# SaurabhIndi/unet-segmentation

Measured on AMD Instinct MI355X. Metric: training images/sec (512×512×1, batch=8) at 1/2/4/8 MI355X; IoU vs ref, higher is better.
Workload: dtype fp32; 1 GPU; U-Net train step 512x512x1, batch 8/GPU, fp32 GEMMs (fwd+WCE+bwd+SGD); global_batch=8, image=512, parallelism=dp1

## Files before the change

### include/unet_hip.h

```cpp
#ifndef UNET_HIP_H
#define UNET_HIP_H

#include <stddef.h>
#include <stdint.h>

#ifdef __cplusplus
extern "C" {
#endif

typedef void* unet_stream_t;

const char* unet_version(void);
const char* unet_last_error(void);

typedef struct unet_plan unet_plan;

unet_plan* unet_plan_create(int n, int c_in, int h, int w, int n_classes);

enum { UNET_PREC_FP32 = 0, UNET_PREC_BF16 = 1, UNET_PREC_BF16X3 = 2 };
unet_plan* unet_plan_create_ex(int n, int c_in, int h, int w, int n_classes, int precision);
int unet_plan_precision(const unet_plan* p);
void unet_plan_destroy(unet_plan* p);
int unet_plan_out_hw(const unet_plan* p, int* out_h, int* out_w);
size_t unet_plan_workspace_bytes(const unet_plan* p);
size_t unet_plan_forward_workspace_bytes(const unet_plan* p);
int unet_plan_num_params(const unet_plan* p);
int unet_plan_num_grads(const unet_plan* p);

int unet_plan_forward(unet_plan* p, void* const* host_params, const float* x_nchw,
                      float* logits_nchw, void* workspace, int train, unet_stream_t stream);

int unet_plan_num_segments(const unet_plan* p);
int unet_plan_segment_grads(const unet_plan* p, int seg, int* first_grad, int* n_grads);
int unet_plan_backward(unet_plan* p, void* const* host_params, void* const* host_grads,
                       const float* x_nchw, const float* dlogits_nchw, void* workspace,
                       int seg_begin, int seg_end, unet_stream_t stream);
size_t unet_plan_input_grad_scratch_bytes(const unet_plan* p);
int unet_plan_input_grad(unet_plan* p, void* const* params, float* dx, void* workspace, void* scratch,
                         unet_stream_t stream);
enum { UNET_BWD_DEFER_JOIN = 1 };
int unet_plan_backward_ex(unet_plan* p, void* const* host_params, void* const* host_grads,
                          const float* x_nchw, const float* dlogits_nchw, void* workspace,
                          int seg_begin, int seg_end, int flags, unet_stream_t stream);
int unet_plan_wait_segment(unet_plan* p, int seg, unet_stream_t stream);
int unet_plan_join(unet_plan* p, unet_stream_t stream);

enum {
  UNET_KC_CONV_FWD = 0, UNET_KC_CONV_DGRAD = 1, UNET_KC_CONV_WGRAD = 2,
  UNET_KC_STAGE1 = 3,
  UNET_KC_ELEMWISE = 4,
  UNET_KC_BOTTLENECK = 5,
  UNET_KC_COUNT = 6
};
int unet_plan_set_timing(unet_plan* p, int enable);
int unet_plan_timing(const unet_plan* p, double* ms, double* flops, double* bytes, int* launches);
int unet_plan_timing_mfma_flops(const unet_plan* p, double* mfma_flops);
size_t unet_plan_timing_sites(const unet_plan* p, char* buf, size_t cap);

int unet_wce_fwd_bwd(const float* logits, const int64_t* targets, const float* weights,
                     int n, int k, int h, int w,
                     const int64_t* t_strides , const int64_t* w_strides ,
                     float* loss_out, float* dlogits, float grad_scale, void* ws,
                     unet_stream_t stream);
int unet_scale_by_device_scalar(float* x, size_t n, const float* g, unet_stream_t stream);
int unet_scale_by_device_scalar_out(const float* x, float* y, size_t n, const float* g, unet_stream_t stream);

int unet_sgd_momentum(float* p, const float* g, float* buf, size_t n, float lr, float momentum,
                      float grad_scale, int first_step, unet_stream_t stream);

int unet_iou_counts(const uint8_t* pred, const uint8_t* gt, size_t n, unsigned long long* out,
                    unet_stream_t stream);
int unet_mask_from_logits(const float* logits, uint8_t* mask, int n, int h, int w,
                          unet_stream_t stream);

size_t unet_elastic_ws_bytes(int n, int h, int w);
int unet_elastic_deform(const uint8_t* image, const uint16_t* labels, int n, int h, int w,
                        const double* noise, double alpha, double sigma, float* x_out,
                        uint8_t* target_out, uint8_t* image_out, void* ws, unet_stream_t stream);
int unet_elastic_deform_ex(const uint8_t* image, const uint16_t* labels, int n, int h, int w,
                           const double* noise, double alpha, double sigma, float* x_out,
                           uint8_t* target_out, uint8_t* image_out, uint16_t* ids_out, void* ws,
                           unet_stream_t stream);

int unet_tile_gather(const float* image, int c, int h, int w, int tile_in, int tile_out, int top, int left,
                     int nx, int first, int stride, int ntiles, float* tiles, unet_stream_t stream);
int unet_tile_scatter(const float* tile_logits, int k, int tile_out, int nx, int first, int stride, int ntiles,
                      int h, int w, float* logits, uint8_t* mask, unet_stream_t stream);

size_t unet_weight_map_ws_bytes(int n);
int unet_weight_map(const uint16_t* labels, int n, int h, int w, double w0, double sigma, float* weights,
                    double* weights64, void* ws, unet_stream_t stream);

size_t unet_weight_map_border_ws_bytes(int n, int h, int w);
int unet_weight_map_border(const uint16_t* labels, int n, int h, int w, double w0, double sigma, float* weights,
                           double* weights64, int32_t* d1sq, int32_t* d2sq, void* ws, unet_stream_t stream);

size_t unet_instance_masks_ws_bytes(int n, int h, int w);
int unet_instance_masks(const uint8_t* mask, int n, int h, int w, int min_size, uint16_t* labels, void* ws,
                        unet_stream_t stream);
size_t unet_rand_index_ws_bytes(int h, int w);
int unet_rand_index(const uint16_t* gt, const uint16_t* pred, int h, int w, double* out, void* ws,
                    unet_stream_t stream);

typedef struct unet_tracker unet_tracker;
unet_tracker* unet_tracker_create(int h, int w, double iou_track, double iou_division, int max_children);
void unet_tracker_destroy(unet_tracker* t);
size_t unet_tracker_ws_bytes(int h, int w);
int unet_tracker_add_frame(unet_tracker* t, const uint16_t* labels, int frame, void* ws, unet_stream_t stream);
int unet_tracker_step_host(unet_tracker* t, int frame, int n_curr, const int32_t* host_labels,
                           const int64_t* host_areas, const int64_t* host_inter);
int unet_tracker_num_tracks(const unet_tracker* t);
int unet_tracker_tracks(const unet_tracker* t, int32_t* host_out, int cap);
int unet_linear_sum_assignment(long long nr, long long nc, const double* host_cost, int64_t* host_row_ind,
                               int64_t* host_col_ind);

enum { UNET_CTC_SEG = 0, UNET_CTC_TRA = 1 };
enum { UNET_CTC_GT = 0, UNET_CTC_RES = 1 };
typedef struct unet_ctc unet_ctc;
unet_ctc* unet_ctc_create(void);
void unet_ctc_destroy(unet_ctc* c);
size_t unet_ctc_ws_bytes(int t, int h, int w);
int unet_ctc_add_frames(unet_ctc* c, int kind, const uint16_t* gt, const uint16_t* res, const int32_t* host_frames,
                        int t, int h, int w, void* ws, unet_stream_t stream);
int unet_ctc_add_frame_host(unet_ctc* c, int kind, int frame, int n_gt, const int32_t* host_gt_labels,
                            const int64_t* host_gt_areas, int n_res, const int32_t* host_res_labels,
                            const int64_t* host_res_areas, int n_pairs, const int64_t* host_pairs);
int unet_ctc_set_tracks(unet_ctc* c, int side, const int32_t* host_rows, int n);
int unet_ctc_measures(unet_ctc* c, double* host_out, int64_t* host_counts);
long long unet_ctc_log(unet_ctc* c, char* buf, size_t cap);
int unet_ctc_num_frames(const unet_ctc* c, int kind);
int unet_ctc_frame_sizes(const unet_ctc* c, int kind, int index, int32_t* host_out);
int unet_ctc_frame_tables(const unet_ctc* c, int kind, int index, int32_t* host_gt_labels, int64_t* host_gt_areas,
                          int32_t* host_res_labels, int64_t* host_res_areas, int64_t* host_pairs);
int unet_ctc_stats(const unet_ctc* c, int64_t* host_out);

enum { UNET_WARP_FORCE_WS = 1 };
size_t unet_warping_error_ws_bytes(int n, int h, int w);
int unet_warping_error(const uint16_t* gt, const uint8_t* pred, int n, int h, int w, int radius, int separate,
                       int max_sweeps, int flags, uint8_t* warped, int64_t* counts, void* ws, unet_stream_t stream);
void unet_simple_point_table(uint8_t out[256]);

int unet_set_tuning(const char* key, int value);
size_t unet_tuning_report(char* buf, size_t len);
int unet_tuning_reset(void);
long long unet_slab_fallbacks(int reset);
long long unet_nondeterministic_sites(int reset);
long long unet_fused_bnb_sites(int reset);
long long unet_wgrad_oihw_sites(int reset);
long long unet_igemm_plane_launches(int reset);
int unet_tuning_save(const char* path);
int unet_tuning_load(const char* path);

int unet_conv3x3_fwd(const float* x, int n, int h, int w, int ci, const float* wt_oihw,
                     const float* bias, int co, const float* x_scale, const float* x_shift,
                     float* y, void* ws, unet_stream_t stream);
int unet_conv3x3_dgrad(const float* dy, int n, int h, int w, int ci, const float* wt_oihw,
                       int co, float* dx, void* ws, unet_stream_t stream);
int unet_conv3x3_wgrad(const float* x, const float* dy, int n, int h, int w, int ci, int co,
                       float* dw_oihw, float* db, void* ws, unet_stream_t stream);
size_t unet_conv_ws_bytes(int n, int h, int w, int ci, int co);
int unet_convT2_fwd(const float* x, int n, int h, int w, int ci, const float* wt, const float* bias,
                    int co, float* y, void* ws, unet_stream_t stream);
int unet_convT2_bwd(const float* x, const float* dy, int n, int h, int w, int ci, const float* wt,
                    int co, float* dx, float* dw, float* db, void* ws, unet_stream_t stream);
int unet_maxpool2_fwd(const float* x, int n, int h, int w, int c, float* y, uint8_t* arg,
                      unet_stream_t stream);
int unet_maxpool2_bwd(const float* dy, const uint8_t* arg, int n, int h, int w, int c, float* dx,
                      unet_stream_t stream);
int unet_bn_train_fwd(const float* x, int n, int h, int w, int c, const float* gamma,
                      const float* beta, float* running_mean, float* running_var, float* y,
                      float* save_mean, float* save_invstd, void* ws, unet_stream_t stream);
int unet_bn_train_bwd(const float* x, const float* dy, int n, int h, int w, int c,
                      const float* gamma, const float* save_mean, const float* save_invstd,
                      float* dx, float* dgamma, float* dbeta, void* ws, unet_stream_t stream);
size_t unet_bn_ws_bytes(int c);

size_t unet_bn_relu_ws_bytes(int n, int h, int w, int c);
int unet_bn_relu_fwd(const float* x, int n, int h, int w, int c, const float* gamma, const float* beta,
                     float* running_mean, float* running_var, int64_t* nbt, float momentum, float eps,
                     int training, int relu, float* y, float* save_mean, float* save_invstd, void* ws,
                     unet_stream_t stream);
int unet_bn_relu_bwd(const float* x, const float* y, const float* dy, int n, int h, int w, int c,
                     const float* gamma, const float* save_mean, const float* save_invstd, int training,
                     int relu, float* dx, float* dgamma, float* dbeta, void* ws, unet_stream_t stream);
size_t unet_conv_first_ws_bytes(int n, int ci, int h, int w);
int unet_conv_first_fwd(const float* x_nchw, int n, int ci, int h, int w, const float* wt, const float* bias,
                        float* y, unet_stream_t stream);
int unet_conv_first_bwd(const float* x_nchw, const float* dy, int n, int ci, int h, int w, const float* wt,
                        float* dx_nchw, float* dw, float* db, void* ws, unet_stream_t stream);
size_t unet_conv1x1_ws_bytes(int k);
int unet_conv1x1_fwd(const float* x, int n, int h, int w, int c, const float* wt, const float* bias, int k,
                     float* logits_nchw, unet_stream_t stream);
int unet_conv1x1_bwd(const float* x, const float* dlogits_nchw, int n, int h, int w, int c, const float* wt, int k,
                     float* dx, float* dw, float* db, void* ws, unet_stream_t stream);

int unet_peak_probe(int kind, int reps, double* result, unet_stream_t stream);

#ifdef __cplusplus
}
#endif
#endif
```

### unet-segmentation_amd/csrc/igemm.hip

```cpp
#include <algorithm>
#include <cstdio>
#include <cstdlib>

#include "gemm_common.h"
#include "ring_common.h"

namespace unet {
constexpr int igemm_minw(int BM, int BN, int WM, int WN, int BK) {
  const int lds = 2 * (BM + BN) * (BK + 4) * 4 + WM * 3 * BN * 4;
  int blocks = 163840 / lds;
  if (blocks > 8) blocks = 8;
  int w = blocks * WM * WN * 64 / 256;
  if (WM * WN >= 8 && w > 2) w = 2;
  return w < 1 ? 1 : (w > 8 ? 8 : w);
}

template <int BM, int BN, int WM, int WN, int BK, int ABL = 0, int PF = 1>
__global__ __launch_bounds__(WM * WN * 64, igemm_minw(BM, BN, WM, WN, BK)) void k_igemm(const IgemmArgs args) {
  constexpr int NT = WM * WN * 64;
  constexpr int LDK = BK + 4;
  constexpr int TM = BM / (WM * 32), TN = BN / (WN * 32);
  constexpr int C4 = BK / 4;
  constexpr int RPP = NT / C4;
  constexpr int AV = BM / RPP, BV = BN / RPP;
// ... 963 lines not shown
int g_tune_igemm = env_int("UNET_IGEMM_VARIANT", -1);
int g_tune_wgrad = env_int("UNET_WGRAD_VARIANT", -1);
std::atomic<long long> g_slab_fallbacks{0};
int g_wino_max = env_int("UNET_WINO_MAX", 4);
int g_wino_dgrad_max = env_int("UNET_WINO_DGRAD_MAX", 4);
int g_wino_wgrad_max = env_int("UNET_WINO_WGRAD_MAX", 6);
int g_wino4_fwd_min_cg = env_int("UNET_WINO4_FWD_MIN_CG", 128);
int g_wino4_fwd_small_cg = env_int("UNET_WINO4_FWD_SMALL_CG", 0);
template <int BM, int BN, int WM, int WN, int BK>
static hipError_t go_igemm(const IgemmArgs& a, hipStream_t s) {
  if (a.N % BN != 0 || a.K % BK != 0 || a.a.Cg % BK != 0 || a.a.c_split % BK != 0) return hipErrorInvalidValue;
  if (a.batch > 1) {
    if (a.ksplit > 1 || a.batch_rows < 1) return hipErrorInvalidValue;
    dim3 grid((a.batch_rows + BM - 1) / BM, a.N / BN, a.batch);
    if (WM == 2 && WN == 2 && igemm_plane_applies(a, BM, BN, BK)) return launch_igemm_plane(a, s, grid, BM, BN, BK);
    hipLaunchKernelGGL((k_igemm<BM, BN, WM, WN, BK>), grid, dim3(WM * WN * 64), 0, s, a);
    return hipGetLastError();
  }
  dim3 grid((a.M + BM - 1) / BM, a.N / BN, a.ksplit > 1 ? a.ksplit : 1);
  hipLaunchKernelGGL((k_igemm<BM, BN, WM, WN, BK>), grid, dim3(WM * WN * 64), 0, s, a);
  return hipGetLastError();
}

template <int BM, int BN, int WM, int WN>
static hipError_t go_igemm_g(const IgemmArgs& a, hipStream_t s) {
  if (a.N % BN != 0 || a.K % 16 != 0 || a.a.Cg % 16 != 0 || a.a.c_split % 16 != 0) return hipErrorInvalidValue;
  static bool attr = false;
  const size_t full = igemm_g_smem<BM, BN>(1024);
  if (!attr) {
    hipError_t e = hipFuncSetAttribute(reinterpret_cast<const void*>(&k_igemm_g<BM, BN, WM, WN>),
                                       hipFuncAttributeMaxDynamicSharedMemorySize, (int)full);
    if (e != hipSuccess) return e;
    attr = true;
  }
  const bool tf = a.a.s[0].scale != nullptr || (a.a.c_split < a.a.Cg && a.a.s[1].scale != nullptr);
  if (tf && a.a.Cg > 1024) return hipErrorInvalidValue;
  const size_t smem = igemm_g_smem<BM, BN>(tf ? a.a.Cg : 0);
  dim3 grid((a.M + BM - 1) / BM, a.N / BN, a.ksplit > 1 ? a.ksplit : 1);
  hipLaunchKernelGGL((k_igemm_g<BM, BN, WM, WN>), grid, dim3(WM * WN * 64), smem, s, a);
  return hipGetLastError();
}

template <int TH, int TW, int BN, int WM, int WN, int MINW>
static hipError_t go_halo32(const IgemmArgs& a, hipStream_t s) {
  if (a.b == nullptr || a.N % BN != 0 || a.a.Cg % 16 != 0 || a.a.c_split % 16 != 0 || a.a.taps_h != 3 ||
      a.a.taps_w != 3 || a.a.stride != 1 || a.K != 9 * a.a.Cg)
    return hipErrorInvalidValue;
  constexpr size_t smem = conv3_f32_smem<TH, TW, BN>();
  static bool attr = false;
  if (!attr) {
    hipError_t e = hipFuncSetAttribute(reinterpret_cast<const void*>(&k_conv3_f32<TH, TW, BN, WM, WN, MINW>),
                                       hipFuncAttributeMaxDynamicSharedMemorySize, (int)smem);
    if (e != hipSuccess) return e;
    attr = true;
  }
  const long long tiles = (long long)a.a.nimg * ((a.a.Hg + TH - 1) / TH) * ((a.a.Wg + TW - 1) / TW);
  dim3 grid((unsigned)tiles, a.N / BN, a.ksplit > 1 ? a.ksplit : 1);
  hipLaunchKernelGGL((k_conv3_f32<TH, TW, BN, WM, WN, MINW>), grid, dim3(WM * WN * 64), smem, s, a);
  return hipGetLastError();
}


template <int BM, int BN>
static hipError_t go_wgrad_f32(const WgradArgs& a, hipStream_t s, dim3 grid) {
  hipLaunchKernelGGL((k_wgrad<BM, BN, 2, 2>), grid, dim3(256), 0, s, a);
  return hipGetLastError();
}

bool reg_tile_fits(const IgemmArgs& a, const IgemmTile& t) {
  return igemm_prec_ok(a, t) && a.N % t.bn == 0 && a.K % t.bk == 0 && a.a.Cg % t.bk == 0 && a.a.c_split % t.bk == 0;
}
bool halo_tile_fits(const IgemmArgs& a, const IgemmTile& t) {
  return igemm_prec_ok(a, t) && a.N % t.bn == 0 && a.a.taps_h == 3 && a.a.taps_w == 3 && a.a.stride == 1 &&
         a.K == 9 * a.a.Cg && a.a.Cg % t.ch == 0 && a.a.c_split % t.ch == 0 && (!t.bf16 || a.a.Cg <= 1024);
}
template <int BM, int BN, int WM, int WN, int BK>
static constexpr IgemmTile reg_tile(int id, int slots) {
  return {id, IgemmFamily::Reg, BM, BN, BK, slots, 0, 0, 0, 0, false, false, true, true, reg_tile_fits,
          &go_igemm<BM, BN, WM, WN, BK>, nullptr, nullptr};
}
template <int BM, int BN, int WM, int WN>
static constexpr IgemmTile dma_tile(int id, int slots) {
  return {id, IgemmFamily::Reg, BM, BN, 16, slots, 0, 0, 0, 0, false, false, true, true, reg_tile_fits,
          &go_igemm_g<BM, BN, WM, WN>, nullptr, nullptr};
}
template <int TH, int TW, int BN, int WM, int WN, int MINW>
static constexpr IgemmTile halo32_tile(int id, int slots) {
  return conv3_tile(id, IgemmFamily::Halo, TH, TW, BN, 16, slots, false, false, true, halo_tile_fits,
                    &go_halo32<TH, TW, BN, WM, WN, MINW>);
}
static const IgemmTile kF32Tiles[] = {
    reg_tile<256, 128, 4, 2, 16>(4, 2),    reg_tile<128, 128, 2, 2, 16>(1, 3),   reg_tile<64, 128, 2, 2, 16>(2, 4),
    reg_tile<128, 64, 2, 2, 16>(8, 4),     reg_tile<256, 64, 4, 1, 16>(6, 2),    reg_tile<128, 128, 2, 2, 32>(3, 2),
    reg_tile<64, 128, 2, 2, 32>(9, 2),     reg_tile<256, 64, 4, 1, 32>(7, 1),    dma_tile<256, 128, 4, 2>(11, 2),
    dma_tile<128, 128, 2, 2>(12, 3),       dma_tile<64, 128, 2, 2>(13, 4),       dma_tile<128, 64, 2, 2>(14, 4),
    halo32_tile<8, 32, 64, 8, 1, 4>(51, 2), halo32_tile<16, 16, 64, 8, 1, 4>(52, 2), halo32_tile<8, 32, 64, 4, 1, 2>(53, 2),
    halo32_tile<8, 16, 64, 4, 1, 2>(54, 2),
};

const std::vector<IgemmTile>& igemm_tiles() {
  static const std::vector<IgemmTile> table = [] {
    std::vector<IgemmTile> v;
    for (IgemmTileRows r : {tile_rows(kF32Tiles), igemm_bf16_tile_rows(), conv3_dma_tile_rows(), conv3_ring_tile_rows(),
                            conv3_ring_pt_tile_rows(), conv3_flat_tile_rows(), wino_tile_rows(),
                            conv3_ring_persistent_tile_rows(), gemm_ring_tile_rows(), gemm_ring_p1_tile_rows(),
                            gemm_ring_p2_tile_rows(), conv3_c64_tile_rows()})
      v.insert(v.end(), r.p, r.p + r.n);
    std::stable_partition(v.begin(), v.end(), [](const IgemmTile& t) { return t.tuned; });
    return v;
  }();
  return table;
}

const IgemmTile* igemm_tile(int id) {
  static const std::vector<const IgemmTile*> by_id = [] {
    std::vector<const IgemmTile*> v;
    for (const IgemmTile& t : igemm_tiles()) {
      if ((size_t)t.id >= v.size()) v.resize(t.id + 1, nullptr);
      v[t.id] = &t;
    }
    return v;
  }();
  return id >= 0 && (size_t)id < by_id.size() ? by_id[id] : nullptr;
}

bool igemm_tile_fits(const IgemmArgs& a, int tile) {
  const IgemmTile* t = igemm_tile(tile);
  if (!t) return false;
  const bool fwd = a.fwd != 0;
  if (t->wino_m > (fwd ? g_wino_max : g_wino_dgrad_max)) return false;
  if (fwd && t->wino_m >= 4 && a.a.Cg < g_wino4_fwd_min_cg && a.a.Cg > g_wino4_fwd_small_cg) return false;
  return t->fits(a, *t);
}
long long igemm_tile_count(const IgemmArgs& a, int tile) {
  const IgemmTile* t = igemm_tile(tile);
  if (!t) return 0;
  if (t->count) return t->count(a);
  if (t->th) return (long long)a.a.nimg * ((a.a.Hg + t->th - 1) / t->th) * ((a.a.Wg + t->tw - 1) / t->tw) * (a.N / t->bn);
  return (long long)((a.M + t->bm - 1) / t->bm) * (a.N / t->bn);
}
int igemm_tile_slots(int tile) {
  const IgemmTile* t = igemm_tile(tile);
  return t ? t->slots : 0;
}
size_t igemm_slab_bytes(const IgemmArgs& a, int ksplit) {
  return ksplit > 1 ? (size_t)ksplit * a.M * a.N * sizeof(float) : 0;
}

static hipError_t go_tile(const IgemmArgs& a, hipStream_t s, int tile) {
  const IgemmTile* t = igemm_tile(tile);
  return t ? t->go(a, s) : hipErrorInvalidValue;
}

static bool igemm_args_ok(const IgemmArgs& a) {
  return a.M > 0 && a.N > 0 && a.K > 0 && (a.K % 16) == 0 && (a.a.Cg % 16) == 0 && (a.a.c_split % 16) == 0;
}

GemmChoice resolve_forced_igemm(const IgemmArgs& a, int knob) {
  return knob > 0 && igemm_tile_fits(a, knob) ? GemmChoice{knob, 1} : GemmChoice{};
}

int igemm_heuristic_tile(const IgemmArgs& a) {
  const GemmChoice forced = resolve_forced_igemm(a, g_tune_igemm);
  if (forced.tile >= 0) return forced.tile;
  const long long cus = num_cus();
  if (a.bh != nullptr) {
    if (a.K % 32 || a.a.Cg % 32 || a.a.c_split % 32) return -1;
    if (a.N % 128 == 0) {
      const long long t256 = ((a.M + 255) / 256) * (long long)(a.N / 128);
      const long long t128 = ((a.M + 127) / 128) * (long long)(a.N / 128);
      if (a.N >= 256 && t256 >= 3 * cus / 2) return 21;
      if (t128 >= 2 * cus) return 22;
      return 24;
    }
    return a.N % 64 == 0 ? 23 : -1;
  }
  if (a.N % 128 == 0) {
    const long long t256 = ((a.M + 255) / 256) * (long long)(a.N / 128);
    const long long t128 = ((a.M + 127) / 128) * (long long)(a.N / 128);
    if (a.N >= 256 && t256 >= 3 * cus / 2) return 4;
    if (t128 >= 4 * cus) return 1;
    return 2;
  }
  if (a.N % 64 == 0) return 8;
  return -1;
}

hipError_t launch_igemm(const IgemmArgs& a0, hipStream_t s) {
  if (!igemm_args_ok(a0)) return hipErrorInvalidValue;
  IgemmArgs a = a0;
  a.ksplit = 1;
  return go_tile(a, s, igemm_heuristic_tile(a));
}

hipError_t launch_igemm_v(const IgemmArgs& a0, hipStream_t s, GemmChoice c) {
  if (c.tile < 0) return launch_igemm(a0, s);
  if (!igemm_args_ok(a0) || !igemm_tile_fits(a0, c.tile)) return hipErrorInvalidValue;
  const IgemmTile& t = *igemm_tile(c.tile);
  IgemmArgs a = a0;
  const int nk = a.K / t.bk;
  if (t.family == IgemmFamily::Wino && c.split >= 100) a.wino_choice.tile = c.split - 100;
  int ks = c.split < 1 || t.wino_m ? 1 : (c.split > nk ? nk : c.split);
  if (ks > 1) {
    const int per = (nk + ks - 1) / ks;
    ks = (nk + per - 1) / per;
  }
  a.ksplit = ks;
  if (ks > 1 && (!t.ksplit || a.slab == nullptr || a.N % 64 != 0)) return hipErrorInvalidValue;
  hipError_t e = t.go(a, s);
  if (e != hipSuccess || ks == 1) return e;
  dim3 grid((a.M + 127) / 128, a.N / 64);
  hipLaunchKernelGGL(k_splitk_epi, grid, dim3(256), 0, s, a);
  return hipGetLastError();
}

static bool wgrad_column_fits(const WgradArgs& a, const WgradTile& t) {
  return t.bf16 == (a.bf16 != 0) && a.Mo % t.bm == 0 && a.No % t.bn == 0;
}
template <int BM, int BN>
static constexpr WgradTile wgrad_f32_tile(int id) {
  return {id, WgradFamily::Column, BM, BN, 0, 0, 0, false, 8, wgrad_column_fits, nullptr, &go_wgrad_f32<BM, BN>};
}
template <int TH, int TW>
static constexpr WgradTile wgrad3_f32_tile(int id) {
  return {id, WgradFamily::Halo, 64, 64, TH, TW, 0, false, 4, wgrad3_f32_fits,
          [](const WgradArgs& a, hipStream_t s, WgradMode m) { return go_wgrad3_f32<TH, TW>(a, s, m.per_cu); }, nullptr};
}
static const WgradTile kWgradF32Tiles[] = {wgrad_f32_tile<128, 128>(0), wgrad_f32_tile<128, 192>(1),
                                           wgrad_f32_tile<64, 192>(2), wgrad_f32_tile<64, 128>(3),
                                           wgrad_f32_tile<64, 64>(4)};
static const WgradTile kWgrad3F32Tiles[] = {wgrad3_f32_tile<8, 16>(22), wgrad3_f32_tile<4, 32>(23)};

const std::vector<WgradTile>& wgrad_tiles() {
  static const std::vector<WgradTile> table = [] {
    std::vector<WgradTile> v;
    for (WgradTileRows r : {tile_rows(kWgradF32Tiles), wgrad_bf16_tile_rows(), wgrad3_bf16_tile_rows(),
                            tile_rows(kWgrad3F32Tiles), wgrad3w_tile_rows(), wgrad3_ring_tile_rows(),
                            wgradT_ring_tile_rows(), wino_wgrad_tile_rows()})
      v.insert(v.end(), r.p, r.p + r.n);
    return v;
  }();
  return table;
}

const WgradTile* wgrad_tile(int id) {
  for (const WgradTile& t : wgrad_tiles())
    if (t.id == id) return &t;
  return nullptr;
}

WgradMode decode(const WgradTile& t, int code) {
  WgradMode m{t.default_per_cu, -1, false};
  switch (t.family) {
    case WgradFamily::Column:
      m.slab = code >= 100;
      if (m.slab) code -= 100;
      if (code > 0) m.per_cu = code;
      break;
    case WgradFamily::Halo:
      if (code > 0) m.per_cu = code;
      break;
    case WgradFamily::Ring:
    case WgradFamily::RingT:
      if (code <= 0) code = t.default_per_cu;
      m.slab = code >= 10;
      m.per_cu = m.slab ? code - 10 : code;
      break;
    case WgradFamily::Wino:
      m.slab = code >= 1000;
      code %= 1000;
      if (code >= 100) m.inner = code / 100 - 1;
      if (code % 100 > 0) m.per_cu = code % 100;
      break;
  }
  return m;
}
int encode(const WgradTile& t, WgradMode m) {
  switch (t.family) {
    case WgradFamily::Column: return m.per_cu + (m.slab ? 100 : 0);
    case WgradFamily::Halo: return m.per_cu;
    case WgradFamily::Ring:
    case WgradFamily::RingT: return m.per_cu + (m.slab ? 10 : 0);
    default: return m.per_cu + 100 * (m.inner + 1) + (m.slab ? 1000 : 0);
  }
}

bool wgrad_tile_fits(const WgradArgs& a, int tile) {
  const WgradTile* t = wgrad_tile(tile);
  if (!t || t->wino_m > g_wino_wgrad_max) return false;
  if (a.batch > 1 && (t->family != WgradFamily::Column || t->bf16)) return false;
  return t->fits(a, *t);
}

GemmChoice resolve_forced_wgrad(const WgradArgs& a, int knob) {
  const bool bf16 = a.bf16 != 0;
  const WgradTile* t = wgrad_tile(knob);
  if (t && (bf16 ? knob >= 10 : t->family != WgradFamily::Column) && wgrad_tile_fits(a, knob))
    return {knob, t->family == WgradFamily::Column ? knob : 1};
  t = wgrad_tile(knob - 1000);
  if (t && t->family == WgradFamily::Wino && !bf16 && wgrad_tile_fits(a, t->id)) return {t->id, encode(*t, {0, -1, true})};
  t = wgrad_tile(knob - 100);
  if (t && t->bf16 == bf16 && wgrad_tile_fits(a, t->id)) {
    if (t->family == WgradFamily::Column) return {t->id, encode(*t, {2, -1, true})};
    if (t->family == WgradFamily::Ring || t->family == WgradFamily::RingT) return {t->id, encode(*t, {1, -1, true})};
  }
  if (knob == 1 && !bf16) return {4, 8};
  return {};
}

static int wgrad_heuristic_tile(const WgradArgs& a) {
  if (a.bf16) {
    if (wgrad3_fits(a)) return 20;
    if (a.Mo % 128 == 0 && a.No % 128 == 0) return 10;
    return a.No % 128 == 0 ? 12 : 13;
  }
  if (a.Mo % 128 == 0 && a.No % 128 == 0) return 0;
  if (a.Mo % 128 == 0 && a.No % 192 == 0) return 1;
  if (a.No % 192 == 0) return 2;
  return a.No % 128 == 0 ? 3 : 4;
}

hipError_t launch_wgrad_v(const WgradArgs& a0, hipStream_t s, GemmChoice c) {
  WgradArgs a = a0;
  if (a.Mo % 64 != 0 || a.P <= 0 || a.gb.Cg % 4 != 0 || a.gb.c_split % 4 != 0 || a.ga.Cg % 4 != 0)
    return hipErrorInvalidValue;
  const bool heuristic = c.tile < 0 && resolve_forced_wgrad(a, g_tune_wgrad).tile < 0;
  if (heuristic) c.tile = wgrad_heuristic_tile(a);
  else if (c.tile < 0) c = resolve_forced_wgrad(a, g_tune_wgrad);
  if (!wgrad_tile_fits(a, c.tile)) return hipErrorInvalidValue;
  const WgradTile& t = *wgrad_tile(c.tile);
  WgradMode m = decode(t, c.split);
  if (heuristic && t.family == WgradFamily::Column) m = {g_tune_wgrad >= 2 ? g_tune_wgrad : 8, -1, false};
  if (t.go) return t.go(a, s, m);
  int pps = 0;
  const int splits = wgrad_splits(a, t, m.per_cu, pps);
  a.pix_per_split = pps;
  const size_t plane = (size_t)a.Mo * a.No;
  if (!(m.slab && wgrad_slab_fits(a, splits))) {
    if (m.slab) ++g_slab_fallbacks;
    a.slab = nullptr;
  }
  else if (splits == 1) a.slab = a.out;
// ... 57 lines not shown
```

### unet-segmentation_amd/csrc/ops.hip

```cpp
#include <algorithm>
#include <cerrno>
#include <string>

#include "../../include/unet_hip.h"
#include "unet_internal.h"

using namespace unet;

namespace unet {
extern int g_tune_igemm, g_tune_wgrad, g_autotune, g_force_split, g_force_tile, g_concurrent, g_wino_max,
    g_wino_dgrad_max, g_wino_wgrad_max, g_bf16_norm, g_bn_fold, g_wino4_fwd_min_cg, g_wino4_fwd_small_cg,
    g_maxpool_vec8, g_wgrad_fwd_u, g_ctc_chunk_frames, g_ctc_dense_cells;
hipError_t launch_fill(float* p, size_t n, float v, hipStream_t s);
hipError_t launch_pair_sum(const double* st, int g, int c, float* out, hipStream_t s);
}

namespace {
thread_local std::string g_op_err;
inline size_t al256(size_t b) { return (b + 255) / 256 * 256; }
int g_op_prec = UNET_PREC_FP32;
int g_op_a16 = 0;

hipError_t op_b_to_bf16(IgemmArgs& a, size_t n, void* scratch, hipStream_t s) {
  if (g_op_prec == UNET_PREC_FP32) return hipSuccess;
  uint16_t* bh = reinterpret_cast<uint16_t*>(scratch);
  uint16_t* bl = g_op_prec == UNET_PREC_BF16X3 ? bh + n : nullptr;
  hipError_t e = launch_f2bf(a.b, bh, n, s, bl);
  a.bh = bh;
  a.bl = bl;
  a.b = nullptr;
  return e;
}
}

namespace {
__global__ void k_relu_mask(const float* __restrict__ dy, const float* __restrict__ y, long long n4,
                            float* __restrict__ dz) {
  for (long long i = blockIdx.x * (long long)blockDim.x + threadIdx.x; i < n4; i += (long long)gridDim.x * blockDim.x) {
    const float4 g = reinterpret_cast<const float4*>(dy)[i], v = reinterpret_cast<const float4*>(y)[i];
    reinterpret_cast<float4*>(dz)[i] =
        make_float4(v.x > 0.f ? g.x : 0.f, v.y > 0.f ? g.y : 0.f, v.z > 0.f ? g.z : 0.f, v.w > 0.f ? g.w : 0.f);
  }
}

__global__ void k_bn_eval_stats(int C, const float* rm, const float* rv, float eps, float* mean, float* invstd) {
  const int c = blockIdx.x * blockDim.x + threadIdx.x;
  if (c >= C) return;
  mean[c] = rm[c];
  invstd[c] = (float)(1.0 / sqrt((double)rv[c] + (double)eps));
}
}

#define OPCK(x)                                                           \
  do {                                                                    \
    hipError_t e_ = (x);                                                  \
    if (e_ != hipSuccess) return e_ == hipErrorInvalidValue ? -EINVAL : -EIO; \
  } while (0)

extern "C" {

static size_t op_wino_bytes(int ci, int co) { return al256(sizeof(float) * 36 * (size_t)ci * co); }
static size_t op_wgrad_wino_bytes(int n, int h, int w, int ci, int co);
static size_t op_wgrad_extra_bytes(int n, int h, int w, int ci, int co);
static void op_set_wino(IgemmArgs& a, void* ws, int n, int h, int w, int ci, int co) {
  const size_t ws_bytes = unet_conv_ws_bytes(n, h, w, ci, co);
  const IgemmTile* forced = igemm_tile(g_tune_igemm);
  if (forced && forced->family == IgemmFamily::Wino && op_wgrad_extra_bytes(n, h, w, ci, co)) {
    a.wino_ws = reinterpret_cast<float*>(reinterpret_cast<char*>(ws) + ws_bytes - op_wino_bytes(ci, co) -
                                         op_wgrad_extra_bytes(n, h, w, ci, co));
    a.wino_ws_bytes = op_wgrad_wino_bytes(n, h, w, ci, co);
    return;
  }
  a.wino_ws = reinterpret_cast<float*>(reinterpret_cast<char*>(ws) + ws_bytes - op_wino_bytes(ci, co));
  a.wino_ws_bytes = op_wino_bytes(ci, co);
}

static size_t op_wgrad_wino_bytes(int n, int h, int w, int ci, int co) {
  return al256(wino_ws_bytes_grid(n, h, w, ci, co));
}
static size_t op_wgrad_slab_bytes(int n, int h, int w, int ci, int co) {
  const long long t4 = (long long)n * ((h + 3) / 4) * ((w + 3) / 4);
  return al256(sizeof(float) * 64 * (size_t)std::min<long long>(64, (t4 + 255) / 256) * ci * co);
}
static size_t op_wgrad_extra_bytes(int n, int h, int w, int ci, int co) {
  const size_t b = op_wgrad_wino_bytes(n, h, w, ci, co) + op_wgrad_slab_bytes(n, h, w, ci, co);
  return b <= ((size_t)256 << 20) ? b : 0;
}

size_t unet_conv_ws_bytes(int n, int h, int w, int ci, int co) {
  const size_t wb = al256(sizeof(float) * 9 * (size_t)ci * co);
  const size_t pad = al256(sizeof(float) * (size_t)n * (h + 2) * (w + 2) * co);
  const size_t misc = al256(sizeof(float) * 4 * co) + al256(sizeof(double) * kStatGroups * 2 * co);
  const size_t x16 = al256(sizeof(uint16_t) * (size_t)n * h * w * ci);
  return 2 * wb + pad + misc + x16 + op_wgrad_extra_bytes(n, h, w, ci, co) + op_wino_bytes(ci, co);
}

int unet_conv3x3_fwd(const float* x, int n, int h, int w, int ci, const float* wt, const float* bias, int co,
                     const float* xs, const float* xb, float* y, void* ws, unet_stream_t st) {
  if (ci % 16 || co % 64 || h < 3 || w < 3) return -EINVAL;
  hipStream_t s = reinterpret_cast<hipStream_t>(st);
  float* wf = reinterpret_cast<float*>(ws);
  OPCK(launch_pack_conv(wt, co, ci, 3, 3, wf, nullptr, s));
  IgemmArgs a;
  Src x0;
  x0.ptr = x;
  x0.H = h;
  x0.W = w;
  x0.C = ci;
  x0.scale = xs;
  x0.shift = xb;
  if (g_op_prec == UNET_PREC_BF16 && g_op_a16) {
    const size_t wb = al256(sizeof(float) * 9 * (size_t)ci * co);
    const size_t off = 2 * wb + al256(sizeof(float) * (size_t)n * (h + 2) * (w + 2) * co) +
                       al256(sizeof(float) * 4 * co) + al256(sizeof(double) * kStatGroups * 2 * co);
    uint16_t* x16 = reinterpret_cast<uint16_t*>(reinterpret_cast<char*>(ws) + off);
    OPCK(launch_f2bf(x, x16, (size_t)n * h * w * ci, s));
    x0.ptr = reinterpret_cast<const float*>(x16);
    x0.h16 = 1;
  }
  a.a.s[0] = a.a.s[1] = x0;
  a.a.Cg = a.a.c_split = ci;
  a.a.taps_h = a.a.taps_w = 3;
  a.a.Hg = h - 2;
  a.a.Wg = w - 2;
  a.a.nimg = n;
  a.b = wf;
  a.M = n * (h - 2) * (w - 2);
  a.N = co;
  a.K = 9 * ci;
  a.e.bias = bias;
  a.e.d[0] = Dst{y, h - 2, w - 2, co, 0, 0};
  op_set_wino(a, ws, n, h, w, ci, co);
  OPCK(op_b_to_bf16(a, 9 * (size_t)ci * co, reinterpret_cast<char*>(ws) + al256(sizeof(float) * 9 * (size_t)ci * co),
                    s));
  OPCK(launch_igemm(a, s));
  return 0;
}

int unet_conv3x3_dgrad(const float* dy, int n, int h, int w, int ci, const float* wt, int co, float* dx, void* ws,
                       unet_stream_t st) {
  if (ci % 64 || co % 16 || h < 3 || w < 3) return -EINVAL;
  hipStream_t s = reinterpret_cast<hipStream_t>(st);
  char* p = reinterpret_cast<char*>(ws);
  const size_t wb = al256(sizeof(float) * 9 * (size_t)ci * co);
  float* wf = reinterpret_cast<float*>(p);
  float* wd = reinterpret_cast<float*>(p + wb);
  float* dyp = reinterpret_cast<float*>(p + 2 * wb);
  float* coef = reinterpret_cast<float*>(p + 2 * wb + al256(sizeof(float) * (size_t)n * (h + 2) * (w + 2) * co));
  OPCK(launch_pack_conv(wt, co, ci, 3, 3, wf, wd, s));
  OPCK(launch_fill(coef, co, 1.f, s));
  OPCK(launch_fill(coef + co, 3 * (size_t)co, 0.f, s));
  const int dy16 = g_op_prec == UNET_PREC_BF16 && g_op_a16;
  OPCK(launch_bnb_apply(dy, dy, coef, n, h - 2, w - 2, co, dyp, 2, s, dy16, 0));
  IgemmArgs a;
  Src d;
  d.ptr = dyp;
  d.h16 = dy16;
  d.H = h + 2;
  d.W = w + 2;
  d.C = co;
  a.a.s[0] = a.a.s[1] = d;
  a.a.Cg = a.a.c_split = co;
  a.a.taps_h = a.a.taps_w = 3;
  a.a.Hg = h;
  a.a.Wg = w;
  a.a.nimg = n;
  a.b = wd;
  a.M = n * h * w;
  a.N = ci;
  a.K = 9 * co;
  a.e.d[0] = Dst{dx, h, w, ci, 0, 0};
  op_set_wino(a, ws, n, h, w, ci, co);
  OPCK(op_b_to_bf16(a, 9 * (size_t)ci * co, wf, s));
  OPCK(launch_igemm(a, s));
  return 0;
}

int unet_conv3x3_wgrad(const float* x, const float* dy, int n, int h, int w, int ci, int co, float* dw, float* db,
                       void* ws, unet_stream_t st) {
  if (ci % 64 || co % 64 || h < 3 || w < 3) return -EINVAL;
  hipStream_t s = reinterpret_cast<hipStream_t>(st);
  char* p = reinterpret_cast<char*>(ws);
  const size_t wb = al256(sizeof(float) * 9 * (size_t)ci * co);
  float* dwp = reinterpret_cast<float*>(p);
  double* st2 = reinterpret_cast<double*>(p + 2 * wb + al256(sizeof(float) * (size_t)n * (h + 2) * (w + 2) * co) +
                                          al256(sizeof(float) * 4 * co));
  OPCK(hipMemsetAsync(dwp, 0, sizeof(float) * 9 * (size_t)ci * co, s));
  WgradArgs a;
  Src d;
  d.ptr = dy;
  d.H = h - 2;
  d.W = w - 2;
  d.C = co;
  a.ga.s[0] = a.ga.s[1] = d;
  a.ga.Cg = a.ga.c_split = co;
  a.ga.Hg = h - 2;
  a.ga.Wg = w - 2;
  a.ga.nimg = n;
  Src xs;
  xs.ptr = x;
  xs.H = h;
  xs.W = w;
  xs.C = ci;
  a.gb.s[0] = a.gb.s[1] = xs;
  a.gb.Cg = a.gb.c_split = ci;
  a.gb.taps_h = a.gb.taps_w = 3;
  a.gb.Hg = h - 2;
  a.gb.Wg = w - 2;
  a.gb.nimg = n;
  a.Mo = co;
  a.No = 9 * ci;
  a.P = n * (h - 2) * (w - 2);
  a.out = dwp;
  a.bf16 = g_op_prec != UNET_PREC_FP32;
  a.split = g_op_prec == UNET_PREC_BF16X3;
  if (g_op_prec == UNET_PREC_BF16 && g_op_a16) {
    uint16_t* dy16 = reinterpret_cast<uint16_t*>(p + 2 * wb);
    float* coef = reinterpret_cast<float*>(p + 2 * wb + al256(sizeof(float) * (size_t)n * (h + 2) * (w + 2) * co));
    uint16_t* x16 = reinterpret_cast<uint16_t*>(p + 2 * wb + al256(sizeof(float) * (size_t)n * (h + 2) * (w + 2) * co) +
                                                al256(sizeof(float) * 4 * co) +
                                                al256(sizeof(double) * kStatGroups * 2 * co));
    OPCK(launch_fill(coef, co, 1.f, s));
    OPCK(launch_fill(coef + co, 3 * (size_t)co, 0.f, s));
    OPCK(launch_bnb_apply(dy, dy, coef, n, h - 2, w - 2, co, reinterpret_cast<float*>(dy16), 2, s, 1, 0));
    OPCK(launch_f2bf(x, x16, (size_t)n * h * w * ci, s));
    a.ga.s[0].ptr = a.ga.s[1].ptr = reinterpret_cast<const float*>(dy16);
    a.ga.s[0].H = a.ga.s[1].H = h + 2;
    a.ga.s[0].W = a.ga.s[1].W = w + 2;
    a.ga.s[0].oy = a.ga.s[1].oy = a.ga.s[0].ox = a.ga.s[1].ox = 2;
    a.ga.s[0].h16 = a.ga.s[1].h16 = 1;
    a.gb.s[0].ptr = a.gb.s[1].ptr = reinterpret_cast<const float*>(x16);
    a.gb.s[0].h16 = a.gb.s[1].h16 = 1;
  }
  const WgradTile* forced = wgrad_tile(g_tune_wgrad >= 1000 ? g_tune_wgrad - 1000 : g_tune_wgrad);
  if (forced && forced->family == WgradFamily::Wino && !a.bf16 && op_wgrad_extra_bytes(n, h, w, ci, co)) {
    char* e = p + unet_conv_ws_bytes(n, h, w, ci, co) - op_wino_bytes(ci, co) - op_wgrad_extra_bytes(n, h, w, ci, co);
    a.wino_ws = reinterpret_cast<float*>(e);
    a.wino_ws_bytes = op_wgrad_wino_bytes(n, h, w, ci, co);
    a.slab = reinterpret_cast<float*>(e + a.wino_ws_bytes);
    a.slab_bytes = op_wgrad_slab_bytes(n, h, w, ci, co);
  }
  OPCK(launch_wgrad(a, s));
  OPCK(launch_permute_last2(dwp, co, 9, ci, dw, s));
  if (db) {
    OPCK(hipMemsetAsync(st2, 0, sizeof(double) * kStatGroups * 2 * co, s));
    OPCK(launch_channel_stats(dy, (size_t)n * (h - 2) * (w - 2), co, st2, s));
    OPCK(launch_pair_sum(st2, kStatGroups, co, db, s));
  }
  return 0;
}

int unet_convT2_fwd(const float* x, int n, int h, int w, int ci, const float* wt, const float* bias, int co, float* y,
                    void* ws, unet_stream_t st) {
  if (ci % 16 || co % 16) return -EINVAL;
  hipStream_t s = reinterpret_cast<hipStream_t>(st);
  char* p = reinterpret_cast<char*>(ws);
  float* wf = reinterpret_cast<float*>(p);
  float* wd = reinterpret_cast<float*>(p + al256(sizeof(float) * 4 * (size_t)ci * co));
  OPCK(launch_pack_convT(wt, ci, co, wf, wd, s));
  IgemmArgs a;
  Src x0;
  x0.ptr = x;
  x0.H = h;
  x0.W = w;
  x0.C = ci;
  a.a.s[0] = a.a.s[1] = x0;
  a.a.Cg = a.a.c_split = ci;
  a.a.Hg = h;
  a.a.Wg = w;
  a.a.nimg = n;
  a.b = wf;
  a.M = n * h * w;
  a.N = 4 * co;
  a.K = ci;
  a.e.bias = bias;
  a.e.shuffle_co = co;
  a.e.d[0] = Dst{y, 2 * h, 2 * w, co, 0, 0};
  OPCK(op_b_to_bf16(a, 4 * (size_t)ci * co, p + 2 * al256(sizeof(float) * 4 * (size_t)ci * co), s));
  OPCK(launch_igemm(a, s));
  return 0;
}

int unet_convT2_bwd(const float* x, const float* dy, int n, int h, int w, int ci, const float* wt, int co, float* dx,
                    float* dw, float* db, void* ws, unet_stream_t st) {
  if (ci % 64 || co % 64) return -EINVAL;
  hipStream_t s = reinterpret_cast<hipStream_t>(st);
  char* p = reinterpret_cast<char*>(ws);
  const size_t wb = al256(sizeof(float) * 4 * (size_t)ci * co);
  float* wf = reinterpret_cast<float*>(p);
  float* wd = reinterpret_cast<float*>(p + wb);
  float* dwp = reinterpret_cast<float*>(p + 2 * wb);
  double* st2 = reinterpret_cast<double*>(p + 3 * wb);
  OPCK(launch_pack_convT(wt, ci, co, wf, wd, s));
  Src d;
  d.ptr = dy;
  d.H = 2 * h;
  d.W = 2 * w;
  d.C = co;
  IgemmArgs a;
  a.a.s[0] = a.a.s[1] = d;
  a.a.Cg = a.a.c_split = co;
  a.a.taps_h = a.a.taps_w = 2;
  a.a.stride = 2;
  a.a.Hg = h;
  a.a.Wg = w;
  a.a.nimg = n;
  a.b = wd;
  a.M = n * h * w;
  a.N = ci;
  a.K = 4 * co;
  a.e.d[0] = Dst{dx, h, w, ci, 0, 0};
  OPCK(op_b_to_bf16(a, 4 * (size_t)ci * co, wf, s));
  OPCK(launch_igemm(a, s));
  OPCK(hipMemsetAsync(dwp, 0, sizeof(float) * 4 * (size_t)ci * co, s));
  WgradArgs g;
  Src x0;
  x0.ptr = x;
  x0.H = h;
  x0.W = w;
  x0.C = ci;
  g.ga.s[0] = g.ga.s[1] = x0;
  g.ga.Cg = g.ga.c_split = ci;
  g.ga.Hg = h;
  g.ga.Wg = w;
  g.ga.nimg = n;
// ... 81 lines not shown
  double* stats = reinterpret_cast<double*>(p);
  float* scale = reinterpret_cast<float*>(p + al256(sizeof(double) * kStatGroups * 2 * c));
  float* shift = scale + al256(sizeof(float) * c) / 4;
  const size_t pix = (size_t)n * h * w;
  if (training) {
    OPCK(hipMemsetAsync(stats, 0, sizeof(double) * kStatGroups * 2 * c, s));
    OPCK(launch_channel_stats(x, pix, c, stats, s));
    OPCK(launch_bn_finalize(stats, c, (double)pix, gamma, beta, rm, rv, nbt, save_mean, save_invstd, scale, shift,
                            momentum, eps, s));
  } else {
    OPCK(launch_bn_eval_prepare(c, gamma, beta, rm, rv, scale, shift, eps, s));
    hipLaunchKernelGGL(k_bn_eval_stats, dim3((c + 255) / 256), dim3(256), 0, s, c, rm, rv, eps, save_mean,
                       save_invstd);
    OPCK(hipGetLastError());
  }
  OPCK(launch_affine_relu(x, pix, c, scale, shift, relu, y, s));
  return 0;
}

int unet_bn_relu_bwd(const float* x, const float* y, const float* dy, int n, int h, int w, int c, const float* gamma,
                     const float* save_mean, const float* save_invstd, int training, int relu, float* dx,
                     float* dgamma, float* dbeta, void* ws, unet_stream_t st) {
  if (!x || !dy || !dx || !gamma || c < 4 || c % 4 || 256 % (c / 4) || n < 1 || (relu && !y)) return -EINVAL;
  hipStream_t s = reinterpret_cast<hipStream_t>(st);
  char* p = reinterpret_cast<char*>(ws);
  double* stats = reinterpret_cast<double*>(p);
  float* coef = reinterpret_cast<float*>(p + al256(sizeof(double) * kStatGroups * 2 * c));
  float* dz = reinterpret_cast<float*>(p + unet_bn_ws_bytes(c));
  const size_t pix = (size_t)n * h * w;
  const float* g = dy;
  if (relu) {
    const long long n4 = (long long)(pix * c / 4);
    hipLaunchKernelGGL(k_relu_mask, dim3((unsigned)std::min<long long>((n4 + 255) / 256, 8192)), dim3(256), 0, s, dy,
                       y, n4, dz);
    OPCK(hipGetLastError());
    g = dz;
  }
  OPCK(hipMemsetAsync(stats, 0, sizeof(double) * kStatGroups * 2 * c, s));
  OPCK(launch_bn_bwd_stats(g, x, save_mean, save_invstd, pix, c, stats, s));
  OPCK(launch_bnb_finalize(stats, c, (double)pix, gamma, save_mean, save_invstd, dgamma, dbeta, nullptr, coef, s,
                           training ? 0 : 1));
  OPCK(launch_bnb_apply(g, x, coef, n, h, w, c, dx, 0, s));
  return 0;
}

size_t unet_conv_first_ws_bytes(int n, int ci, int h, int w) {
  (void)n; (void)h; (void)w;
  return conv_first_wgrad_ws_bytes(ci) + al256(sizeof(double) * kStatGroups * 2 * 64);
}

int unet_conv_first_fwd(const float* x, int n, int ci, int h, int w, const float* wt, const float* bias, float* y,
                        unet_stream_t st) {
  if (!x || !wt || !bias || !y || n < 1 || ci < 1 || h < 3 || w < 3) return -EINVAL;
  OPCK(launch_conv_first_fwd(x, n, ci, h, w, wt, bias, 64, y, nullptr, reinterpret_cast<hipStream_t>(st)));
  return 0;
}

int unet_conv_first_bwd(const float* x, const float* dy, int n, int ci, int h, int w, const float* wt, float* dx,
                        float* dw, float* db, void* ws, unet_stream_t st) {
  if (!x || !dy || !wt || !dw || !db || !ws || n < 1 || ci < 1 || h < 3 || w < 3) return -EINVAL;
  hipStream_t s = reinterpret_cast<hipStream_t>(st);
  char* p = reinterpret_cast<char*>(ws);
  float* slabs = reinterpret_cast<float*>(p);
  double* st2 = reinterpret_cast<double*>(p + conv_first_wgrad_ws_bytes(ci));
  Src d;
  d.ptr = dy;
  d.H = h - 2;
  d.W = w - 2;
  d.C = 64;
  OPCK(launch_conv_first_wgrad(x, n, ci, h, w, d, 64, dw, slabs, s));
  OPCK(hipMemsetAsync(st2, 0, sizeof(double) * kStatGroups * 2 * 64, s));
  OPCK(launch_channel_stats(dy, (size_t)n * (h - 2) * (w - 2), 64, st2, s));
  OPCK(launch_pair_sum(st2, kStatGroups, 64, db, s));
  if (dx) OPCK(launch_conv_first_dgrad(dy, n, ci, h, w, wt, dx, s));
  return 0;
}

size_t unet_conv1x1_ws_bytes(int k) { return al256(sizeof(double) * ((size_t)k * 64 + k)); }

int unet_conv1x1_fwd(const float* x, int n, int h, int w, int c, const float* wt, const float* bias, int k,
                     float* logits, unet_stream_t st) {
  if (!x || !wt || !bias || !logits || c != 64 || k < 1 || n < 1) return -EINVAL;
  Src s0;
  s0.ptr = x;
  s0.H = h;
  s0.W = w;
  s0.C = 64;
  OPCK(launch_head_fwd(s0, n, h, w, 64, wt, bias, k, logits, reinterpret_cast<hipStream_t>(st)));
  return 0;
}

int unet_conv1x1_bwd(const float* x, const float* dl, int n, int h, int w, int c, const float* wt, int k, float* dx,
                     float* dw, float* db, void* ws, unet_stream_t st) {
  if (!x || !dl || !wt || !dw || !db || !ws || c != 64 || k < 1 || n < 1) return -EINVAL;
  OPCK(launch_head_bwd_plain(x, dl, n, h, w, wt, k, dx, dw, db, reinterpret_cast<double*>(ws),
                             reinterpret_cast<hipStream_t>(st)));
  return 0;
}

int unet_wce_fwd_bwd(const float* logits, const int64_t* t, const float* wm, int n, int k, int h, int w,
                     const int64_t* ts, const int64_t* wsd, float* loss, float* dl, float gscale, void* ws,
                     unet_stream_t st) {
  if (!ts || !wsd || k < 1) return -EINVAL;
  OPCK(launch_wce(logits, t, wm, n, k, h, w, ts, wsd, loss, dl, gscale, reinterpret_cast<double*>(ws),
                  reinterpret_cast<hipStream_t>(st)));
  return 0;
}

int unet_scale_by_device_scalar(float* x, size_t n, const float* g, unet_stream_t st) {
  OPCK(launch_scale_by_dev(x, x, n, g, reinterpret_cast<hipStream_t>(st)));
  return 0;
}

int unet_scale_by_device_scalar_out(const float* x, float* y, size_t n, const float* g, unet_stream_t st) {
  OPCK(launch_scale_by_dev(x, y, n, g, reinterpret_cast<hipStream_t>(st)));
  return 0;
}

int unet_sgd_momentum(float* p, const float* g, float* buf, size_t n, float lr, float mom, float gscale, int first,
                      unet_stream_t st) {
  OPCK(launch_sgd(p, g, buf, n, lr, mom, gscale, first, reinterpret_cast<hipStream_t>(st)));
  return 0;
}

int unet_iou_counts(const uint8_t* a, const uint8_t* b, size_t n, unsigned long long* out, unet_stream_t st) {
  OPCK(launch_iou(a, b, n, out, reinterpret_cast<hipStream_t>(st)));
  return 0;
}

int unet_set_tuning(const char* key, int value) {
  if (!key) return -EINVAL;
  const std::string k(key);
  if (k == "igemm_variant") g_tune_igemm = value;
  else if (k == "wgrad_variant") g_tune_wgrad = value;
  else if (k == "autotune") g_autotune = value;
  else if (k == "force_split") g_force_split = value;
  else if (k == "force_tile") g_force_tile = value;
  else if (k == "concurrent") g_concurrent = value;
  else if (k == "wino_max") g_wino_max = value;
  else if (k == "bf16_norm") g_bf16_norm = value;
  else if (k == "bn_fold") g_bn_fold = value != 0;
  else if (k == "wino_dgrad_max") g_wino_dgrad_max = value;
  else if (k == "wino_wgrad_max") g_wino_wgrad_max = value;
  else if (k == "wino4_fwd_min_cg") g_wino4_fwd_min_cg = value;
  else if (k == "wino4_fwd_small_cg") g_wino4_fwd_small_cg = value;
  else if (k == "op_a16") g_op_a16 = value != 0;
  else if (k == "maxpool_vec8") g_maxpool_vec8 = value;
  else if (k == "bnb_fuse") g_bnb_fuse = value;
  else if (k == "wgrad_early_u") g_wgrad_early_u = value;
  else if (k == "wgrad_fwd_u") g_wgrad_fwd_u = value;
  else if (k == "wgrad_plane") g_wgrad_plane = value;
  else if (k == "wgrad_oihw") g_wgrad_oihw = value;
  else if (k == "igemm_plane") g_igemm_plane = value;
  else if (k == "wino_point_tile") g_wino_point_tile = value;
  else if (k == "ctc_chunk_frames" || k == "ctc_dense_cells") {
    if (value < -1 || (value == 0 && k == "ctc_chunk_frames")) return -EINVAL;
    (k == "ctc_chunk_frames" ? g_ctc_chunk_frames : g_ctc_dense_cells) = value;
  }
  else if (k == "deterministic") g_deterministic = value != 0;
  else if (k == "op_precision") {
    if (value != UNET_PREC_FP32 && value != UNET_PREC_BF16 && value != UNET_PREC_BF16X3) return -EINVAL;
    g_op_prec = value;
  } else return -EINVAL;
  return 0;
}

int unet_tile_gather(const float* image, int c, int h, int w, int tile_in, int tile_out, int top, int left, int nx,
                     int first, int stride, int ntiles, float* tiles, unet_stream_t st) {
  if (!image || !tiles) return -EINVAL;
  OPCK(launch_tile_gather(image, c, h, w, tile_in, tile_out, top, left, nx, first, stride, ntiles, tiles,
                          reinterpret_cast<hipStream_t>(st)));
  return 0;
}

int unet_tile_scatter(const float* tile_logits, int k, int tile_out, int nx, int first, int stride, int ntiles, int h,
                      int w, float* logits, uint8_t* mask, unet_stream_t st) {
  if (!tile_logits) return -EINVAL;
  OPCK(launch_tile_scatter(tile_logits, k, tile_out, nx, first, stride, ntiles, h, w, logits, mask,
                           reinterpret_cast<hipStream_t>(st)));
  return 0;
}

size_t unet_instance_masks_ws_bytes(int n, int h, int w) {
  return n > 0 && h > 0 && w > 0 ? instance_masks_ws_bytes(n, h, w) : 0;
}

int unet_instance_masks(const uint8_t* mask, int n, int h, int w, int min_size, uint16_t* labels, void* ws,
                        unet_stream_t st) {
  if (!mask || !labels || !ws) return -EINVAL;
  OPCK(launch_instance_masks(mask, n, h, w, min_size, labels, ws, reinterpret_cast<hipStream_t>(st)));
  return 0;
}

size_t unet_rand_index_ws_bytes(int h, int w) { return h > 0 && w > 0 ? rand_index_ws_bytes(h, w) : 0; }

int unet_rand_index(const uint16_t* gt, const uint16_t* pred, int h, int w, double* out, void* ws,
                    unet_stream_t st) {
  if (!gt || !pred || !out || !ws) return -EINVAL;
  OPCK(launch_rand_index(gt, pred, h, w, out, ws, reinterpret_cast<hipStream_t>(st)));
  return 0;
}

size_t unet_weight_map_ws_bytes(int n) { return n > 0 ? weight_map_ws_bytes(n) : 0; }

int unet_weight_map(const uint16_t* labels, int n, int h, int w, double w0, double sigma, float* weights,
                    double* weights64, void* ws, unet_stream_t st) {
  if (!labels || !weights || !ws || (reinterpret_cast<uintptr_t>(ws) & 7)) return -EINVAL;
  OPCK(launch_weight_map(labels, n, h, w, w0, sigma, weights, weights64, ws, reinterpret_cast<hipStream_t>(st)));
  return 0;
}

size_t unet_weight_map_border_ws_bytes(int n, int h, int w) { return weight_map_border_ws_bytes(n, h, w); }

int unet_weight_map_border(const uint16_t* labels, int n, int h, int w, double w0, double sigma, float* weights,
                           double* weights64, int32_t* d1sq, int32_t* d2sq, void* ws, unet_stream_t st) {
  if (n < 1 || h < 1 || w < 1 || h > 16384 || w > 16384) {
    set_last_error("unet_weight_map_border: need n, h, w >= 1 and h, w <= 16384 (h^2 + w^2 must fit int32)");
    return -EINVAL;
  }
  if (!labels || !weights || !ws || (reinterpret_cast<uintptr_t>(ws) & 15)) {
    set_last_error("unet_weight_map_border: null labels / weights / ws, or ws not 16-byte aligned");
    return -EINVAL;
  }
  const hipError_t e = launch_weight_map_border(labels, n, h, w, w0, sigma, weights, weights64, d1sq, d2sq, ws,
                                                reinterpret_cast<hipStream_t>(st));
  if (e != hipSuccess) {
    set_last_error(std::string("unet_weight_map_border: ") + hipGetErrorString(e));
    return e == hipErrorInvalidValue ? -EINVAL : -EIO;
  }
  return 0;
}

size_t unet_elastic_ws_bytes(int n, int h, int w) { return n > 0 && h > 0 && w > 0 ? elastic_ws_bytes(n, h, w) : 0; }

int unet_elastic_deform_ex(const uint8_t* image, const uint16_t* labels, int n, int h, int w, const double* noise,
                           double alpha, double sigma, float* x_out, uint8_t* target_out, uint8_t* image_out,
                           uint16_t* ids_out, void* ws, unet_stream_t st) {
  if (!image || !labels || !noise || !x_out || !target_out || !ws || (reinterpret_cast<uintptr_t>(ws) & 7)) return -EINVAL;
  OPCK(launch_elastic(image, labels, n, h, w, noise, alpha, sigma, x_out, target_out, image_out, ids_out, ws,
                      reinterpret_cast<hipStream_t>(st)));
  return 0;
}

int unet_elastic_deform(const uint8_t* image, const uint16_t* labels, int n, int h, int w, const double* noise,
                        double alpha, double sigma, float* x_out, uint8_t* target_out, uint8_t* image_out, void* ws,
                        unet_stream_t st) {
  return unet_elastic_deform_ex(image, labels, n, h, w, noise, alpha, sigma, x_out, target_out, image_out, nullptr, ws,
                                st);
}

int unet_mask_from_logits(const float* logits, uint8_t* mask, int n, int h, int w, unet_stream_t st) {
  OPCK(launch_mask(logits, mask, n, h, w, reinterpret_cast<hipStream_t>(st)));
  return 0;
}

}
```

### unet-segmentation_amd/csrc/plan.hip

```cpp
#include <cerrno>
#include <cstdio>
#include <cstdlib>
#include <cstring>
#include <algorithm>
#include <array>
#include <map>
#include <mutex>
#include <string>
#include <vector>

#include "../../include/unet_hip.h"
#include "unet_internal.h"

using namespace unet;

namespace unet {
extern int g_wino_max, g_wino_dgrad_max, g_wino_wgrad_max, g_wino4_fwd_min_cg, g_wino4_fwd_small_cg;
int g_autotune = getenv("UNET_AUTOTUNE") ? atoi(getenv("UNET_AUTOTUNE")) : 1;
int g_concurrent = getenv("UNET_CONCURRENT") ? atoi(getenv("UNET_CONCURRENT")) : 1;
int g_bf16_norm = getenv("UNET_BF16_NORM") ? atoi(getenv("UNET_BF16_NORM")) : 0;
int g_bn_fold = getenv("UNET_BN_FOLD") ? atoi(getenv("UNET_BN_FOLD")) : 1;
int g_force_split = 0;
int g_force_tile = 0;
int g_deterministic = getenv("UNET_DETERMINISTIC") ? atoi(getenv("UNET_DETERMINISTIC")) : 0;
// ... 1224 lines not shown
      Conv& L = p->L[l];
      if (L.co % 64 == 0) L.vdw = al.take(bnb_wino6_vd_bytes(n, L.ho, L.wo, L.co));
    }
    for (int l = 1; l < 18 && unet::g_wgrad_fwd_u; ++l) {
      Conv& L = p->L[l];
      L.uws = al.take(wino_ws_bytes_grid(n, L.ho, L.wo, L.ci, L.co));
    }
  }
  p->wslab = al.take((size_t)2 * num_cus() * 128 * 9 * 64 * sizeof(float));
  p->ws_bytes = al.top;
  return p;
}

void unet_plan_destroy(unet_plan* p) {
  if (!p) return;
  if (p->side) {
    (void)hipStreamSynchronize(p->side);
    for (auto ev : p->ev_dy) (void)hipEventDestroy(ev);
    for (auto ev : p->ev_du) (void)hipEventDestroy(ev);
    for (auto ev : p->ev_seg) (void)hipEventDestroy(ev);
    (void)hipEventDestroy(p->ev_join);
    (void)hipEventDestroy(p->ev_bwd0);
    (void)hipEventDestroy(p->ev_fwdu);
    (void)hipStreamDestroy(p->side);
  }
  for (auto& e : p->evs) {
    (void)hipEventDestroy(e.a);
    (void)hipEventDestroy(e.b);
  }
  delete p;
}

int unet_plan_out_hw(const unet_plan* p, int* oh, int* ow) {
  if (!p) return -EINVAL;
  if (oh) *oh = p->ho;
  if (ow) *ow = p->wo;
  return 0;
}
size_t unet_plan_workspace_bytes(const unet_plan* p) { return p ? p->ws_bytes : 0; }
size_t unet_plan_forward_workspace_bytes(const unet_plan* p) { return p ? p->fwd_ws_bytes : 0; }
int unet_plan_num_params(const unet_plan*) { return 136; }
int unet_plan_num_grads(const unet_plan*) { return 82; }
int unet_plan_num_segments(const unet_plan*) { return 9; }
int unet_plan_segment_grads(const unet_plan*, int seg, int* first, int* cnt) {
  int f, k;
  if (seg == 0) { f = 70; k = 12; }
  else if (seg <= 3) { f = 70 - 10 * seg; k = 10; }
  else if (seg <= 8) { f = 8 * (8 - seg); k = 8; }
  else return -EINVAL;
  if (first) *first = f;
  if (cnt) *cnt = k;
  return 0;
}

int unet_plan_forward(unet_plan* p, void* const* prm, const float* x, float* logits, void* ws, int train,
                      unet_stream_t stream) {
  if (!p || !prm || !x || !logits || !ws) {
    set_err("unet_plan_forward: null argument");
    return -EINVAL;
  }
  if (reinterpret_cast<uintptr_t>(ws) & 255) {
    set_err("unet_plan_forward: workspace must be 256-byte aligned");
    return -EINVAL;
  }
  return run_forward(p, prm, x, logits, reinterpret_cast<char*>(ws), train, reinterpret_cast<hipStream_t>(stream));
}

int unet_plan_backward(unet_plan* p, void* const* prm, void* const* grd, const float* x, const float* dlogits,
                       void* ws, int sb, int se, unet_stream_t stream) {
  if (!p || !prm || !grd || !x || !dlogits || !ws || sb < 0 || se > 9 || sb >= se) {
    set_err("unet_plan_backward: bad argument");
    return -EINVAL;
  }
  return run_backward(p, prm, grd, x, dlogits, reinterpret_cast<char*>(ws), sb, se,
                      reinterpret_cast<hipStream_t>(stream), 0);
}

int unet_plan_backward_ex(unet_plan* p, void* const* prm, void* const* grd, const float* x, const float* dlogits,
                          void* ws, int sb, int se, int flags, unet_stream_t stream) {
  if (!p || !prm || !grd || !x || !dlogits || !ws || sb < 0 || se > 9 || sb >= se || (flags & ~UNET_BWD_DEFER_JOIN)) {
    set_err("unet_plan_backward_ex: bad argument");
    return -EINVAL;
  }
  return run_backward(p, prm, grd, x, dlogits, reinterpret_cast<char*>(ws), sb, se,
                      reinterpret_cast<hipStream_t>(stream), flags);
}

size_t unet_plan_input_grad_scratch_bytes(const unet_plan* p) {
  return p ? (size_t)p->n * p->L[0].ho * p->L[0].wo * p->L[0].co * sizeof(float) : 0;
}

int unet_plan_input_grad(unet_plan* p, void* const* prm, float* dx, void* ws, void* scratch, unet_stream_t stream) {
  if (!p || !prm || !dx || !ws || !scratch) {
    set_err("unet_plan_input_grad: bad argument");
    return -EINVAL;
  }
  const hipStream_t s = reinterpret_cast<hipStream_t>(stream);
  Ctx c{p, reinterpret_cast<char*>(ws), s};
  const Conv& L = p->L[0];
  const int g16 = p->prec == UNET_PREC_BF16;
  float* dy0 = reinterpret_cast<float*>(scratch);
  CK(launch_bnb_apply(c.f(L.dz), c.f(L.y), c.f(L.coef), p->n, L.ho, L.wo, L.co, dy0, 0, s, 0,
                      p->prec == UNET_PREC_BF16, g16));
  CK(launch_conv_first_dgrad(dy0, p->n, p->cin, p->h, p->w, P<float>(prm, L.pw), dx, s));
  return 0;
}

int unet_plan_wait_segment(unet_plan* p, int seg, unet_stream_t stream) {
  if (!p || seg < 0 || seg >= 9) {
    set_err("unet_plan_wait_segment: bad argument");
    return -EINVAL;
  }
  if (!p->seg_on_side[seg] || !p->side) return 0;
  CK(hipStreamWaitEvent(reinterpret_cast<hipStream_t>(stream), p->ev_seg[seg], 0));
  return 0;
}

int unet_plan_join(unet_plan* p, unet_stream_t stream) {
  if (!p) {
    set_err("unet_plan_join: null plan");
    return -EINVAL;
  }
  if (!p->side || !p->side_pending) return 0;
  CK(hipEventRecord(p->ev_join, p->side));
  CK(hipStreamWaitEvent(reinterpret_cast<hipStream_t>(stream), p->ev_join, 0));
  p->side_pending = false;
  return 0;
}

size_t unet_tuning_report(char* buf, size_t len) {
  std::string r;
  {
    std::lock_guard<std::mutex> lk(g_tune_mu);
    for (const auto& kv : g_tune_log) r += kv.second + "\n";
  }
  if (buf && len > 0) {
    const size_t k = std::min(len - 1, r.size());
    memcpy(buf, r.data(), k);
    buf[k] = 0;
  }
  return r.size() + 1;
}

long long unet_nondeterministic_sites(int reset) {
  return reset ? g_nondet_sites.exchange(0) : g_nondet_sites.load();
}

long long unet_fused_bnb_sites(int reset) {
  return reset ? unet::g_fused_bnb_sites.exchange(0) : unet::g_fused_bnb_sites.load();
}
long long unet_wgrad_oihw_sites(int reset) {
  return reset ? unet::g_wgrad_oihw_sites.exchange(0) : unet::g_wgrad_oihw_sites.load();
}
long long unet_igemm_plane_launches(int reset) {
  return reset ? unet::g_igemm_plane_launches.exchange(0) : unet::g_igemm_plane_launches.load();
}
long long unet_slab_fallbacks(int reset) {
  return reset ? g_slab_fallbacks.exchange(0) : g_slab_fallbacks.load();
}

int unet_tuning_reset(void) {
  std::lock_guard<std::mutex> lk(g_tune_mu);
  g_tuned.clear();
  g_tune_log.clear();
  return 0;
}

int unet_tuning_save(const char* path) {
  if (!path) return -EINVAL;
  std::lock_guard<std::mutex> lk(g_tune_mu);
  FILE* f = fopen(path, "w");
  if (!f) return -errno;
  for (const auto& kv : g_tuned) fprintf(f, "%s\t%d\t%d\n", kv.first.c_str(), kv.second.tile, kv.second.split);
  fclose(f);
  return (int)g_tuned.size();
}

int unet_tuning_load(const char* path) {
  if (!path) return -EINVAL;
  std::lock_guard<std::mutex> lk(g_tune_mu);
  return tune_db_read(path, true);
}

int unet_plan_set_timing(unet_plan* p, int enable) {
  if (!p) return -EINVAL;
  p->timing = enable != 0;
  return 0;
}

int unet_plan_timing(const unet_plan* pc, double* ms, double* fl, double* by, int* cnt) {
  auto* p = const_cast<unet_plan*>(pc);
  if (!p) return -EINVAL;
  int rc = 0;
  for (auto& e : p->evs) {
    float t = 0;
    if (hipEventSynchronize(e.b) != hipSuccess || hipEventElapsedTime(&t, e.a, e.b) != hipSuccess) {
      set_err("unet_plan_timing: event query failed");
      rc = -EIO;
    } else {
      p->t_ms[e.cls] += t;
      p->t_fl[e.cls] += e.flops;
      p->t_by[e.cls] += e.bytes;
      p->t_xf[e.cls] += e.xflops;
      p->t_n[e.cls] += 1;
      if (e.site >= 0) {
        auto& v = p->sites[e.site];
        v[0] += t;
        v[1] += e.flops;
        v[2] += e.xflops;
      }
    }
    (void)hipEventDestroy(e.a);
    (void)hipEventDestroy(e.b);
  }
  p->evs.clear();
  for (int i = 0; i < UNET_KC_COUNT; ++i) {
    if (ms) ms[i] = p->t_ms[i];
    if (fl) fl[i] = p->t_fl[i];
    if (by) by[i] = p->t_by[i];
    if (cnt) cnt[i] = p->t_n[i];
    p->t_xf_last[i] = p->t_xf[i];
    p->t_ms[i] = p->t_fl[i] = p->t_by[i] = p->t_xf[i] = 0;
    p->t_n[i] = 0;
  }
  p->sites_last.swap(p->sites);
  p->sites.clear();
  return rc;
}

size_t unet_plan_timing_sites(const unet_plan* p, char* buf, size_t cap) {
  if (!p) return 0;
  std::string out;
  for (const auto& kv : p->sites_last) {
    char line[160];
    snprintf(line, sizeof line, "%s\t%.4f\t%.6e\t%.6e\n", site_name(kv.first).c_str(), kv.second[0], kv.second[1],
             kv.second[2]);
    out += line;
  }
  if (buf && cap) {
    const size_t m = out.size() < cap - 1 ? out.size() : cap - 1;
    memcpy(buf, out.data(), m);
    buf[m] = 0;
  }
  return out.size() + 1;
}

int unet_plan_timing_mfma_flops(const unet_plan* p, double* xfl) {
  if (!p || !xfl) return -EINVAL;
  for (int i = 0; i < UNET_KC_COUNT; ++i) xfl[i] = p->t_xf_last[i];
  return 0;
}

}
```

### unet-segmentation_amd/csrc/unet_internal.h

```cpp
#pragma once
#include <hip/hip_runtime.h>
#include <cstddef>
#include <cstdint>
#include <atomic>
#include <string>
#include <vector>

namespace unet {

constexpr int kMaxInChannels = 4096;
constexpr int kMaxClassCount = 4096;

struct Src {
  const float* ptr = nullptr;
  int H = 0, W = 0, C = 0;
  int oy = 0, ox = 0;
  const float* scale = nullptr;
  const float* shift = nullptr;
  int h16 = 0;
};

struct Gather {
  Src s[2];
  int c_split = 0;
  int Cg = 0;
  int taps_h = 1, taps_w = 1;
  int stride = 1;
  int Hg = 0, Wg = 0;
  int nimg = 0;
};

struct Dst {
  float* ptr = nullptr;
  int H = 0, W = 0, C = 0;
  int oy = 0, ox = 0;
  int h16 = 0;
};

struct Epilogue {
  const float* bias = nullptr;
  int shuffle_co = 0;
  Dst d[2];
  int n_split = 1 << 30;
  int relu = 0;
  double* stats = nullptr;
  const float* yref = nullptr;
  int yref_h16 = 0;
  const float* bn_scale = nullptr;
  const float* bn_shift = nullptr;
  const float* bn_mean = nullptr;
  const float* bn_invstd = nullptr;
  double* bstats = nullptr;
  double* colsum1 = nullptr;
};

constexpr int kStatGroups = 64;

struct IgemmArgs {
  Gather a;
  const float* b = nullptr;
  const uint16_t* bh = nullptr;
  const uint16_t* bl = nullptr;
  int M, N, K;
  Epilogue e;
  int ksplit = 1;
  float* slab = nullptr;
  float* wino_ws = nullptr;
  size_t wino_ws_bytes = 0;
  int batch = 1;
  int batch_rows = 0;
  long long batch_b = 0;
  struct { int tile = -1, split = 1; } wino_choice;
  int fwd = 0;
};

extern std::atomic<long long> g_slab_fallbacks;
extern int g_deterministic;
extern int g_bnb_fuse;
extern int g_wgrad_early_u;
extern int g_wgrad_plane;
extern int g_wgrad_oihw;
extern int g_igemm_plane;
extern std::atomic<long long> g_igemm_plane_launches;
extern int g_wino_point_tile;
extern std::atomic<long long> g_nondet_sites;

struct WgradArgs {
  Gather ga;
  Gather gb;
  int Mo, No;
  int P;
  int pix_per_split;
  float* out;
  float* out_oihw = nullptr;
  float* slab = nullptr;
  size_t slab_bytes = 0;
  int accumulate = 0;
  int bf16 = 0;
  int split = 0;
  int batch = 1;
  long long batch_a = 0, batch_b = 0, batch_out = 0;
  float* wino_ws = nullptr;
  size_t wino_ws_bytes = 0;
  const float* vd_pre = nullptr;
  int u_ready = 0;
  int abl = 0;
};

struct GemmChoice {
  int tile = -1;
  int split = 1;
};

enum class IgemmFamily {
  Reg,
  Halo,
  Conv3Dma,
  Ring,
  Flat,
  C64,
  GemmRing,
  Wino,
  WinoFused
};
struct IgemmTile {
  int id;
  IgemmFamily family;
  int bm, bn, bk, slots;
  int th, tw, ch;
  int wino_m;
  bool bf16;
  bool x3;
  bool ksplit;
  bool tuned;
  bool (*fits)(const IgemmArgs&, const IgemmTile&);
  hipError_t (*go)(const IgemmArgs&, hipStream_t);
  long long (*count)(const IgemmArgs&);
  size_t (*slab_bytes)(const IgemmArgs&);
};
struct IgemmTileRows {
  const IgemmTile* p;
  int n;
};
template <int N>
constexpr IgemmTileRows tile_rows(const IgemmTile (&r)[N]) { return {r, N}; }
constexpr IgemmTile conv3_tile(int id, IgemmFamily f, int th, int tw, int bn, int ch, int slots, bool bf16, bool x3,
                               bool ksplit, bool (*fits)(const IgemmArgs&, const IgemmTile&),
                               hipError_t (*go)(const IgemmArgs&, hipStream_t)) {
  return {id, f, th * tw, bn, 9 * ch, slots, th, tw, ch, 0, bf16, x3, ksplit, true, fits, go, nullptr, nullptr};
}
IgemmTileRows igemm_bf16_tile_rows();
IgemmTileRows conv3_dma_tile_rows();
IgemmTileRows conv3_ring_tile_rows();
IgemmTileRows conv3_ring_pt_tile_rows();
IgemmTileRows conv3_ring_persistent_tile_rows();
IgemmTileRows conv3_flat_tile_rows();
IgemmTileRows conv3_c64_tile_rows();
IgemmTileRows gemm_ring_tile_rows();
IgemmTileRows gemm_ring_p1_tile_rows();
IgemmTileRows gemm_ring_p2_tile_rows();
IgemmTileRows wino_tile_rows();
const std::vector<IgemmTile>& igemm_tiles();
const IgemmTile* igemm_tile(int id);
inline bool igemm_prec_ok(const IgemmArgs& a, const IgemmTile& t) {
  return t.bf16 ? a.bh != nullptr && (a.bl == nullptr || t.x3) : a.b != nullptr;
}

enum class WgradFamily { Column, Halo, Ring, RingT, Wino };
struct WgradMode {
  int per_cu;
  int inner;
  bool slab;
};
struct WgradTile {
  int id;
  WgradFamily family;
  int bm, bn;
  int th, tw;
  int wino_m;
  bool bf16;
  int default_per_cu;
  bool (*fits)(const WgradArgs&, const WgradTile&);
  hipError_t (*go)(const WgradArgs&, hipStream_t, WgradMode);
  hipError_t (*go_column)(const WgradArgs&, hipStream_t, dim3 grid);
};
struct WgradTileRows {
  const WgradTile* p;
  int n;
};
template <int N>
constexpr WgradTileRows tile_rows(const WgradTile (&r)[N]) { return {r, N}; }
WgradTileRows wgrad_bf16_tile_rows();
WgradTileRows wgrad3_bf16_tile_rows();
WgradTileRows wgrad3w_tile_rows();
WgradTileRows wgrad3_ring_tile_rows();
WgradTileRows wgradT_ring_tile_rows();
WgradTileRows wino_wgrad_tile_rows();
const std::vector<WgradTile>& wgrad_tiles();
const WgradTile* wgrad_tile(int id);
WgradMode decode(const WgradTile& t, int code);
int encode(const WgradTile& t, WgradMode m);
GemmChoice resolve_forced_igemm(const IgemmArgs& a, int knob);
GemmChoice resolve_forced_wgrad(const WgradArgs& a, int knob);
size_t wino_ws_bytes(long long T, int Cg, int N);
size_t wino_ws_bytes_grid(int nimg, int H, int W, int Cg, int N);
bool wino_applies(const IgemmArgs& a, int mt);
hipError_t launch_wino(const IgemmArgs& a, hipStream_t s, int mt);
bool wino_wgrad_applies(const WgradArgs& a, int mt);
double igemm_exec_flops(const IgemmArgs& a, GemmChoice c);
double wgrad_exec_flops(const WgradArgs& a, GemmChoice c);
hipError_t launch_wino_wgrad(const WgradArgs& a, hipStream_t s, WgradMode m, int mt);
int wgrad_winograd_mt(const WgradArgs& a, GemmChoice c);
hipError_t launch_wino_wgrad_u(const WgradArgs& a, hipStream_t s, int mt);
size_t bnb_wino6_vd_bytes(int n, int h, int w, int c);
hipError_t launch_bnb_wino6_dy(const float* dz, const float* y, const float* coef, int n, int h, int w, int c,
                               float* dypad, float* vd, hipStream_t s);
bool conv3_ring_fits(const IgemmArgs& a, const IgemmTile& t);
bool gemm_ring_fits(const IgemmArgs& a, const IgemmTile& t);
size_t conv3_flat_sk_slab_bytes(const IgemmArgs& a);
int num_cus();

int ablation_env(const char* name);
hipError_t launch_igemm(const IgemmArgs& a, hipStream_t s);
hipError_t launch_igemm_v(const IgemmArgs& a, hipStream_t s, GemmChoice c);
int igemm_heuristic_tile(const IgemmArgs& a);
bool igemm_tile_fits(const IgemmArgs& a, int tile);
long long igemm_tile_count(const IgemmArgs& a, int tile);
int igemm_tile_slots(int tile);
size_t igemm_slab_bytes(const IgemmArgs& a, int ksplit);
std::string igemm_key(const IgemmArgs& a);
std::string wgrad_key(const WgradArgs& a);
std::vector<GemmChoice> igemm_candidates(const IgemmArgs& a, size_t slab_bytes);
std::vector<GemmChoice> wgrad_candidates(const WgradArgs& a);
bool wgrad_choice_deterministic(const GemmChoice& g);
hipError_t launch_wgrad(const WgradArgs& a, hipStream_t s);
hipError_t launch_wgrad_v(const WgradArgs& a, hipStream_t s, GemmChoice c);
// ... 123 lines not shown
```

### unet-segmentation_amd/csrc/winograd.hip

```cpp
#include <algorithm>
#include <cstdlib>

#include "gemm_common.h"
#include "ring_common.h"

namespace unet {

__global__ void k_wino_w(const float* __restrict__ b, int N, int Cg, float* __restrict__ v) {
  const long long i = blockIdx.x * (long long)blockDim.x + threadIdx.x;
  if (i >= (long long)N * Cg) return;
  const int n = (int)(i / Cg), c = (int)(i - (long long)n * Cg);
  float g[3][3];
#pragma unroll
  for (int t = 0; t < 9; ++t) g[t / 3][t % 3] = b[((size_t)n * 9 + t) * Cg + c];
  float tg[4][3];
#pragma unroll
  for (int k = 0; k < 3; ++k) {
    tg[0][k] = g[0][k];
    tg[1][k] = 0.5f * (g[0][k] + g[1][k] + g[2][k]);
    tg[2][k] = 0.5f * (g[0][k] - g[1][k] + g[2][k]);
    tg[3][k] = g[2][k];
  }
  const size_t plane = (size_t)N * Cg, o = (size_t)n * Cg + c;
#pragma unroll
  for (int r = 0; r < 4; ++r) {
    v[(r * 4 + 0) * plane + o] = tg[r][0];
    v[(r * 4 + 1) * plane + o] = 0.5f * (tg[r][0] + tg[r][1] + tg[r][2]);
    v[(r * 4 + 2) * plane + o] = 0.5f * (tg[r][0] - tg[r][1] + tg[r][2]);
    v[(r * 4 + 3) * plane + o] = tg[r][2];
  }
}

__global__ __launch_bounds__(256) void k_wino_in(Gather g, int Th, int Tw, long long T, float* __restrict__ u) {
  const int C4 = g.Cg / 4;
  const long long i = blockIdx.x * (long long)blockDim.x + threadIdx.x;
  if (i >= T * C4) return;
  const long long t = i / C4;
  const int c = (int)(i - t * C4) * 4;
  const int tx = (int)(t % Tw);
  const long long r = t / Tw;
  const int ty = (int)(r % Th), n = (int)(r / Th);
  const bool second = c >= g.c_split;
  const Src s = pick_src(g, second);
  const int cl = second ? c - g.c_split : c;
  float4 sc = make_float4(1.f, 1.f, 1.f, 1.f), sh = make_float4(0.f, 0.f, 0.f, 0.f);
  if (s.scale) {
    sc = ld4(s.scale + cl);
    sh = ld4(s.shift + cl);
  }
  float4 d[4][4];
#pragma unroll
  for (int yy = 0; yy < 4; ++yy)
#pragma unroll
    for (int xx = 0; xx < 4; ++xx) {
      const int y = 2 * ty + yy, x = 2 * tx + xx;
      const bool in = y < g.Hg + 2 && x < g.Wg + 2;
      float4 v = ld4(s.ptr + ((size_t)(n * s.H + (in ? y : 0) + s.oy) * s.W + (in ? x : 0) + s.ox) * s.C + cl);
      if (s.scale) v = affine_relu4(v, sc, sh);
      d[yy][xx] = in ? v : make_float4(0.f, 0.f, 0.f, 0.f);
    }
  float4 e[4][4];
#pragma unroll
  for (int xx = 0; xx < 4; ++xx) {
    e[0][xx] = d[0][xx] - d[2][xx];
    e[1][xx] = d[1][xx] + d[2][xx];
    e[2][xx] = d[2][xx] - d[1][xx];
    e[3][xx] = d[1][xx] - d[3][xx];
  }
  const size_t plane = (size_t)T * g.Cg, o = (size_t)t * g.Cg + c;
#pragma unroll
  for (int a = 0; a < 4; ++a) {
    st4(u + (a * 4 + 0) * plane + o, e[a][0] - e[a][2]);
    st4(u + (a * 4 + 1) * plane + o, e[a][1] + e[a][2]);
    st4(u + (a * 4 + 2) * plane + o, e[a][2] - e[a][1]);
    st4(u + (a * 4 + 3) * plane + o, e[a][1] - e[a][3]);
  }
}

__global__ __launch_bounds__(256) void k_wino_out(const float* __restrict__ m, long long T, int Th, int Tw, int N,
                                                  Gather g, Epilogue e) {
  const int C4 = N / 4;
  const int cgs = C4 < 64 ? C4 : 64;
  const int lanes = 256 / cgs;
  const int cg = blockIdx.y * cgs + (int)(threadIdx.x % cgs);
  const int tl = threadIdx.x / cgs;
  const bool active = cg < C4 && tl < lanes;
  const int col = cg * 4;
  const bool second = col >= e.n_split;
  float* dptr = second ? e.d[1].ptr : e.d[0].ptr;
  const int dC = second ? e.d[1].C : e.d[0].C;
  const int dcol = second ? col - e.n_split : col;
  const bool bwd_mask = e.yref != nullptr && !second;
  float4 bias = make_float4(0.f, 0.f, 0.f, 0.f), bsc, bsh, bmu, bis;
  if (active && e.bias) bias = ld4(e.bias + col);
  if (active && bwd_mask) {
    bsc = ld4(e.bn_scale + col); bsh = ld4(e.bn_shift + col);
    bmu = ld4(e.bn_mean + col); bis = ld4(e.bn_invstd + col);
  }
  float4 s1 = make_float4(0.f, 0.f, 0.f, 0.f), s2 = s1;
  const size_t plane = (size_t)T * N;
  if (active) {
    for (long long t = blockIdx.x * (long long)lanes + tl; t < T; t += (long long)gridDim.x * lanes) {
      float4 q[16];
#pragma unroll
      for (int p = 0; p < 16; ++p) q[p] = ld4(m + p * plane + (size_t)t * N + col);
      float4 w[2][4];
#pragma unroll
      for (int xx = 0; xx < 4; ++xx) {
        w[0][xx] = q[xx] + q[4 + xx] + q[8 + xx];
        w[1][xx] = q[4 + xx] - q[8 + xx] - q[12 + xx];
      }
      const int tx = (int)(t % Tw);
      const long long r = t / Tw;
      const int ty = (int)(r % Th), n = (int)(r / Th);
#pragma unroll
      for (int a = 0; a < 2; ++a)
#pragma unroll
        for (int bb = 0; bb < 2; ++bb) {
          const int y = 2 * ty + a, x = 2 * tx + bb;
          if (y >= g.Hg || x >= g.Wg) continue;
          float4 v = bb == 0 ? w[a][0] + w[a][1] + w[a][2] : w[a][1] - w[a][2] - w[a][3];
          v = v + bias;
          const size_t idx = ((size_t)(n * g.Hg + y) * g.Wg + x) * dC + dcol;
          if (bwd_mask) {
            const float4 yv = ld4(e.yref + idx);
            v.x = fmaf(yv.x, bsc.x, bsh.x) > 0.f ? v.x : 0.f;
            v.y = fmaf(yv.y, bsc.y, bsh.y) > 0.f ? v.y : 0.f;
            v.z = fmaf(yv.z, bsc.z, bsh.z) > 0.f ? v.z : 0.f;
            v.w = fmaf(yv.w, bsc.w, bsh.w) > 0.f ? v.w : 0.f;
            s1 = s1 + v;
            s2.x += v.x * ((yv.x - bmu.x) * bis.x);
            s2.y += v.y * ((yv.y - bmu.y) * bis.y);
            s2.z += v.z * ((yv.z - bmu.z) * bis.z);
            s2.w += v.w * ((yv.w - bmu.w) * bis.w);
          } else if (e.stats) {
            s1 = s1 + v;
            s2 = s2 + v * v;
          } else if (second && e.colsum1) {
            s1 = s1 + v;
          }
          if (e.relu) v = make_float4(fmaxf(v.x, 0.f), fmaxf(v.y, 0.f), fmaxf(v.z, 0.f), fmaxf(v.w, 0.f));
          st4(dptr + idx, v);
        }
    }
  }
  const bool want = e.stats || e.yref || e.colsum1;
  if (!want) return;
  __shared__ float red[256][8];
  red[threadIdx.x][0] = s1.x; red[threadIdx.x][1] = s1.y; red[threadIdx.x][2] = s1.z; red[threadIdx.x][3] = s1.w;
  red[threadIdx.x][4] = s2.x; red[threadIdx.x][5] = s2.y; red[threadIdx.x][6] = s2.z; red[threadIdx.x][7] = s2.w;
  __syncthreads();
  if (threadIdx.x < cgs && cg < C4) {
    float a[8] = {0, 0, 0, 0, 0, 0, 0, 0};
    for (int l = 0; l < lanes; ++l)
// ... 748 lines not shown
#pragma unroll
      for (int yy = 0; yy < 6; ++yy)
#pragma unroll
        for (int xx = 0; xx < 6; ++xx)
          raw[yy * 6 + xx] = *reinterpret_cast<const float*>(sb + (o0 + (yy * rs + xx * cs)));
    } else {
      const unsigned lr = (unsigned)max(vrows - 1, 0), lcn = (unsigned)max(vcols - 1, 0);
#pragma unroll
      for (int yy = 0; yy < 6; ++yy)
#pragma unroll
        for (int xx = 0; xx < 6; ++xx)
          raw[yy * 6 + xx] = *reinterpret_cast<const float*>(
              sb + (o0 + (min((unsigned)yy, lr) * rs + min((unsigned)xx, lcn) * cs)));
    }
    const char* vb = reinterpret_cast<const char*>(V + ((size_t)kc * 36 * N + n0) * 16);
    const unsigned vo = ((unsigned)(tid >> 7) * N * 16u + ((tid >> 2) & 31) * 16u + (tid & 3) * 4u) * 4u;
    const unsigned vstep = 4u * N * 16u * 4u;
#pragma unroll
    for (int j = 0; j < 9; ++j) vr[j] = *reinterpret_cast<const float4*>(vb + (vo + j * vstep));
  };
  auto commit = [&](int kc) {
    const bool second = kc * 16 >= g.c_split;
    const float* scp = second ? g.s[1].scale : g.s[0].scale;
    const float* shp = second ? g.s[1].shift : g.s[0].shift;
    const int cl = kc * 16 - (second ? g.c_split : 0) + lc;
    if constexpr (ABL & 1) {
#pragma unroll
      for (int q = 0; q < 36; ++q) Us[q * PS + uoff] = raw[q];
    } else {
    if (scp) {
      const float sc = scp[cl], sh = shp[cl];
#pragma unroll
      for (int q = 0; q < 36; ++q) raw[q] = fmaxf(fmaf(raw[q], sc, sh), 0.f);
    }
    if (!wfull) {
#pragma unroll
      for (int q = 0; q < 36; ++q) raw[q] = (q / 6 < vrows && q % 6 < vcols) ? raw[q] : 0.f;
    }
#pragma unroll
    for (int xx = 0; xx < 6; ++xx) {
      float d[6];
#pragma unroll
      for (int yy = 0; yy < 6; ++yy) d[yy] = raw[yy * 6 + xx];
      float rr[6];
      bt6(d, rr);
#pragma unroll
      for (int a = 0; a < 6; ++a) raw[a * 6 + xx] = rr[a];
    }
#pragma unroll
    for (int a = 0; a < 6; ++a) {
      float d[6];
#pragma unroll
      for (int xx = 0; xx < 6; ++xx) d[xx] = raw[a * 6 + xx];
      float rr[6];
      bt6(d, rr);
#pragma unroll
      for (int bb = 0; bb < 6; ++bb) Us[(a * 6 + bb) * PS + uoff] = rr[bb];
    }
    }
#pragma unroll
    for (int j = 0; j < 9; ++j) {
      const int q = tid + 512 * j;
      const int p = q >> 7, n = (q >> 2) & 31, piece = q & 3;
      st4(Vs + p * PS + wf_off(n, piece), vr[j]);
    }
  };

  const int th = wave & 1, pg = wave >> 1;
  const int mi = lane & 15, mq = lane >> 4;
  const int aoff = wf_off(16 * th + mi, mq);
  const int boff0 = wf_off(mi, mq), boff1 = wf_off(16 + mi, mq);
  floatx4 acc[9][2];
#pragma unroll
  for (int j = 0; j < 9; ++j)
#pragma unroll
    for (int hh = 0; hh < 2; ++hh) acc[j][hh] = (floatx4){0.f, 0.f, 0.f, 0.f};
  load(0);
  for (int kc = 0; kc < nk; ++kc) {
    commit(kc);
    __syncthreads();
    if (!(ABL & 4) && kc + 1 < nk) load(kc + 1);
    if constexpr (!(ABL & 2))
#pragma unroll
    for (int j = 0; j < 9; ++j) {
      const int p = pg * 9 + j;
      const float4 a = ld4(Us + p * PS + aoff);
      const float4 b0 = ld4(Vs + p * PS + boff0);
      const float4 b1 = ld4(Vs + p * PS + boff1);
      acc[j][0] = __builtin_amdgcn_mfma_f32_16x16x4f32(a.x, b0.x, acc[j][0], 0, 0, 0);
      acc[j][1] = __builtin_amdgcn_mfma_f32_16x16x4f32(a.x, b1.x, acc[j][1], 0, 0, 0);
      acc[j][0] = __builtin_amdgcn_mfma_f32_16x16x4f32(a.y, b0.y, acc[j][0], 0, 0, 0);
      acc[j][1] = __builtin_amdgcn_mfma_f32_16x16x4f32(a.y, b1.y, acc[j][1], 0, 0, 0);
      acc[j][0] = __builtin_amdgcn_mfma_f32_16x16x4f32(a.z, b0.z, acc[j][0], 0, 0, 0);
      acc[j][1] = __builtin_amdgcn_mfma_f32_16x16x4f32(a.z, b1.z, acc[j][1], 0, 0, 0);
      acc[j][0] = __builtin_amdgcn_mfma_f32_16x16x4f32(a.w, b0.w, acc[j][0], 0, 0, 0);
      acc[j][1] = __builtin_amdgcn_mfma_f32_16x16x4f32(a.w, b1.w, acc[j][1], 0, 0, 0);
    }
    __syncthreads();
  }

  float* X = lds;
#pragma unroll
  for (int j = 0; j < 9; ++j)
#pragma unroll
    for (int hh = 0; hh < 2; ++hh)
#pragma unroll
      for (int r = 0; r < 4; ++r)
        X[(pg * 9 + j) * 1024 + (16 * th + 4 * mq + r) * 32 + 16 * hh + mi] = acc[j][hh][r];
  __syncthreads();

  wf_output(lds, tid, t0, n0, T, Th, Tw, N, g, e);
}

bool wino_fused_applies(const IgemmArgs& a) {
  constexpr int ck = 16;
  const Gather& g = a.a;
  if (a.b == nullptr || a.bh != nullptr || a.batch != 1) return false;
  if (g.taps_h != 3 || g.taps_w != 3 || g.stride != 1 || a.K != 9 * g.Cg || g.Cg % ck != 0 ||
      g.c_split % ck != 0 || a.N % 32 != 0)
    return false;
  if (g.s[0].h16 || g.s[1].h16 || a.e.shuffle_co || a.e.d[0].h16 || a.e.d[1].h16 || a.e.yref_h16) return false;
  if (a.e.d[0].oy || a.e.d[0].ox || a.e.d[0].H != g.Hg || a.e.d[0].W != g.Wg) return false;
  if (a.e.n_split < a.N && (a.e.d[1].oy || a.e.d[1].ox || a.e.d[1].H != g.Hg || a.e.d[1].W != g.Wg)) return false;
  for (int k = 0; k < 2; ++k)
    if ((long long)g.nimg * g.s[k].H * g.s[k].W * g.s[k].C * 4 >= (1ll << 32)) return false;
  const long long T = (long long)g.nimg * ((g.Hg + 3) / 4) * ((g.Wg + 3) / 4);
  if ((T + 31) / 32 * (a.N / 32) > 0x7fffffffLL) return false;
  return a.wino_ws != nullptr && (size_t)36 * a.N * g.Cg * 4 <= a.wino_ws_bytes;
}

hipError_t launch_wino_fused(const IgemmArgs& a, hipStream_t s) {
  if (!wino_fused_applies(a)) return hipErrorInvalidValue;
  const Gather& g = a.a;
  const int Th = (g.Hg + 3) / 4, Tw = (g.Wg + 3) / 4;
  const long long T = (long long)g.nimg * Th * Tw;
  float* V = reinterpret_cast<float*>(a.wino_ws);
  const long long nw = (long long)a.N * g.Cg;
  const int NB = a.N / 32;
  const long long G = (T + 31) / 32 * NB;
  hipLaunchKernelGGL(k_wino4f_w<16>, dim3((unsigned)((nw + 255) / 256)), dim3(256), 0, s, a.b, a.N, g.Cg, V);
  static const int abl = ablation_env("UNET_WF_ABL");
  switch (abl) {
    case 1: hipLaunchKernelGGL(k_wino4f<1>, dim3((unsigned)G), dim3(512), 0, s, g, (const float*)V, a.N, T, Th, Tw, NB, a.e); break;
    case 2: hipLaunchKernelGGL(k_wino4f<2>, dim3((unsigned)G), dim3(512), 0, s, g, (const float*)V, a.N, T, Th, Tw, NB, a.e); break;
    case 4: hipLaunchKernelGGL(k_wino4f<4>, dim3((unsigned)G), dim3(512), 0, s, g, (const float*)V, a.N, T, Th, Tw, NB, a.e); break;
    case 6: hipLaunchKernelGGL(k_wino4f<6>, dim3((unsigned)G), dim3(512), 0, s, g, (const float*)V, a.N, T, Th, Tw, NB, a.e); break;
    default: hipLaunchKernelGGL(k_wino4f<0>, dim3((unsigned)G), dim3(512), 0, s, g, (const float*)V, a.N, T, Th, Tw, NB, a.e);
  }
  return hipGetLastError();
}

__device__ __forceinline__ int wf8_slot(int row, int q) { return (q ^ ((row >> 2) & 3)) << 1; }

__global__ void k_wino4f_w8(const float* __restrict__ b, int N, int Cg, float* __restrict__ v) {
  const long long i = blockIdx.x * (long long)blockDim.x + threadIdx.x;
  if (i >= (long long)N * Cg) return;
  const int n = (int)(i / Cg), c = (int)(i - (long long)n * Cg);
  float tg[6][3];
#pragma unroll
  for (int k = 0; k < 3; ++k) {
    float col[3] = {b[((size_t)n * 9 + 0 + k) * Cg + c], b[((size_t)n * 9 + 3 + k) * Cg + c],
                    b[((size_t)n * 9 + 6 + k) * Cg + c]};
    float r[6];
    g6(col, r);
#pragma unroll
    for (int a = 0; a < 6; ++a) tg[a][k] = r[a];
  }
  const size_t base = (size_t)(c >> 3) * 36 * N;
  const int pos = wf8_slot(n, c & 3) + ((c >> 2) & 1);
#pragma unroll
  for (int a = 0; a < 6; ++a) {
    float r[6];
    g6(tg[a], r);
#pragma unroll
    for (int bb = 0; bb < 6; ++bb) v[(base + (size_t)(a * 6 + bb) * N + n) * 8 + pos] = r[bb];
  }
}

__device__ __forceinline__ float wf_epi(float v, float yv, float sc, float sh, float mu, float is, bool bwd_mask,
                                        bool relu, float& s1, float& s2) {
  v = (bwd_mask && !(fmaf(yv, sc, sh) > 0.f)) ? 0.f : v;
  s1 += v;
  s2 += v * (bwd_mask ? (yv - mu) * is : v);
  return relu ? fmaxf(v, 0.f) : v;
}

__device__ __forceinline__ void wf64_output(const floatx4 (&acc)[36], const Gather& g, const Epilogue& e, int N,
                                            long long T, int Th, int Tw, long long t0, int n0, int th, int cb,
                                            int mi, int mq, int lane, int wave, float* lds) {
  const long long tt = t0 + 16 * th + mi;
  const int col0 = n0 + 16 * cb + 4 * mq;
  const bool second = col0 >= e.n_split;
  float* dptr = second ? e.d[1].ptr : e.d[0].ptr;
  const int dC = second ? e.d[1].C : e.d[0].C;
  const int dcol = second ? col0 - e.n_split : col0;
  const bool bwd_mask = e.yref != nullptr && !second;
  float s1[4] = {0.f, 0.f, 0.f, 0.f}, s2[4] = {0.f, 0.f, 0.f, 0.f};
  if (tt < T) {
    const int ox = (int)(tt % Tw);
    const long long rq = tt / Tw;
    const int oy = (int)(rq % Th), on = (int)(rq / Th);
    float o[4][4][4];
#pragma unroll
    for (int r = 0; r < 4; ++r) {
      float w[4][6];
#pragma unroll
      for (int xx = 0; xx < 6; ++xx) {
        float m[6];
#pragma unroll
        for (int yy = 0; yy < 6; ++yy) m[yy] = acc[yy * 6 + xx][r];
        float t4[4];
        at4(m, t4);
#pragma unroll
        for (int a = 0; a < 4; ++a) w[a][xx] = t4[a];
      }
#pragma unroll
      for (int a = 0; a < 4; ++a) at4(w[a], o[r][a]);
    }
    const float4 bias = e.bias ? ld4(e.bias + col0) : make_float4(0.f, 0.f, 0.f, 0.f);
    float4 bsc = make_float4(0.f, 0.f, 0.f, 0.f), bsh = bsc, bmu = bsc, bis = bsc;
    if (bwd_mask) { bsc = ld4(e.bn_scale + col0); bsh = ld4(e.bn_shift + col0); bmu = ld4(e.bn_mean + col0); bis = ld4(e.bn_invstd + col0); }
    const float bsv[4] = {bias.x, bias.y, bias.z, bias.w};
    const float scv[4] = {bsc.x, bsc.y, bsc.z, bsc.w}, shv[4] = {bsh.x, bsh.y, bsh.z, bsh.w};
    const float muv[4] = {bmu.x, bmu.y, bmu.z, bmu.w}, isv[4] = {bis.x, bis.y, bis.z, bis.w};
    const unsigned long long ybase = uniform_u64(e.yref);
    const unsigned ylds = (unsigned)(size_t)(lds_u8_t*)lds + (unsigned)wave * 8192u;
#pragma unroll
    for (int h = 0; h < 2; ++h) {
      if (bwd_mask) {
#pragma unroll
        for (int q = 0; q < 8; ++q) {
          const int y = min(4 * oy + 2 * h + (q >> 2), g.Hg - 1), x = min(4 * ox + (q & 3), g.Wg - 1);
          dma_sv((((unsigned)(on * g.Hg + y) * g.Wg + x) * dC + dcol) * 4u, ybase, ylds + q * 1024u);
        }
      }
      __builtin_amdgcn_s_waitcnt(0x0F70);
#pragma unroll
      for (int q = 0; q < 8; ++q) {
        const int a = 2 * h + (q >> 2), bb = q & 3;
        const int y = 4 * oy + a, x = 4 * ox + bb;
        if (y >= g.Hg || x >= g.Wg) continue;
        const float4 yq = bwd_mask ? *reinterpret_cast<const float4*>(lds + wave * 2048 + q * 256 + lane * 4)
                                   : make_float4(0.f, 0.f, 0.f, 0.f);
        const float yv[4] = {yq.x, yq.y, yq.z, yq.w};
        float v[4];
#pragma unroll
        for (int r = 0; r < 4; ++r) v[r] = wf_epi(o[r][a][bb] + bsv[r], yv[r], scv[r], shv[r], muv[r], isv[r],
                                                   bwd_mask, e.relu, s1[r], s2[r]);
        st4(dptr + ((size_t)(on * g.Hg + y) * g.Wg + x) * dC + dcol, make_float4(v[0], v[1], v[2], v[3]));
      }
    }
  }
  const bool want = e.stats || e.yref || e.colsum1;
  if (!want) return;
#pragma unroll
  for (int r = 0; r < 4; ++r)
#pragma unroll
    for (int o2 = 1; o2 < 16; o2 <<= 1) {
      s1[r] += __shfl_xor(s1[r], o2);
      s2[r] += __shfl_xor(s2[r], o2);
    }
  if (mi == 0) {
    const int grp = blockIdx.x % kStatGroups;
    const int nsplit = e.n_split < N ? e.n_split : N;
#pragma unroll
    for (int r = 0; r < 4; ++r) {
      const int col = col0 + r;
      if (col < nsplit) {
        double* st = e.yref ? e.bstats : e.stats;
        if (st) {
          atomicAdd(st + ((size_t)grp * nsplit + col) * 2 + 0, (double)s1[r]);
          atomicAdd(st + ((size_t)grp * nsplit + col) * 2 + 1, (double)s2[r]);
        }
      } else if (e.colsum1) {
        atomicAdd(e.colsum1 + (size_t)grp * (N - nsplit) + (col - nsplit), (double)s1[r]);
      }
    }
  }
}

template <int ABL>
__global__ __launch_bounds__(512, 1) void k_wino4f64(Gather g, const float* __restrict__ V, int N, long long T,
                                                     int Th, int Tw, int NB, Epilogue e) {
  constexpr int PU = 32 * 8 + 8;
  constexpr int PV = 64 * 8;
  __shared__ __attribute__((aligned(16))) float lds[36 * PU + 36 * PV];
  float* Us = lds;
  float* Vs = lds + 36 * PU;
  const int tid = threadIdx.x, lane = tid & 63, wave = tid >> 6;
  long long bid = blockIdx.x;
  const long long G = gridDim.x;
  if ((G & 7) == 0) bid = (bid & 7) * (G >> 3) + (bid >> 3);
  const int nb = (int)(bid % NB);
  const long long t0 = (bid / NB) * 32;
  const int n0 = nb * 64;

  const int hf = (lane >> 4) & 1;
  const int pt = wave * 32 + (lane & 15) + ((lane >> 5) << 4);
  const int lt = pt >> 3, lc = pt & 7;
  const long long t = t0 + lt;
  int img = 0, ty = 0, tx = 0;
  if (t < T) {
    tx = (int)(t % Tw);
    const long long r = t / Tw;
    ty = (int)(r % Th);
    img = (int)(r / Th);
  }
  const int vrows = t < T ? min(6, g.Hg + 2 - 4 * ty) : 0;
  const int vcols = t < T ? min(6, g.Wg + 2 - 4 * tx) : 0;
  const bool wfull = __all(vrows == 6 && vcols == 6);
  float* const ubase = Us + (3 * hf) * 6 * PU + lt * 8 + wf8_slot(lt, lc & 3) + (lc >> 2);
  float raw[18];
  float sc = 1.f, sh = 0.f;
  const int nk = g.Cg >> 3;
  const unsigned long long vbase = uniform_u64(V);
  const unsigned vlds = (unsigned)(size_t)(lds_u8_t*)lds + (unsigned)(36 * PU * 4);
  auto load = [&](int kc) {
    const bool second = kc * 8 >= g.c_split;
    const float* sp = second ? g.s[1].ptr : g.s[0].ptr;
    const int sH = second ? g.s[1].H : g.s[0].H, sW = second ? g.s[1].W : g.s[0].W;
    const int sC = second ? g.s[1].C : g.s[0].C;
    const int soy = second ? g.s[1].oy : g.s[0].oy, sox = second ? g.s[1].ox : g.s[0].ox;
    const int cl = kc * 8 - (second ? g.c_split : 0) + lc;
    const float* scp = second ? g.s[1].scale : g.s[0].scale;
    if (scp) {
      sc = scp[cl];
      sh = (second ? g.s[1].shift : g.s[0].shift)[cl];
    }
    const char* sb = reinterpret_cast<const char*>(sp);
    const unsigned o0 = ((unsigned)((img * sH + 4 * ty + soy) * sW + 4 * tx + sox) * sC + cl) * 4u;
    const unsigned rs = (unsigned)sW * sC * 4u, cs = (unsigned)sC * 4u;
    if (wfull) {
      const unsigned oh = o0 + 3u * hf * cs;
#pragma unroll
      for (int yy = 0; yy < 6; ++yy)
#pragma unroll
        for (int xx = 0; xx < 3; ++xx)
          raw[yy * 3 + xx] = *reinterpret_cast<const float*>(sb + (oh + (yy * rs + xx * cs)));
    } else {
      const unsigned lr = (unsigned)max(vrows - 1, 0), lcn = (unsigned)max(vcols - 1, 0);
#pragma unroll
      for (int yy = 0; yy < 6; ++yy)
#pragma unroll
        for (int xx = 0; xx < 3; ++xx)
          raw[yy * 3 + xx] = *reinterpret_cast<const float*>(
              sb + (o0 + (min((unsigned)yy, lr) * rs + min((unsigned)(3 * hf + xx), lcn) * cs)));
    }
  };
  auto commit = [&](int kc) {
    const bool second = kc * 8 >= g.c_split;
    const float* scp = second ? g.s[1].scale : g.s[0].scale;
    __builtin_amdgcn_s_waitcnt(0x0F70);
#pragma unroll
    for (int j = 0; j < 9; ++j) {
      const int pc = wave + 8 * j;
      dma_sv((unsigned)((((size_t)kc * 36 + (pc >> 1)) * N + n0) * 32) + (unsigned)((pc & 1) * 1024 + lane * 16),
             vbase, vlds + (unsigned)((pc >> 1) * PV * 4 + (pc & 1) * 1024));
    }
    if constexpr (ABL & 1) {
#pragma unroll
      for (int a = 0; a < 3; ++a)
#pragma unroll
        for (int bb = 0; bb < 6; ++bb) ubase[(a * 6 + bb) * PU] = raw[a * 6 + bb];
    } else {
    if (scp) {
#pragma unroll
      for (int q = 0; q < 18; ++q) raw[q] = fmaxf(fmaf(raw[q], sc, sh), 0.f);
    }
    if (!wfull) {
#pragma unroll
      for (int q = 0; q < 18; ++q) raw[q] = (q / 3 < vrows && 3 * hf + q % 3 < vcols) ? raw[q] : 0.f;
    }
#pragma unroll
    for (int xx = 0; xx < 3; ++xx) {
      float d[6];
#pragma unroll
      for (int yy = 0; yy < 6; ++yy) d[yy] = raw[yy * 3 + xx];
      float rr[6];
      bt6(d, rr);
#pragma unroll
      for (int a = 0; a < 6; ++a) raw[a * 3 + xx] = rr[a];
    }
#pragma unroll
    for (int k = 0; k < 9; ++k) {
      const auto sw = __builtin_amdgcn_permlane16_swap(__float_as_uint(raw[k]), __float_as_uint(raw[9 + k]),
                                                       false, false);
      raw[k] = __uint_as_float(sw[0]);
      raw[9 + k] = __uint_as_float(sw[1]);
    }
#pragma unroll
    for (int a = 0; a < 3; ++a) {
      const float d[6] = {raw[a * 3 + 0], raw[a * 3 + 1], raw[a * 3 + 2],
                          raw[9 + a * 3 + 0], raw[9 + a * 3 + 1], raw[9 + a * 3 + 2]};
      float rr[6];
      bt6(d, rr);
#pragma unroll
      for (int bb = 0; bb < 6; ++bb) ubase[(a * 6 + bb) * PU] = rr[bb];
    }
    }
    if constexpr (!(ABL & 16)) vm_wait<0>();
  };

  const int th = wave & 1, cb = wave >> 1;
  const int mi = lane & 15, mq = lane >> 4;
  const int aoff = (16 * th + mi) * 8 + wf8_slot(16 * th + mi, mq);
  const int boff = (16 * cb + mi) * 8 + wf8_slot(mi, mq);
  floatx4 acc[36];
#pragma unroll
  for (int p = 0; p < 36; ++p) acc[p] = (floatx4){0.f, 0.f, 0.f, 0.f};
  load(0);
  for (int kc = 0; kc < nk; ++kc) {
    commit(kc);
    __syncthreads();
    if (!(ABL & 4) && kc + 1 < nk) load(kc + 1);
    if constexpr (!(ABL & 2))
#pragma unroll
    for (int p = 0; p < 36; ++p) {
      const float2 a = *reinterpret_cast<const float2*>(Us + p * PU + aoff);
      const float2 b = *reinterpret_cast<const float2*>(Vs + p * PV + boff);
      acc[p] = __builtin_amdgcn_mfma_f32_16x16x4f32(b.x, a.x, acc[p], 0, 0, 0);
      acc[p] = __builtin_amdgcn_mfma_f32_16x16x4f32(b.y, a.y, acc[p], 0, 0, 0);
    }
    __syncthreads();
  }
  if constexpr (ABL & 8) {
    float sum = 0.f;
#pragma unroll
    for (int p = 0; p < 36; ++p) sum += acc[p][0] + acc[p][1] + acc[p][2] + acc[p][3];
    if (sum == 1.2345f) e.d[0].ptr[tid] = sum;
    return;
  }

  wf64_output(acc, g, e, N, T, Th, Tw, t0, n0, th, cb, mi, mq, lane, wave, lds);
}

bool wino_fused64_applies(const IgemmArgs& a) {
  return wino_fused_applies(a) && a.N % 64 == 0 &&
         (a.e.yref == nullptr || (long long)a.a.nimg * a.a.Hg * a.a.Wg * a.e.d[0].C * 4 < (1ll << 32));
}

hipError_t launch_wino_fused64(const IgemmArgs& a, hipStream_t s) {
  if (!wino_fused64_applies(a)) return hipErrorInvalidValue;
  const Gather& g = a.a;
  const int Th = (g.Hg + 3) / 4, Tw = (g.Wg + 3) / 4;
  const long long T = (long long)g.nimg * Th * Tw;
  float* V = reinterpret_cast<float*>(a.wino_ws);
  const long long nw = (long long)a.N * g.Cg;
  const int NB = a.N / 64;
  const long long G = (T + 31) / 32 * NB;
  hipLaunchKernelGGL(k_wino4f_w8, dim3((unsigned)((nw + 255) / 256)), dim3(256), 0, s, a.b, a.N, g.Cg, V);
  static const int abl = ablation_env("UNET_WF64_ABL");
  switch (abl) {
#define WF64(A) \
  case A: hipLaunchKernelGGL(k_wino4f64<A>, dim3((unsigned)G), dim3(512), 0, s, g, (const float*)V, a.N, T, Th, Tw, NB, a.e); break;
    WF64(1) WF64(2) WF64(4) WF64(8) WF64(6) WF64(3) WF64(16) WF64(20) WF64(18) WF64(7) WF64(15)
#undef WF64
    default: hipLaunchKernelGGL(k_wino4f64<0>, dim3((unsigned)G), dim3(512), 0, s, g, (const float*)V, a.N, T, Th, Tw, NB, a.e);
  }
  return hipGetLastError();
}



constexpr int kWf64pMaxCg = 1024;

__global__ __launch_bounds__(512, 1) void k_wino4f64p(Gather g, const float* __restrict__ V, int N, long long T,
                                                      int Th, int Tw, int NB, Epilogue e) {
  constexpr int PU = 32 * 8 + 8, PV = 64 * 8;
  constexpr int PA = 16;
  constexpr int U_F = 36 * PU, VA_F = PA * PV, VB_F = (36 - PA) * PV, RAW_F = 8 * 18 * 64;
  __shared__ __attribute__((aligned(16))) float lds[U_F + VA_F + VB_F + RAW_F + 2 * kWf64pMaxCg];
  float* Us = lds;
  float* VAs = lds + U_F;
  float* VBs = VAs + VA_F;
  float* raws = VBs + VB_F;
  float* ss = raws + RAW_F;
  const int tid = threadIdx.x, lane = tid & 63, wave = tid >> 6;
  long long bid = blockIdx.x;
  const long long G = gridDim.x;
  if ((G & 7) == 0) bid = (bid & 7) * (G >> 3) + (bid >> 3);
  const int nb = (int)(bid % NB);
  const long long t0 = (bid / NB) * 32;
  const int n0 = nb * 64;
  const int Cg = g.Cg, nk = Cg >> 3;

  const int hf = (lane >> 4) & 1;
  const int pt = wave * 32 + (lane & 15) + ((lane >> 5) << 4);
  const int lt = pt >> 3, lc = pt & 7;
  const long long t = t0 + lt;
  int img = 0, ty = 0, tx = 0;
  if (t < T) {
    tx = (int)(t % Tw);
    const long long r = t / Tw;
    ty = (int)(r % Th);
    img = (int)(r / Th);
  }
  const int vrows = t < T ? min(6, g.Hg + 2 - 4 * ty) : 0;
  const int vcols = t < T ? min(6, g.Wg + 2 - 4 * tx) : 0;
  const bool wfull = __all(vrows == 6 && vcols == 6);
  float* const ubase = Us + (3 * hf) * 6 * PU + lt * 8 + wf8_slot(lt, lc & 3) + (lc >> 2);

  const bool tf0 = g.s[0].scale != nullptr, tf1 = g.c_split < Cg && g.s[1].scale != nullptr;
  if (tf0 || tf1) {
    for (int c = tid; c < Cg; c += 512) {
      const bool sec = c >= g.c_split;
      const float* scp = sec ? g.s[1].scale : g.s[0].scale;
      const float* shp = sec ? g.s[1].shift : g.s[0].shift;
      const int cl = sec ? c - g.c_split : c;
      ss[c] = scp ? scp[cl] : 1.f;
      ss[kWf64pMaxCg + c] = scp ? shp[cl] : 0.f;
    }
  }

  const unsigned raw_lds = (unsigned)(size_t)(lds_u8_t*)raws + (unsigned)wave * (18u * 256u);
  auto issue_raw = [&](int kc) {
    const bool second = kc * 8 >= g.c_split;
    const unsigned long long sb = uniform_u64(second ? g.s[1].ptr : g.s[0].ptr);
    const int sH = second ? g.s[1].H : g.s[0].H, sW = second ? g.s[1].W : g.s[0].W;
    const int sC = second ? g.s[1].C : g.s[0].C;
    const int soy = second ? g.s[1].oy : g.s[0].oy, sox = second ? g.s[1].ox : g.s[0].ox;
    const int cl = kc * 8 - (second ? g.c_split : 0) + lc;
    const unsigned o0 = ((unsigned)((img * sH + 4 * ty + soy) * sW + 4 * tx + sox) * sC + cl) * 4u;
    const unsigned rs = (unsigned)sW * sC * 4u, cs = (unsigned)sC * 4u;
    if (wfull) {
      const unsigned oh = o0 + 3u * hf * cs;
#pragma unroll
      for (int yy = 0; yy < 6; ++yy)
#pragma unroll
        for (int xx = 0; xx < 3; ++xx) dma4_sv(oh + (yy * rs + xx * cs), sb, raw_lds + (yy * 3 + xx) * 256u);
    } else {
      const unsigned lr = (unsigned)max(vrows - 1, 0), lcn = (unsigned)max(vcols - 1, 0);
#pragma unroll
      for (int yy = 0; yy < 6; ++yy)
#pragma unroll
        for (int xx = 0; xx < 3; ++xx)
          dma4_sv(o0 + (min((unsigned)yy, lr) * rs + min((unsigned)(3 * hf + xx), lcn) * cs), sb,
                  raw_lds + (yy * 3 + xx) * 256u);
    }
  };
  const unsigned long long vbase = uniform_u64(V);
  const unsigned va_lds = (unsigned)(size_t)(lds_u8_t*)VAs, vb_lds = (unsigned)(size_t)(lds_u8_t*)VBs;
  auto issue_v = [&](int kc, int half) {
    const int np = half ? 5 : 4, p0 = half ? PA : 0;
    const unsigned dst = half ? vb_lds : va_lds;
#pragma unroll
    for (int j = 0; j < 5; ++j) {
      if (j < np) {
        const int pc = wave + 8 * j;
        dma_sv((unsigned)((((size_t)kc * 36 + p0 + (pc >> 1)) * N + n0) * 32) + (unsigned)((pc & 1) * 1024 + lane * 16),
               vbase, dst + (unsigned)((pc >> 1) * PV * 4 + (pc & 1) * 1024));
      }
    }
  };
  auto commit = [&](int kc) {
    vm_wait<9>();
    float raw[18];
#pragma unroll
    for (int q = 0; q < 18; ++q) raw[q] = raws[wave * (18 * 64) + q * 64 + lane];
    lgkm_wait0();
    issue_raw(kc + 1 < nk ? kc + 1 : kc);
    const bool second = kc * 8 >= g.c_split;
    const bool tf = second ? tf1 : tf0;
    if (tf) {
      const float sc = ss[kc * 8 + lc], sh = ss[kWf64pMaxCg + kc * 8 + lc];
#pragma unroll
      for (int q = 0; q < 18; ++q) raw[q] = fmaxf(fmaf(raw[q], sc, sh), 0.f);
    }
    if (!wfull) {
#pragma unroll
      for (int q = 0; q < 18; ++q) raw[q] = (q / 3 < vrows && 3 * hf + q % 3 < vcols) ? raw[q] : 0.f;
    }
#pragma unroll
    for (int xx = 0; xx < 3; ++xx) {
      float d[6];
#pragma unroll
      for (int yy = 0; yy < 6; ++yy) d[yy] = raw[yy * 3 + xx];
      float rr[6];
      bt6(d, rr);
#pragma unroll
      for (int a = 0; a < 6; ++a) raw[a * 3 + xx] = rr[a];
    }
#pragma unroll
    for (int k = 0; k < 9; ++k) {
      const auto sw = __builtin_amdgcn_permlane16_swap(__float_as_uint(raw[k]), __float_as_uint(raw[9 + k]),
                                                       false, false);
      raw[k] = __uint_as_float(sw[0]);
      raw[9 + k] = __uint_as_float(sw[1]);
    }
#pragma unroll
    for (int a = 0; a < 3; ++a) {
      const float d[6] = {raw[a * 3 + 0], raw[a * 3 + 1], raw[a * 3 + 2],
                          raw[9 + a * 3 + 0], raw[9 + a * 3 + 1], raw[9 + a * 3 + 2]};
      float rr[6];
      bt6(d, rr);
#pragma unroll
      for (int bb = 0; bb < 6; ++bb) ubase[(a * 6 + bb) * PU] = rr[bb];
    }
  };

  const int th = wave & 1, cb = wave >> 1;
  const int mi = lane & 15, mq = lane >> 4;
  const int aoff = (16 * th + mi) * 8 + wf8_slot(16 * th + mi, mq);
  const int boff = (16 * cb + mi) * 8 + wf8_slot(mi, mq);
  floatx4 acc[36];
#pragma unroll
  for (int p = 0; p < 36; ++p) acc[p] = (floatx4){0.f, 0.f, 0.f, 0.f};

  __syncthreads();
  issue_raw(0);
  issue_v(0, 0);
  issue_v(0, 1);
  for (int kc = 0; kc < nk; ++kc) {
    const int kn = kc + 1 < nk ? kc + 1 : kc;
    commit(kc);
    vm_wait<23>();
    lgkm_wait0();
    raw_barrier();
#pragma unroll
    for (int p = 0; p < PA; ++p) {
      const float2 a = *reinterpret_cast<const float2*>(Us + p * PU + aoff);
      const float2 b = *reinterpret_cast<const float2*>(VAs + p * PV + boff);
      acc[p] = __builtin_amdgcn_mfma_f32_16x16x4f32(b.x, a.x, acc[p], 0, 0, 0);
      acc[p] = __builtin_amdgcn_mfma_f32_16x16x4f32(b.y, a.y, acc[p], 0, 0, 0);
    }
    vm_wait<18>();
    lgkm_wait0();
    raw_barrier();
    issue_v(kn, 0);
#pragma unroll
    for (int p = PA; p < 36; ++p) {
      const float2 a = *reinterpret_cast<const float2*>(Us + p * PU + aoff);
      const float2 b = *reinterpret_cast<const float2*>(VBs + (p - PA) * PV + boff);
      acc[p] = __builtin_amdgcn_mfma_f32_16x16x4f32(b.x, a.x, acc[p], 0, 0, 0);
      acc[p] = __builtin_amdgcn_mfma_f32_16x16x4f32(b.y, a.y, acc[p], 0, 0, 0);
    }
    lgkm_wait0();
    raw_barrier();
    issue_v(kn, 1);
  }
  vm_wait<0>();
  __syncthreads();
  wf64_output(acc, g, e, N, T, Th, Tw, t0, n0, th, cb, mi, mq, lane, wave, lds);
}

bool wino_fused64p_applies(const IgemmArgs& a) { return wino_fused64_applies(a) && a.a.Cg <= kWf64pMaxCg; }

hipError_t launch_wino_fused64p(const IgemmArgs& a, hipStream_t s) {
  if (!wino_fused64p_applies(a)) return hipErrorInvalidValue;
  const Gather& g = a.a;
  const int Th = (g.Hg + 3) / 4, Tw = (g.Wg + 3) / 4;
  const long long T = (long long)g.nimg * Th * Tw;
  float* V = reinterpret_cast<float*>(a.wino_ws);
  const long long nw = (long long)a.N * g.Cg;
  const int NB = a.N / 64;
  const long long G = (T + 31) / 32 * NB;
  hipLaunchKernelGGL(k_wino4f_w8, dim3((unsigned)((nw + 255) / 256)), dim3(256), 0, s, a.b, a.N, g.Cg, V);
  hipLaunchKernelGGL(k_wino4f64p, dim3((unsigned)G), dim3(512), 0, s, g, (const float*)V, a.N, T, Th, Tw, NB, a.e);
  return hipGetLastError();
}

__global__ void k_wino2f_w8(const float* __restrict__ b, int N, int Cg, float* __restrict__ v) {
  const long long i = blockIdx.x * (long long)blockDim.x + threadIdx.x;
  if (i >= (long long)N * Cg) return;
  const int n = (int)(i / Cg), c = (int)(i - (long long)n * Cg);
  float g[3][3];
#pragma unroll
  for (int t = 0; t < 9; ++t) g[t / 3][t % 3] = b[((size_t)n * 9 + t) * Cg + c];
  float tg[4][3];
#pragma unroll
  for (int k = 0; k < 3; ++k) {
    tg[0][k] = g[0][k];
    tg[1][k] = 0.5f * (g[0][k] + g[1][k] + g[2][k]);
    tg[2][k] = 0.5f * (g[0][k] - g[1][k] + g[2][k]);
    tg[3][k] = g[2][k];
  }
  const size_t base = (size_t)(c >> 3) * 16 * N;
  const int pos = wf8_slot(n, c & 3) + ((c >> 2) & 1);
#pragma unroll
  for (int r = 0; r < 4; ++r) {
    const float w4[4] = {tg[r][0], 0.5f * (tg[r][0] + tg[r][1] + tg[r][2]), 0.5f * (tg[r][0] - tg[r][1] + tg[r][2]),
                         tg[r][2]};
#pragma unroll
    for (int q = 0; q < 4; ++q) v[(base + (size_t)(r * 4 + q) * N + n) * 8 + pos] = w4[q];
  }
}

template <int NC>
__global__ __launch_bounds__(512, NC == 32 ? 2 : 1) void k_wino2f64(Gather g, const float* __restrict__ V, int N,
                                                                   long long T, int Th, int Tw, int NB, Epilogue e) {
  constexpr int TT = 64;
  constexpr int PU = TT * 8;
  constexpr int PV = NC * 8;
  constexpr int NJ = NC / 32;
  __shared__ __attribute__((aligned(16))) float lds[16 * PU + 16 * PV];
  float* Us = lds;
  float* Vs = lds + 16 * PU;
  const int tid = threadIdx.x, lane = tid & 63, wave = tid >> 6;
  long long bid = blockIdx.x;
  const long long G = gridDim.x;
  if ((G & 7) == 0) bid = (bid & 7) * (G >> 3) + (bid >> 3);
  const int nb = (int)(bid % NB);
  const long long t0 = (bid / NB) * TT;
  const int n0 = nb * NC;

  const int lt = tid >> 3, lc = tid & 7;
  const long long t = t0 + lt;
  int img = 0, ty = 0, tx = 0;
  if (t < T) {
    tx = (int)(t % Tw);
    const long long r = t / Tw;
    ty = (int)(r % Th);
    img = (int)(r / Th);
  }
  const int vrows = t < T ? min(4, g.Hg + 2 - 2 * ty) : 0;
  const int vcols = t < T ? min(4, g.Wg + 2 - 2 * tx) : 0;
  const bool wfull = __all(vrows == 4 && vcols == 4);
  float* const ubase = Us + lt * 8 + wf8_slot(lt, lc & 3) + (lc >> 2);
  float raw[16];
  float sc = 1.f, sh = 0.f;
  const int nk = g.Cg >> 3;
  const unsigned long long vbase = uniform_u64(V);
  const unsigned vlds = (unsigned)(size_t)(lds_u8_t*)lds + (unsigned)(16 * PU * 4);
  auto load = [&](int kc) {
    const bool second = kc * 8 >= g.c_split;
    const float* sp = second ? g.s[1].ptr : g.s[0].ptr;
    const int sH = second ? g.s[1].H : g.s[0].H, sW = second ? g.s[1].W : g.s[0].W;
    const int sC = second ? g.s[1].C : g.s[0].C;
    const int soy = second ? g.s[1].oy : g.s[0].oy, sox = second ? g.s[1].ox : g.s[0].ox;
    const int cl = kc * 8 - (second ? g.c_split : 0) + lc;
    const float* scp = second ? g.s[1].scale : g.s[0].scale;
    if (scp) {
      sc = scp[cl];
      sh = (second ? g.s[1].shift : g.s[0].shift)[cl];
    }
    const char* sb = reinterpret_cast<const char*>(sp);
    const unsigned o0 = ((unsigned)((img * sH + 2 * ty + soy) * sW + 2 * tx + sox) * sC + cl) * 4u;
    const unsigned rs = (unsigned)sW * sC * 4u, cs = (unsigned)sC * 4u;
    if (wfull) {
#pragma unroll
      for (int yy = 0; yy < 4; ++yy)
#pragma unroll
        for (int xx = 0; xx < 4; ++xx)
          raw[yy * 4 + xx] = *reinterpret_cast<const float*>(sb + (o0 + (yy * rs + xx * cs)));
    } else {
      const unsigned lr = (unsigned)max(vrows - 1, 0), lcn = (unsigned)max(vcols - 1, 0);
#pragma unroll
      for (int yy = 0; yy < 4; ++yy)
#pragma unroll
        for (int xx = 0; xx < 4; ++xx)
          raw[yy * 4 + xx] = *reinterpret_cast<const float*>(
              sb + (o0 + (min((unsigned)yy, lr) * rs + min((unsigned)xx, lcn) * cs)));
    }
  };
  auto commit = [&](int kc) {
    const bool second = kc * 8 >= g.c_split;
    const float* scp = second ? g.s[1].scale : g.s[0].scale;
    __builtin_amdgcn_s_waitcnt(0x0F70);
#pragma unroll
    for (int j = 0; j < 2 * NJ; ++j) {
      const int pc = wave + 8 * j;
      dma_sv((unsigned)((((size_t)kc * 16 + pc / NJ) * N + n0) * 32) + (unsigned)((pc % NJ) * 1024 + lane * 16),
             vbase, vlds + (unsigned)((pc / NJ) * PV * 4 + (pc % NJ) * 1024));
    }
    if (scp) {
#pragma unroll
      for (int q = 0; q < 16; ++q) raw[q] = fmaxf(fmaf(raw[q], sc, sh), 0.f);
    }
    if (!wfull) {
#pragma unroll
      for (int q = 0; q < 16; ++q) raw[q] = (q / 4 < vrows && q % 4 < vcols) ? raw[q] : 0.f;
    }
    float ev[4][4];
#pragma unroll
    for (int xx = 0; xx < 4; ++xx) {
      ev[0][xx] = raw[0 * 4 + xx] - raw[2 * 4 + xx];
      ev[1][xx] = raw[1 * 4 + xx] + raw[2 * 4 + xx];
      ev[2][xx] = raw[2 * 4 + xx] - raw[1 * 4 + xx];
      ev[3][xx] = raw[1 * 4 + xx] - raw[3 * 4 + xx];
    }
#pragma unroll
    for (int a = 0; a < 4; ++a) {
      ubase[(a * 4 + 0) * PU] = ev[a][0] - ev[a][2];
      ubase[(a * 4 + 1) * PU] = ev[a][1] + ev[a][2];
      ubase[(a * 4 + 2) * PU] = ev[a][2] - ev[a][1];
      ubase[(a * 4 + 3) * PU] = ev[a][1] - ev[a][3];
    }
    vm_wait<0>();
  };

  const int th = wave & 3, ch = wave >> 2;
  const int mi = lane & 15, mq = lane >> 4;
  const int aoff = (16 * th + mi) * 8 + wf8_slot(16 * th + mi, mq);
  const int boff = (16 * NJ * ch + mi) * 8 + wf8_slot(mi, mq);
  floatx4 acc[16][NJ];
#pragma unroll
  for (int p = 0; p < 16; ++p)
#pragma unroll
    for (int j = 0; j < NJ; ++j) acc[p][j] = (floatx4){0.f, 0.f, 0.f, 0.f};
  load(0);
  for (int kc = 0; kc < nk; ++kc) {
    commit(kc);
    __syncthreads();
    if (kc + 1 < nk) load(kc + 1);
#pragma unroll
    for (int p = 0; p < 16; ++p) {
      const float2 a = *reinterpret_cast<const float2*>(Us + p * PU + aoff);
#pragma unroll
      for (int j = 0; j < NJ; ++j) {
        const float2 b = *reinterpret_cast<const float2*>(Vs + p * PV + boff + 16 * j * 8);
        acc[p][j] = __builtin_amdgcn_mfma_f32_16x16x4f32(b.x, a.x, acc[p][j], 0, 0, 0);
        acc[p][j] = __builtin_amdgcn_mfma_f32_16x16x4f32(b.y, a.y, acc[p][j], 0, 0, 0);
      }
    }
    __syncthreads();
  }

  const long long tt = t0 + 16 * th + mi;
  const bool want = e.stats || e.yref || e.colsum1;
  const int nsplit = e.n_split < N ? e.n_split : N;
  const int grp = blockIdx.x % kStatGroups;
#pragma unroll
  for (int j = 0; j < NJ; ++j) {
    const int col0 = n0 + 16 * NJ * ch + 16 * j + 4 * mq;
    const bool second = col0 >= e.n_split;
    float* dptr = second ? e.d[1].ptr : e.d[0].ptr;
    const int dC = second ? e.d[1].C : e.d[0].C;
    const int dcol = second ? col0 - e.n_split : col0;
    const bool bwd_mask = e.yref != nullptr && !second;
    const float4 bias = e.bias ? ld4(e.bias + col0) : make_float4(0.f, 0.f, 0.f, 0.f);
    float4 bsc = make_float4(0.f, 0.f, 0.f, 0.f), bsh = bsc, bmu = bsc, bis = bsc;
    if (bwd_mask) { bsc = ld4(e.bn_scale + col0); bsh = ld4(e.bn_shift + col0); bmu = ld4(e.bn_mean + col0); bis = ld4(e.bn_invstd + col0); }
    float s1[4] = {0.f, 0.f, 0.f, 0.f}, s2[4] = {0.f, 0.f, 0.f, 0.f};
    if (tt < T) {
      const int ox = (int)(tt % Tw);
      const long long rq = tt / Tw;
      const int oy = (int)(rq % Th), on = (int)(rq / Th);
      float4 y4[4];
      if (bwd_mask) {
#pragma unroll
        for (int a = 0; a < 2; ++a)
#pragma unroll
          for (int bb = 0; bb < 2; ++bb) {
            const int y = min(2 * oy + a, g.Hg - 1), x = min(2 * ox + bb, g.Wg - 1);
            y4[a * 2 + bb] = ld4(e.yref + ((size_t)(on * g.Hg + y) * g.Wg + x) * dC + dcol);
          }
      }
      __builtin_amdgcn_s_waitcnt(0x0F70);
      float o[4][2][2];
#pragma unroll
      for (int r = 0; r < 4; ++r) {
        float w[2][4];
#pragma unroll
        for (int xx = 0; xx < 4; ++xx) {
          const float m0 = acc[0 * 4 + xx][j][r], m1 = acc[1 * 4 + xx][j][r];
          const float m2 = acc[2 * 4 + xx][j][r], m3 = acc[3 * 4 + xx][j][r];
          w[0][xx] = m0 + m1 + m2;
          w[1][xx] = m1 - m2 - m3;
        }
#pragma unroll
        for (int a = 0; a < 2; ++a) {
          o[r][a][0] = w[a][0] + w[a][1] + w[a][2];
          o[r][a][1] = w[a][1] - w[a][2] - w[a][3];
        }
      }
      const float bsv[4] = {bias.x, bias.y, bias.z, bias.w};
      const float scv[4] = {bsc.x, bsc.y, bsc.z, bsc.w}, shv[4] = {bsh.x, bsh.y, bsh.z, bsh.w};
      const float muv[4] = {bmu.x, bmu.y, bmu.z, bmu.w}, isv[4] = {bis.x, bis.y, bis.z, bis.w};
#pragma unroll
      for (int a = 0; a < 2; ++a) {
        const int y = 2 * oy + a;
        if (y >= g.Hg) continue;
#pragma unroll
        for (int bb = 0; bb < 2; ++bb) {
          const int x = 2 * ox + bb;
          if (x >= g.Wg) continue;
          const size_t idx = ((size_t)(on * g.Hg + y) * g.Wg + x) * dC + dcol;
          const float4 yq = bwd_mask ? y4[a * 2 + bb] : make_float4(0.f, 0.f, 0.f, 0.f);
          const float yv[4] = {yq.x, yq.y, yq.z, yq.w};
          float v[4];
#pragma unroll
          for (int r = 0; r < 4; ++r) v[r] = wf_epi(o[r][a][bb] + bsv[r], yv[r], scv[r], shv[r], muv[r], isv[r],
                                                     bwd_mask, e.relu, s1[r], s2[r]);
          st4(dptr + idx, make_float4(v[0], v[1], v[2], v[3]));
        }
      }
    }
    if (!want) continue;
#pragma unroll
    for (int r = 0; r < 4; ++r)
#pragma unroll
      for (int o2 = 1; o2 < 16; o2 <<= 1) {
        s1[r] += __shfl_xor(s1[r], o2);
        s2[r] += __shfl_xor(s2[r], o2);
      }
    if (mi == 0) {
#pragma unroll
      for (int r = 0; r < 4; ++r) {
        const int col = col0 + r;
        if (col < nsplit) {
          double* st = e.yref ? e.bstats : e.stats;
          if (st) {
            atomicAdd(st + ((size_t)grp * nsplit + col) * 2 + 0, (double)s1[r]);
            atomicAdd(st + ((size_t)grp * nsplit + col) * 2 + 1, (double)s2[r]);
          }
        } else if (e.colsum1) {
          atomicAdd(e.colsum1 + (size_t)grp * (N - nsplit) + (col - nsplit), (double)s1[r]);
        }
      }
    }
  }
}

bool wino_fused2_applies(const IgemmArgs& a, int nc) {
  const Gather& g = a.a;
  if (a.b == nullptr || a.bh != nullptr || a.batch != 1) return false;
  if (g.taps_h != 3 || g.taps_w != 3 || g.stride != 1 || a.K != 9 * g.Cg || g.Cg % 8 != 0 || g.c_split % 8 != 0 ||
      a.N % nc != 0 || (a.e.n_split < a.N && a.e.n_split % 16 != 0))
    return false;
  if (g.s[0].h16 || g.s[1].h16 || a.e.shuffle_co || a.e.d[0].h16 || a.e.d[1].h16 || a.e.yref_h16) return false;
  if (a.e.d[0].oy || a.e.d[0].ox || a.e.d[0].H != g.Hg || a.e.d[0].W != g.Wg) return false;
  if (a.e.n_split < a.N && (a.e.d[1].oy || a.e.d[1].ox || a.e.d[1].H != g.Hg || a.e.d[1].W != g.Wg)) return false;
  for (int k = 0; k < 2; ++k)
    if ((long long)g.nimg * g.s[k].H * g.s[k].W * g.s[k].C * 4 >= (1ll << 32)) return false;
  const long long T = (long long)g.nimg * ((g.Hg + 1) / 2) * ((g.Wg + 1) / 2);
  if ((T + 63) / 64 * (a.N / nc) > 0x7fffffffLL) return false;
  return a.wino_ws != nullptr && (size_t)16 * a.N * g.Cg * 4 <= a.wino_ws_bytes;
}

hipError_t launch_wino_fused2(const IgemmArgs& a, hipStream_t s, int nc) {
  if ((nc != 64 && nc != 32) || !wino_fused2_applies(a, nc)) return hipErrorInvalidValue;
  const Gather& g = a.a;
  const int Th = (g.Hg + 1) / 2, Tw = (g.Wg + 1) / 2;
  const long long T = (long long)g.nimg * Th * Tw;
  float* V = reinterpret_cast<float*>(a.wino_ws);
  const long long nw = (long long)a.N * g.Cg;
  const int NB = a.N / nc;
  const long long G = (T + 63) / 64 * NB;
  hipLaunchKernelGGL(k_wino2f_w8, dim3((unsigned)((nw + 255) / 256)), dim3(256), 0, s, a.b, a.N, g.Cg, V);
  if (nc == 64)
    hipLaunchKernelGGL(k_wino2f64<64>, dim3((unsigned)G), dim3(512), 0, s, g, (const float*)V, a.N, T, Th, Tw, NB, a.e);
  else
    hipLaunchKernelGGL(k_wino2f64<32>, dim3((unsigned)G), dim3(512), 0, s, g, (const float*)V, a.N, T, Th, Tw, NB, a.e);
  return hipGetLastError();
}

__device__ __forceinline__ void a6(const float (&y)[4], float (&r)[6]) {
  r[0] = y[0];
  r[1] = y[0] + y[1] + y[2] + y[3];
  r[2] = y[0] - y[1] + y[2] - y[3];
  r[3] = y[0] + 2.f * y[1] + 4.f * y[2] + 8.f * y[3];
  r[4] = y[0] - 0.5f * y[1] + 0.25f * y[2] - 0.125f * y[3];
  r[5] = y[3];
}
__device__ __forceinline__ void gt3(const float (&m)[6], float (&r)[3]) {
  r[0] = m[0] + (m[2] - m[1]) * (1.f / 3.f) + (m[3] - 16.f * m[4]) * (1.f / 15.f);
  r[1] = -(m[1] + m[2]) * (1.f / 3.f) + (2.f * m[3] + 8.f * m[4]) * (1.f / 15.f);
  r[2] = (m[2] - m[1]) * (1.f / 3.f) + (4.f * m[3] - 4.f * m[4]) * (1.f / 15.f) + m[5];
}

__global__ __launch_bounds__(256) void k_wino4_dy(Src dy, int Hg, int Wg, int Th, int Tw, long long T, int Co,
                                                  float* __restrict__ vd) {
  const long long i = blockIdx.x * (long long)blockDim.x + threadIdx.x;
  if (i >= T * Co) return;
  const long long t = i / Co;
  const int c = (int)(i - t * Co);
  const int tx = (int)(t % Tw);
  const long long r = t / Tw;
  const int ty = (int)(r % Th), n = (int)(r / Th);
  float e[6][4];
#pragma unroll
  for (int xx = 0; xx < 4; ++xx) {
    float d[4];
#pragma unroll
    for (int yy = 0; yy < 4; ++yy) {
      const int y = 4 * ty + yy, x = 4 * tx + xx;
      const bool in = y < Hg && x < Wg;
      const float v = dy.ptr[((size_t)(n * dy.H + (in ? y : 0) + dy.oy) * dy.W + (in ? x : 0) + dy.ox) * dy.C + c];
      d[yy] = in ? v : 0.f;
    }
    float rr[6];
    a6(d, rr);
#pragma unroll
    for (int a = 0; a < 6; ++a) e[a][xx] = rr[a];
  }
  const size_t plane = (size_t)T * Co, o = (size_t)t * Co + c;
#pragma unroll
  for (int a = 0; a < 6; ++a) {
    float rr[6];
    a6(e[a], rr);
#pragma unroll
    for (int bb = 0; bb < 6; ++bb) vd[(a * 6 + bb) * plane + o] = rr[bb];
  }
}

__device__ __forceinline__ void wout_store(const float (&dwv)[9], long long i, long long n, int Ci,
                                           float* __restrict__ out, int oihw) {
  float dw[9];
#pragma unroll
  for (int t = 0; t < 9; ++t) {
    dw[t] = dwv[t];
    asm volatile("" : "+v"(dw[t]));
  }
  if (!oihw) {
    if (i >= n) return;
    const int co = (int)(i / Ci), ci = (int)(i - (long long)co * Ci);
#pragma unroll
    for (int t = 0; t < 9; ++t) out[((size_t)co * 9 + t) * Ci + ci] = dw[t];
    return;
  }
  __shared__ float st[256 * 9];
#pragma unroll
  for (int t = 0; t < 9; ++t) st[threadIdx.x * 9 + t] = dw[t];
  __syncthreads();
  const long long base = blockIdx.x * (long long)(256 * 9), lim = n * 9;
#pragma unroll
  for (int k = 0; k < 9; ++k) {
    const int e = k * 256 + threadIdx.x;
    if (base + e < lim) out[base + e] = st[e];
  }
}

__global__ __launch_bounds__(256) void k_wino4_wout(const float* __restrict__ mw, int Co, int Ci,
                                                    float* __restrict__ out, int oihw) {
  const long long n = (long long)Co * Ci;
  const long long i = blockIdx.x * (long long)blockDim.x + threadIdx.x, il = i < n ? i : n - 1;
  const size_t plane = (size_t)Co * Ci;
  float w[3][6];
#pragma unroll
  for (int bb = 0; bb < 6; ++bb) {
    float m[6];
#pragma unroll
    for (int a = 0; a < 6; ++a) m[a] = mw[(a * 6 + bb) * plane + il];
    float r[3];
    gt3(m, r);
#pragma unroll
    for (int k = 0; k < 3; ++k) w[k][bb] = r[k];
  }
  float dw[9];
#pragma unroll
  for (int k = 0; k < 3; ++k) {
    float r[3];
    gt3(w[k], r);
#pragma unroll
    for (int kx = 0; kx < 3; ++kx) dw[k * 3 + kx] = r[kx];
  }
  wout_store(dw, i, n, Ci, out, oihw);
}

__device__ __forceinline__ void a8(const float (&y)[6], float (&r)[8]) {
  constexpr float A[8][6] = {{1, 0, 0, 0, 0, 0},
                             {1, 1, 1, 1, 1, 1},
                             {1, -1, 1, -1, 1, -1},
                             {1, 2, 4, 8, 16, 32},
                             {1, -2, 4, -8, 16, -32},
                             {1, 0.5f, 0.25f, 0.125f, 0.0625f, 0.03125f},
                             {1, -0.5f, 0.25f, -0.125f, 0.0625f, -0.03125f},
                             {0, 0, 0, 0, 0, 1}};
  mat_apply(A, y, r);
}
__device__ __forceinline__ void gt8(const float (&m)[8], float (&r)[3]) {
  constexpr float GT[3][8] = {{1, -2.f / 9, -2.f / 9, 1.f / 90, 1.f / 90, 32.f / 45, 32.f / 45, 0},
                              {0, -2.f / 9, 2.f / 9, 1.f / 45, -1.f / 45, 16.f / 45, -16.f / 45, 0},
                              {0, -2.f / 9, -2.f / 9, 2.f / 45, 2.f / 45, 8.f / 45, 8.f / 45, 1}};
  mat_apply(GT, m, r);
}

template <int V>
__global__ __launch_bounds__(256) void k_wino6_dy(Src dy, int Hg, int Wg, int Th, int Tw, long long T, int Co,
                                                  float* __restrict__ vd) {
  typedef float vec __attribute__((ext_vector_type(V)));
  const int CV = Co / V;
  const long long i = blockIdx.x * (long long)blockDim.x + threadIdx.x;
  if (i >= T * CV) return;
  const long long t = i / CV;
  const int c = (int)(i - t * CV) * V;
  const int tx = (int)(t % Tw);
  const long long r = t / Tw;
  const int ty = (int)(r % Th), n = (int)(r / Th);
  const int vr = min(6, Hg - 6 * ty), vc = min(6, Wg - 6 * tx);
  const char* base = reinterpret_cast<const char*>(dy.ptr) +
                     (((size_t)(n * dy.H + 6 * ty + dy.oy) * dy.W + 6 * tx + dy.ox) * dy.C + c) * 4;
  const unsigned rs = (unsigned)dy.W * dy.C * 4u, cs = (unsigned)dy.C * 4u;
  float e[V][8][6];
#pragma unroll
  for (int xx = 0; xx < 6; ++xx) {
    float d[V][6];
#pragma unroll
    for (int yy = 0; yy < 6; ++yy) {
      const bool in = yy < vr && xx < vc;
      const vec v = *reinterpret_cast<const vec*>(base + (in ? yy * rs + xx * cs : 0u));
#pragma unroll
      for (int k = 0; k < V; ++k) d[k][yy] = in ? v[k] : 0.f;
    }
#pragma unroll
    for (int k = 0; k < V; ++k) {
// ... 300 lines not shown
```

### unet-segmentation_amd/unet_amd/_lib.py

```python
from __future__ import annotations

import ctypes
import os

_HERE = os.path.dirname(os.path.abspath(__file__))
LIB_PATH = os.environ.get("UNET_HIP_LIB", os.path.join(_HERE, "libunet_hip.so"))

_vp = ctypes.c_void_p
_i = ctypes.c_int
_f = ctypes.c_float
_sz = ctypes.c_size_t

SIGNATURES = {
    "unet_version": (ctypes.c_char_p, []),
    "unet_last_error": (ctypes.c_char_p, []),
    "unet_plan_create": (_vp, [_i, _i, _i, _i, _i]),
    "unet_plan_create_ex": (_vp, [_i, _i, _i, _i, _i, _i]),
    "unet_plan_precision": (_i, [_vp]),
    "unet_plan_destroy": (None, [_vp]),
    "unet_plan_out_hw": (_i, [_vp, ctypes.POINTER(_i), ctypes.POINTER(_i)]),
    "unet_plan_workspace_bytes": (_sz, [_vp]),
    "unet_plan_forward_workspace_bytes": (_sz, [_vp]),
    "unet_plan_num_params": (_i, [_vp]),
    "unet_plan_num_grads": (_i, [_vp]),
    "unet_plan_forward": (_i, [_vp, _vp, _vp, _vp, _vp, _i, _vp]),
    "unet_plan_num_segments": (_i, [_vp]),
    "unet_plan_segment_grads": (_i, [_vp, _i, ctypes.POINTER(_i), ctypes.POINTER(_i)]),
    "unet_plan_backward": (_i, [_vp, _vp, _vp, _vp, _vp, _vp, _i, _i, _vp]),
    "unet_plan_backward_ex": (_i, [_vp, _vp, _vp, _vp, _vp, _vp, _i, _i, _i, _vp]),
    "unet_plan_wait_segment": (_i, [_vp, _i, _vp]),
    "unet_plan_input_grad_scratch_bytes": (_sz, [_vp]),
    "unet_plan_input_grad": (_i, [_vp, _vp, _vp, _vp, _vp, _vp]),
    "unet_plan_join": (_i, [_vp, _vp]),
    "unet_plan_set_timing": (_i, [_vp, _i]),
    "unet_plan_timing": (_i, [_vp, _vp, _vp, _vp, _vp]),
    "unet_plan_timing_mfma_flops": (_i, [_vp, _vp]),
    "unet_plan_timing_sites": (_sz, [_vp, ctypes.c_char_p, _sz]),
    "unet_wce_fwd_bwd": (_i, [_vp, _vp, _vp, _i, _i, _i, _i, _vp, _vp, _vp, _vp, _f, _vp, _vp]),
    "unet_scale_by_device_scalar": (_i, [_vp, _sz, _vp, _vp]),
    "unet_scale_by_device_scalar_out": (_i, [_vp, _vp, _sz, _vp, _vp]),
    "unet_sgd_momentum": (_i, [_vp, _vp, _vp, _sz, _f, _f, _f, _i, _vp]),
    "unet_iou_counts": (_i, [_vp, _vp, _sz, _vp, _vp]),
    "unet_mask_from_logits": (_i, [_vp, _vp, _i, _i, _i, _vp]),
    "unet_tile_gather": (_i, [_vp, _i, _i, _i, _i, _i, _i, _i, _i, _i, _i, _i, _vp, _vp]),
    "unet_tile_scatter": (_i, [_vp, _i, _i, _i, _i, _i, _i, _i, _i, _vp, _vp, _vp]),
    "unet_instance_masks_ws_bytes": (_sz, [_i, _i, _i]),
    "unet_instance_masks": (_i, [_vp, _i, _i, _i, _i, _vp, _vp, _vp]),
    "unet_rand_index_ws_bytes": (_sz, [_i, _i]),
    "unet_rand_index": (_i, [_vp, _vp, _i, _i, _vp, _vp, _vp]),
    "unet_weight_map_ws_bytes": (_sz, [_i]),
    "unet_weight_map": (_i, [_vp, _i, _i, _i, ctypes.c_double, ctypes.c_double, _vp, _vp, _vp, _vp]),
    "unet_weight_map_border_ws_bytes": (_sz, [_i, _i, _i]),
    "unet_weight_map_border": (_i, [_vp, _i, _i, _i, ctypes.c_double, ctypes.c_double, _vp, _vp, _vp, _vp, _vp, _vp]),
    "unet_elastic_ws_bytes": (_sz, [_i, _i, _i]),
    "unet_elastic_deform": (_i, [_vp, _vp, _i, _i, _i, _vp, ctypes.c_double, ctypes.c_double, _vp, _vp, _vp, _vp,
                                 _vp]),
    "unet_elastic_deform_ex": (_i, [_vp, _vp, _i, _i, _i, _vp, ctypes.c_double, ctypes.c_double, _vp, _vp, _vp, _vp,
                                    _vp, _vp]),
    "unet_conv3x3_fwd": (_i, [_vp, _i, _i, _i, _i, _vp, _vp, _i, _vp, _vp, _vp, _vp, _vp]),
    "unet_conv3x3_dgrad": (_i, [_vp, _i, _i, _i, _i, _vp, _i, _vp, _vp, _vp]),
    "unet_conv3x3_wgrad": (_i, [_vp, _vp, _i, _i, _i, _i, _i, _vp, _vp, _vp, _vp]),
    "unet_conv_ws_bytes": (_sz, [_i, _i, _i, _i, _i]),
    "unet_convT2_fwd": (_i, [_vp, _i, _i, _i, _i, _vp, _vp, _i, _vp, _vp, _vp]),
    "unet_convT2_bwd": (_i, [_vp, _vp, _i, _i, _i, _i, _vp, _i, _vp, _vp, _vp, _vp, _vp]),
    "unet_maxpool2_fwd": (_i, [_vp, _i, _i, _i, _i, _vp, _vp, _vp]),
    "unet_maxpool2_bwd": (_i, [_vp, _vp, _i, _i, _i, _i, _vp, _vp]),
    "unet_bn_train_fwd": (_i, [_vp, _i, _i, _i, _i, _vp, _vp, _vp, _vp, _vp, _vp, _vp, _vp, _vp]),
    "unet_bn_train_bwd": (_i, [_vp, _vp, _i, _i, _i, _i, _vp, _vp, _vp, _vp, _vp, _vp, _vp, _vp]),
    "unet_bn_ws_bytes": (_sz, [_i]),
    "unet_bn_relu_ws_bytes": (_sz, [_i, _i, _i, _i]),
    "unet_bn_relu_fwd": (_i, [_vp, _i, _i, _i, _i, _vp, _vp, _vp, _vp, _vp, _f, _f, _i, _i, _vp, _vp, _vp, _vp,
                              _vp]),
    "unet_bn_relu_bwd": (_i, [_vp, _vp, _vp, _i, _i, _i, _i, _vp, _vp, _vp, _i, _i, _vp, _vp, _vp, _vp, _vp]),
    "unet_conv_first_ws_bytes": (_sz, [_i, _i, _i, _i]),
    "unet_conv_first_fwd": (_i, [_vp, _i, _i, _i, _i, _vp, _vp, _vp, _vp]),
    "unet_conv_first_bwd": (_i, [_vp, _vp, _i, _i, _i, _i, _vp, _vp, _vp, _vp, _vp, _vp]),
    "unet_conv1x1_ws_bytes": (_sz, [_i]),
    "unet_conv1x1_fwd": (_i, [_vp, _i, _i, _i, _i, _vp, _vp, _i, _vp, _vp]),
    "unet_conv1x1_bwd": (_i, [_vp, _vp, _i, _i, _i, _i, _vp, _i, _vp, _vp, _vp, _vp, _vp]),
    "unet_peak_probe": (_i, [_i, _i, ctypes.POINTER(ctypes.c_double), _vp]),
    "unet_tracker_create": (_vp, [_i, _i, ctypes.c_double, ctypes.c_double, _i]),
    "unet_tracker_destroy": (None, [_vp]),
    "unet_tracker_ws_bytes": (_sz, [_i, _i]),
    "unet_tracker_add_frame": (_i, [_vp, _vp, _i, _vp, _vp]),
    "unet_tracker_step_host": (_i, [_vp, _i, _i, _vp, _vp, _vp]),
    "unet_tracker_num_tracks": (_i, [_vp]),
    "unet_tracker_tracks": (_i, [_vp, _vp, _i]),
    "unet_linear_sum_assignment": (_i, [ctypes.c_longlong, ctypes.c_longlong, _vp, _vp, _vp]),
    "unet_ctc_create": (_vp, []),
    "unet_ctc_destroy": (None, [_vp]),
    "unet_ctc_ws_bytes": (_sz, [_i, _i, _i]),
    "unet_ctc_add_frames": (_i, [_vp, _i, _vp, _vp, _vp, _i, _i, _i, _vp, _vp]),
    "unet_ctc_add_frame_host": (_i, [_vp, _i, _i, _i, _vp, _vp, _i, _vp, _vp, _i, _vp]),
    "unet_ctc_set_tracks": (_i, [_vp, _i, _vp, _i]),
    "unet_ctc_measures": (_i, [_vp, _vp, _vp]),
    "unet_ctc_log": (ctypes.c_longlong, [_vp, ctypes.c_char_p, _sz]),
    "unet_ctc_num_frames": (_i, [_vp, _i]),
    "unet_ctc_frame_sizes": (_i, [_vp, _i, _i, _vp]),
    "unet_ctc_frame_tables": (_i, [_vp, _i, _i, _vp, _vp, _vp, _vp, _vp]),
    "unet_ctc_stats": (_i, [_vp, _vp]),
    "unet_warping_error_ws_bytes": (_sz, [_i, _i, _i]),
    "unet_warping_error": (_i, [_vp, _vp, _i, _i, _i, _i, _i, _i, _i, _vp, _vp, _vp, _vp]),
    "unet_simple_point_table": (None, [_vp]),
    "unet_set_tuning": (_i, [ctypes.c_char_p, _i]),
    "unet_tuning_report": (_sz, [ctypes.c_char_p, _sz]),
    "unet_tuning_reset": (_i, []),
    "unet_slab_fallbacks": (ctypes.c_longlong, [_i]),
    "unet_nondeterministic_sites": (ctypes.c_longlong, [_i]),
    "unet_fused_bnb_sites": (ctypes.c_longlong, [_i]),
    "unet_wgrad_oihw_sites": (ctypes.c_longlong, [_i]),
    "unet_igemm_plane_launches": (ctypes.c_longlong, [_i]),
    "unet_tuning_save": (_i, [ctypes.c_char_p]),
    "unet_tuning_load": (_i, [ctypes.c_char_p]),
}

_lib = None
_load_error = None


def load():
    global _lib, _load_error
    if _lib is not None:
        return _lib
    if _load_error is not None:
        raise RuntimeError(_load_error)
    try:
        lib = ctypes.CDLL(LIB_PATH, mode=ctypes.RTLD_GLOBAL)
    except OSError as e:
        _load_error = (f"libunet_hip.so could not be loaded from {LIB_PATH} ({e}); "
                       "build it with `python -c 'import __graft_entry__ as g; g.build()'`")
        raise RuntimeError(_load_error) from e
    for name, (res, args) in SIGNATURES.items():
        fn = getattr(lib, name)
        fn.restype = res
        fn.argtypes = args
    _lib = lib
    return lib


def last_error() -> str:
    msg = load().unet_last_error()
    return msg.decode() if msg else ""


def check(rc: int, what: str) -> None:
    if rc != 0:
        raise RuntimeError(f"{what} failed (rc={rc}): {last_error()}")


def ptr(t) -> int:
    return None if t is None else t.data_ptr()


def ptr_array(tensors):
    arr = (ctypes.c_void_p * len(tensors))()
    for i, t in enumerate(tensors):
        arr[i] = t.data_ptr()
    return arr


def stream_of(device=None):
    import torch
    return ctypes.c_void_p(torch.cuda.current_stream(device).cuda_stream)


_HASHED = ["igemm.hip", "igemm_bf16.hip", "conv3_dma.hip", "conv3_ring.hip", "winograd.hip", "elementwise.hip", "elastic.hip",
           "tiling.hip", "weightmap.hip", "postproc.hip", "track.hip", "ops.hip", "plan.hip", "wgrad3_ring.hip",
           "conv3_ring_pt.hip", "peak.hip", "gemm_ring.hip", "wgradT_ring.hip", "conv3_flat.hip", "conv3_c64.hip", "gemm_ring_p1.hip",
           "gemm_ring_p2.hip", "wgrad_plane.hip", "igemm_plane.hip", "ctc.hip", "warp.hip", "unet_internal.h", "gemm_common.h", "ring_common.h", "conv3_ring_kernel.h",
           os.path.join("..", "..", "include", "unet_hip.h")]


def source_hash() -> str:
    import hashlib
    h = hashlib.sha256()
    csrc = os.path.join(_HERE, "..", "csrc")
    for f in _HASHED:
        with open(os.path.join(csrc, f), "rb") as fh:
            h.update(fh.read())
    return h.hexdigest()[:16]


def build_identity() -> dict:
    v = load().unet_version().decode()
    built = v.rsplit(" src ", 1)[-1].split()[0] if " src " in v else "unknown"
    tree = source_hash()
    return {"version": v, "lib_src": built, "tree_src": tree, "src_match": built == tree,
            "ablation_build": v.endswith(" ablations")}


def slab_fallbacks(reset: bool = False) -> int:
    return int(load().unet_slab_fallbacks(1 if reset else 0))


def tuning_report() -> str:
    lib = load()
    n = lib.unet_tuning_report(None, 0)
    buf = ctypes.create_string_buffer(n)
    lib.unet_tuning_report(buf, n)
    return buf.value.decode()
```

Baseline: 318.6 images/s.

## Add persistent work-stealing Winograd fused conv kernels with per-XCD tile queues

Turns the fused Winograd forward/dgrad kernels (F(4,3) and F(2,3), 64-channel tiles) into optional persistent variants. Each workgroup takes a contiguous stretch of tiles per XCD, steals leftover tiles from other XCDs through atomic counters, and prefetches the next tile's operands while it writes the current epilogue. The aim is to cut tail imbalance and launch/ramp overhead and to overlap loads with output stores. It also specializes the kernels on a forward/backward template flag, uses unsigned 32-bit tile indexing, and relaxes channel checks to allow multiples of 8 when a fused Winograd tile is forced. The cost is atomic contention, counter initialization folded into the weight-transform kernel, and extra workspace.

```diff
diff --git a/include/unet_hip.h b/include/unet_hip.h
--- a/include/unet_hip.h
+++ b/include/unet_hip.h
@@ -148,6 +148,7 @@
 long long unet_fused_bnb_sites(int reset);
 long long unet_wgrad_oihw_sites(int reset);
 long long unet_igemm_plane_launches(int reset);
+long long unet_wino_persist_launches(int reset);
 int unet_tuning_save(const char* path);
 int unet_tuning_load(const char* path);
 
diff --git a/unet-segmentation_amd/csrc/igemm.hip b/unet-segmentation_amd/csrc/igemm.hip
--- a/unet-segmentation_amd/csrc/igemm.hip
+++ b/unet-segmentation_amd/csrc/igemm.hip
@@ -1139,8 +1139,8 @@
   return t ? t->go(a, s) : hipErrorInvalidValue;
 }
 
-static bool igemm_args_ok(const IgemmArgs& a) {
-  return a.M > 0 && a.N > 0 && a.K > 0 && (a.K % 16) == 0 && (a.a.Cg % 16) == 0 && (a.a.c_split % 16) == 0;
+static bool igemm_args_ok(const IgemmArgs& a, int q = 16) {
+  return a.M > 0 && a.N > 0 && a.K > 0 && (a.K % q) == 0 && (a.a.Cg % q) == 0 && (a.a.c_split % q) == 0;
 }
 
 GemmChoice resolve_forced_igemm(const IgemmArgs& a, int knob) {
@@ -1173,8 +1173,13 @@
   return -1;
 }
 
+static int igemm_forced_quantum(const IgemmArgs& a) {
+  const IgemmTile* t = igemm_tile(resolve_forced_igemm(a, g_tune_igemm).tile);
+  return t && t->family == IgemmFamily::WinoFused && t->wino_m == 2 ? 8 : 16;
+}
+
 hipError_t launch_igemm(const IgemmArgs& a0, hipStream_t s) {
-  if (!igemm_args_ok(a0)) return hipErrorInvalidValue;
+  if (!igemm_args_ok(a0, igemm_forced_quantum(a0))) return hipErrorInvalidValue;
   IgemmArgs a = a0;
   a.ksplit = 1;
   return go_tile(a, s, igemm_heuristic_tile(a));
diff --git a/unet-segmentation_amd/csrc/ops.hip b/unet-segmentation_amd/csrc/ops.hip
--- a/unet-segmentation_amd/csrc/ops.hip
+++ b/unet-segmentation_amd/csrc/ops.hip
@@ -59,7 +59,7 @@
 
 extern "C" {
 
-static size_t op_wino_bytes(int ci, int co) { return al256(sizeof(float) * 36 * (size_t)ci * co); }
+static size_t op_wino_bytes(int ci, int co) { return al256(sizeof(float) * 36 * (size_t)ci * co) + 256; }
 static size_t op_wgrad_wino_bytes(int n, int h, int w, int ci, int co);
 static size_t op_wgrad_extra_bytes(int n, int h, int w, int ci, int co);
 static void op_set_wino(IgemmArgs& a, void* ws, int n, int h, int w, int ci, int co) {
@@ -97,7 +97,8 @@
 
 int unet_conv3x3_fwd(const float* x, int n, int h, int w, int ci, const float* wt, const float* bias, int co,
                      const float* xs, const float* xb, float* y, void* ws, unet_stream_t st) {
-  if (ci % 16 || co % 64 || h < 3 || w < 3) return -EINVAL;
+  if (ci % 8 || co % 64 || h < 3 || w < 3) return -EINVAL;
+  if (ci % 16 && (g_op_prec != UNET_PREC_FP32 || g_tune_igemm <= 0)) return -EINVAL;
   hipStream_t s = reinterpret_cast<hipStream_t>(st);
   float* wf = reinterpret_cast<float*>(ws);
   OPCK(launch_pack_conv(wt, co, ci, 3, 3, wf, nullptr, s));
@@ -131,6 +132,7 @@
   a.e.bias = bias;
   a.e.d[0] = Dst{y, h - 2, w - 2, co, 0, 0};
   op_set_wino(a, ws, n, h, w, ci, co);
+  if (ci % 16 && resolve_forced_igemm(a, g_tune_igemm).tile < 0) return -EINVAL;
   OPCK(op_b_to_bf16(a, 9 * (size_t)ci * co, reinterpret_cast<char*>(ws) + al256(sizeof(float) * 9 * (size_t)ci * co),
                     s));
   OPCK(launch_igemm(a, s));
@@ -139,7 +141,8 @@
 
 int unet_conv3x3_dgrad(const float* dy, int n, int h, int w, int ci, const float* wt, int co, float* dx, void* ws,
                        unet_stream_t st) {
-  if (ci % 64 || co % 16 || h < 3 || w < 3) return -EINVAL;
+  if (ci % 64 || co % 8 || h < 3 || w < 3) return -EINVAL;
+  if (co % 16 && (g_op_prec != UNET_PREC_FP32 || g_tune_igemm <= 0)) return -EINVAL;
   hipStream_t s = reinterpret_cast<hipStream_t>(st);
   char* p = reinterpret_cast<char*>(ws);
   const size_t wb = al256(sizeof(float) * 9 * (size_t)ci * co);
@@ -171,6 +174,7 @@
   a.K = 9 * co;
   a.e.d[0] = Dst{dx, h, w, ci, 0, 0};
   op_set_wino(a, ws, n, h, w, ci, co);
+  if (co % 16 && resolve_forced_igemm(a, g_tune_igemm).tile < 0) return -EINVAL;
   OPCK(op_b_to_bf16(a, 9 * (size_t)ci * co, wf, s));
   OPCK(launch_igemm(a, s));
   return 0;
@@ -558,6 +562,8 @@
   else if (k == "wgrad_plane") g_wgrad_plane = value;
   else if (k == "wgrad_oihw") g_wgrad_oihw = value;
   else if (k == "igemm_plane") g_igemm_plane = value;
+  else if (k == "wino_persist") g_wino_persist = value;
+  else if (k == "wino_persist_wgs") g_wino_persist_wgs = value;
   else if (k == "wino_point_tile") g_wino_point_tile = value;
   else if (k == "ctc_chunk_frames" || k == "ctc_dense_cells") {
     if (value < -1 || (value == 0 && k == "ctc_chunk_frames")) return -EINVAL;
diff --git a/unet-segmentation_amd/csrc/plan.hip b/unet-segmentation_amd/csrc/plan.hip
--- a/unet-segmentation_amd/csrc/plan.hip
+++ b/unet-segmentation_amd/csrc/plan.hip
@@ -1400,6 +1400,10 @@
 long long unet_wgrad_oihw_sites(int reset) {
   return reset ? unet::g_wgrad_oihw_sites.exchange(0) : unet::g_wgrad_oihw_sites.load();
 }
+long long unet_wino_persist_launches(int reset) {
+  return reset ? unet::g_wino_persist_launches.exchange(0) : unet::g_wino_persist_launches.load();
+}
+
 long long unet_igemm_plane_launches(int reset) {
   return reset ? unet::g_igemm_plane_launches.exchange(0) : unet::g_igemm_plane_launches.load();
 }
diff --git a/unet-segmentation_amd/csrc/unet_internal.h b/unet-segmentation_amd/csrc/unet_internal.h
--- a/unet-segmentation_amd/csrc/unet_internal.h
+++ b/unet-segmentation_amd/csrc/unet_internal.h
@@ -82,6 +82,9 @@
 extern int g_wgrad_oihw;
 extern int g_igemm_plane;
 extern std::atomic<long long> g_igemm_plane_launches;
+extern int g_wino_persist;
+extern int g_wino_persist_wgs;
+extern std::atomic<long long> g_wino_persist_launches;
 extern int g_wino_point_tile;
 extern std::atomic<long long> g_nondet_sites;
 
diff --git a/unet-segmentation_amd/csrc/winograd.hip b/unet-segmentation_amd/csrc/winograd.hip
--- a/unet-segmentation_amd/csrc/winograd.hip
+++ b/unet-segmentation_amd/csrc/winograd.hip
@@ -1,5 +1,6 @@
 #include <algorithm>
 #include <cstdlib>
+#include <type_traits>
 
 #include "gemm_common.h"
 #include "ring_common.h"
@@ -1054,8 +1055,51 @@
 
 __device__ __forceinline__ int wf8_slot(int row, int q) { return (q ^ ((row >> 2) & 3)) << 1; }
 
-__global__ void k_wino4f_w8(const float* __restrict__ b, int N, int Cg, float* __restrict__ v) {
+constexpr int kWinoPersistCtrs = 8;
+__device__ __forceinline__ unsigned wp_ctr_init(unsigned pgrid, int x) { return (pgrid + 7u - (unsigned)x) >> 3; }
+__device__ __forceinline__ void wp_stretch(unsigned G, int x, unsigned& lo, unsigned& hi) {
+  lo = (unsigned)(((unsigned long long)G * (unsigned)x) >> 3);
+  hi = (unsigned)(((unsigned long long)G * (unsigned)(x + 1)) >> 3);
+}
+__device__ __forceinline__ int wp_resolve(unsigned* ctr, unsigned G, int x, unsigned k) {
+  unsigned lo, hi;
+  wp_stretch(G, x, lo, hi);
+  if (k < hi - lo) return (int)(lo + k);
+  for (int i = 1; i < 8; ++i) {
+    const int s = (x + i) & 7;
+    wp_stretch(G, s, lo, hi);
+    if (hi == lo) continue;
+    k = atomicAdd(ctr + s, 1u);
+    if (k < hi - lo) return (int)(lo + k);
+  }
+  return -1;
+}
+__device__ __forceinline__ unsigned wp_block_of(unsigned G, unsigned gid) {
+  if (G & 7u) return gid;
+  const unsigned q = G >> 3;
+  return (gid % q) * 8u + gid / q;
+}
+struct WfPatch {
+  int img, ty, tx, vrows, vcols;
+};
+template <int MT, class TI>
+__device__ __forceinline__ WfPatch wf_patch(TI t, TI T, int Th, int Tw, int Hg, int Wg) {
+  WfPatch p{0, 0, 0, 0, 0};
+  if (t < T) {
+    p.tx = (int)(t % (TI)Tw);
+    const TI r = t / (TI)Tw;
+    p.ty = (int)(r % (TI)Th);
+    p.img = (int)(r / (TI)Th);
+    p.vrows = min(MT + 2, Hg + 2 - MT * p.ty);
+    p.vcols = min(MT + 2, Wg + 2 - MT * p.tx);
+  }
+  return p;
+}
+
+__global__ void k_wino4f_w8(const float* __restrict__ b, int N, int Cg, float* __restrict__ v, unsigned* ctr,
+                            unsigned pgrid) {
   const long long i = blockIdx.x * (long long)blockDim.x + threadIdx.x;
+  if (ctr && i < kWinoPersistCtrs) ctr[i] = wp_ctr_init(pgrid, (int)i);
   if (i >= (long long)N * Cg) return;
   const int n = (int)(i / Cg), c = (int)(i - (long long)n * Cg);
   float tg[6][3];
@@ -1087,21 +1131,22 @@
   return relu ? fmaxf(v, 0.f) : v;
 }
 
+template <bool FWD, class TI>
 __device__ __forceinline__ void wf64_output(const floatx4 (&acc)[36], const Gather& g, const Epilogue& e, int N,
-                                            long long T, int Th, int Tw, long long t0, int n0, int th, int cb,
-                                            int mi, int mq, int lane, int wave, float* lds) {
-  const long long tt = t0 + 16 * th + mi;
+                                            TI T, int Th, int Tw, TI t0, int n0, int th, int cb,
+                                            int mi, int mq, int lane, int wave, float* lds, int grp) {
+  const TI tt = t0 + (TI)(16 * th + mi);
   const int col0 = n0 + 16 * cb + 4 * mq;
   const bool second = col0 >= e.n_split;
   float* dptr = second ? e.d[1].ptr : e.d[0].ptr;
   const int dC = second ? e.d[1].C : e.d[0].C;
   const int dcol = second ? col0 - e.n_split : col0;
-  const bool bwd_mask = e.yref != nullptr && !second;
+  const bool bwd_mask = !FWD && e.yref != nullptr && !second;
   float s1[4] = {0.f, 0.f, 0.f, 0.f}, s2[4] = {0.f, 0.f, 0.f, 0.f};
   if (tt < T) {
-    const int ox = (int)(tt % Tw);
-    const long long rq = tt / Tw;
-    const int oy = (int)(rq % Th), on = (int)(rq / Th);
+    const int ox = (int)(tt % (TI)Tw);
+    const TI rq = tt / (TI)Tw;
+    const int oy = (int)(rq % (TI)Th), on = (int)(rq / (TI)Th);
     float o[4][4][4];
 #pragma unroll
     for (int r = 0; r < 4; ++r) {
@@ -1163,7 +1208,6 @@
       s2[r] += __shfl_xor(s2[r], o2);
     }
   if (mi == 0) {
-    const int grp = blockIdx.x % kStatGroups;
     const int nsplit = e.n_split < N ? e.n_split : N;
 #pragma unroll
     for (int r = 0; r < 4; ++r) {
@@ -1333,7 +1377,8 @@
     return;
   }
 
-  wf64_output(acc, g, e, N, T, Th, Tw, t0, n0, th, cb, mi, mq, lane, wave, lds);
+  wf64_output<false, long long>(acc, g, e, N, T, Th, Tw, t0, n0, th, cb, mi, mq, lane, wave, lds,
+                                (int)(blockIdx.x % kStatGroups));
 }
 
 bool wino_fused64_applies(const IgemmArgs& a) {
@@ -1350,7 +1395,8 @@
   const long long nw = (long long)a.N * g.Cg;
   const int NB = a.N / 64;
   const long long G = (T + 31) / 32 * NB;
-  hipLaunchKernelGGL(k_wino4f_w8, dim3((unsigned)((nw + 255) / 256)), dim3(256), 0, s, a.b, a.N, g.Cg, V);
+  hipLaunchKernelGGL(k_wino4f_w8, dim3((unsigned)((nw + 255) / 256)), dim3(256), 0, s, a.b, a.N, g.Cg, V,
+                     (unsigned*)nullptr, 0u);
   static const int abl = ablation_env("UNET_WF64_ABL");
   switch (abl) {
 #define WF64(A) \
@@ -1366,41 +1412,81 @@
 
 constexpr int kWf64pMaxCg = 1024;
 
+template <bool PERSIST, bool FWD>
 __global__ __launch_bounds__(512, 1) void k_wino4f64p(Gather g, const float* __restrict__ V, int N, long long T,
-                                                      int Th, int Tw, int NB, Epilogue e) {
+                                                      int Th, int Tw, int NB, Epilogue e, unsigned G,
+                                                      unsigned* __restrict__ ctr) {
   constexpr int PU = 32 * 8 + 8, PV = 64 * 8;
   constexpr int PA = 16;
   constexpr int U_F = 36 * PU, VA_F = PA * PV, VB_F = (36 - PA) * PV, RAW_F = 8 * 18 * 64;
   __shared__ __attribute__((aligned(16))) float lds[U_F + VA_F + VB_F + RAW_F + 2 * kWf64pMaxCg];
+  __shared__ int sclaim[3];
   float* Us = lds;
-  float* VAs = lds + U_F;
-  float* VBs = VAs + VA_F;
-  float* raws = VBs + VB_F;
+  float* VBs = lds + U_F;
+  float* VAs = VBs + VB_F;
+  float* raws = VAs + VA_F;
   float* ss = raws + RAW_F;
-  const int tid = threadIdx.x, lane = tid & 63, wave = tid >> 6;
-  long long bid = blockIdx.x;
-  const long long G = gridDim.x;
-  if ((G & 7) == 0) bid = (bid & 7) * (G >> 3) + (bid >> 3);
-  const int nb = (int)(bid % NB);
-  const long long t0 = (bid / NB) * 32;
-  const int n0 = nb * 64;
+  static_assert((U_F + VB_F) * 4 >= 8 * 8192, "mask operand staging");
+  const int tid = threadIdx.x;
+  using TI = typename std::conditional<PERSIST, unsigned, long long>::type;
   const int Cg = g.Cg, nk = Cg >> 3;
-
-  const int hf = (lane >> 4) & 1;
-  const int pt = wave * 32 + (lane & 15) + ((lane >> 5) << 4);
-  const int lt = pt >> 3, lc = pt & 7;
-  const long long t = t0 + lt;
-  int img = 0, ty = 0, tx = 0;
-  if (t < T) {
-    tx = (int)(t % Tw);
-    const long long r = t / Tw;
-    ty = (int)(r % Th);
-    img = (int)(r / Th);
-  }
-  const int vrows = t < T ? min(6, g.Hg + 2 - 4 * ty) : 0;
-  const int vcols = t < T ? min(6, g.Wg + 2 - 4 * tx) : 0;
-  const bool wfull = __all(vrows == 6 && vcols == 6);
-  float* const ubase = Us + (3 * hf) * 6 * PU + lt * 8 + wf8_slot(lt, lc & 3) + (lc >> 2);
+  int lane, wave, hf, lt, lc, th, cb, mi, mq, aoff, boff;
+  float* ubase;
+  unsigned raw_lds;
+  WfPatch pc;
+  bool wfc;
+
+  TI t0;
+  int n0, grp;
+  const int xcd = blockIdx.x & 7;
+  unsigned kfire = 0;
+  if constexpr (PERSIST) {
+    unsigned lo, hi;
+    wp_stretch(G, xcd, lo, hi);
+    const unsigned k0 = blockIdx.x >> 3;
+    int gid;
+    if (k0 < hi - lo) {
+      gid = (int)(lo + k0);
+    } else {
+      if (tid == 0) sclaim[0] = wp_resolve(ctr, G, xcd, k0);
+      __syncthreads();
+      gid = sclaim[0];
+      if (gid < 0) return;
+    }
+    gid = __builtin_amdgcn_readfirstlane(gid);
+    if (tid == 0) kfire = atomicAdd(ctr + xcd, 1u);
+    n0 = (int)((unsigned)gid % (unsigned)NB) * 64;
+    t0 = (unsigned)gid / (unsigned)NB * 32u;
+    grp = (int)(wp_block_of(G, (unsigned)gid) % kStatGroups);
+  } else {
+    long long bid = blockIdx.x;
+    const long long Gd = gridDim.x;
+    if ((Gd & 7) == 0) bid = (bid & 7) * (Gd >> 3) + (bid >> 3);
+    n0 = (int)(bid % NB) * 64;
+    t0 = (bid / NB) * 32;
+    grp = (int)(blockIdx.x % kStatGroups);
+  }
+
+  auto roles = [&]() {
+    int tv = tid;
+    if constexpr (PERSIST) asm volatile("" : "+v"(tv));
+    lane = tv & 63;
+    wave = tv >> 6;
+    hf = (lane >> 4) & 1;
+    const int pt = wave * 32 + (lane & 15) + ((lane >> 5) << 4);
+    lt = pt >> 3;
+    lc = pt & 7;
+    pc = wf_patch<4, TI>(t0 + (TI)lt, (TI)T, Th, Tw, g.Hg, g.Wg);
+    wfc = __all(pc.vrows == 6 && pc.vcols == 6);
+    ubase = Us + (3 * hf) * 6 * PU + lt * 8 + wf8_slot(lt, lc & 3) + (lc >> 2);
+    raw_lds = (unsigned)(size_t)(lds_u8_t*)raws + (unsigned)wave * (18u * 256u);
+    th = wave & 1;
+    cb = wave >> 1;
+    mi = lane & 15;
+    mq = lane >> 4;
+    aoff = (16 * th + mi) * 8 + wf8_slot(16 * th + mi, mq);
+    boff = (16 * cb + mi) * 8 + wf8_slot(mi, mq);
+  };
 
   const bool tf0 = g.s[0].scale != nullptr, tf1 = g.c_split < Cg && g.s[1].scale != nullptr;
   if (tf0 || tf1) {
@@ -1414,15 +1500,14 @@
     }
   }
 
-  const unsigned raw_lds = (unsigned)(size_t)(lds_u8_t*)raws + (unsigned)wave * (18u * 256u);
-  auto issue_raw = [&](int kc) {
+  auto issue_raw = [&](const WfPatch& p, bool wfull, int kc) {
     const bool second = kc * 8 >= g.c_split;
     const unsigned long long sb = uniform_u64(second ? g.s[1].ptr : g.s[0].ptr);
     const int sH = second ? g.s[1].H : g.s[0].H, sW = second ? g.s[1].W : g.s[0].W;
     const int sC = second ? g.s[1].C : g.s[0].C;
     const int soy = second ? g.s[1].oy : g.s[0].oy, sox = second ? g.s[1].ox : g.s[0].ox;
     const int cl = kc * 8 - (second ? g.c_split : 0) + lc;
-    const unsigned o0 = ((unsigned)((img * sH + 4 * ty + soy) * sW + 4 * tx + sox) * sC + cl) * 4u;
+    const unsigned o0 = ((unsigned)((p.img * sH + 4 * p.ty + soy) * sW + 4 * p.tx + sox) * sC + cl) * 4u;
     const unsigned rs = (unsigned)sW * sC * 4u, cs = (unsigned)sC * 4u;
     if (wfull) {
       const unsigned oh = o0 + 3u * hf * cs;
@@ -1431,7 +1516,7 @@
 #pragma unroll
         for (int xx = 0; xx < 3; ++xx) dma4_sv(oh + (yy * rs + xx * cs), sb, raw_lds + (yy * 3 + xx) * 256u);
     } else {
-      const unsigned lr = (unsigned)max(vrows - 1, 0), lcn = (unsigned)max(vcols - 1, 0);
+      const unsigned lr = (unsigned)max(p.vrows - 1, 0), lcn = (unsigned)max(p.vcols - 1, 0);
 #pragma unroll
       for (int yy = 0; yy < 6; ++yy)
 #pragma unroll
@@ -1442,25 +1527,25 @@
   };
   const unsigned long long vbase = uniform_u64(V);
   const unsigned va_lds = (unsigned)(size_t)(lds_u8_t*)VAs, vb_lds = (unsigned)(size_t)(lds_u8_t*)VBs;
-  auto issue_v = [&](int kc, int half) {
+  auto issue_v = [&](int nn0, int kc, int half) {
     const int np = half ? 5 : 4, p0 = half ? PA : 0;
     const unsigned dst = half ? vb_lds : va_lds;
 #pragma unroll
     for (int j = 0; j < 5; ++j) {
       if (j < np) {
-        const int pc = wave + 8 * j;
-        dma_sv((unsigned)((((size_t)kc * 36 + p0 + (pc >> 1)) * N + n0) * 32) + (unsigned)((pc & 1) * 1024 + lane * 16),
-               vbase, dst + (unsigned)((pc >> 1) * PV * 4 + (pc & 1) * 1024));
+        const int pc2 = wave + 8 * j;
+        dma_sv((unsigned)((((size_t)kc * 36 + p0 + (pc2 >> 1)) * N + nn0) * 32) + (unsigned)((pc2 & 1) * 1024 + lane * 16),
+               vbase, dst + (unsigned)((pc2 >> 1) * PV * 4 + (pc2 & 1) * 1024));
       }
     }
   };
-  auto commit = [&](int kc) {
+  auto commit = [&](int kc, const WfPatch& p, bool wfull, const WfPatch& pn, bool wfn, int kn) {
     vm_wait<9>();
     float raw[18];
 #pragma unroll
     for (int q = 0; q < 18; ++q) raw[q] = raws[wave * (18 * 64) + q * 64 + lane];
     lgkm_wait0();
-    issue_raw(kc + 1 < nk ? kc + 1 : kc);
+    issue_raw(pn, wfn, kn);
     const bool second = kc * 8 >= g.c_split;
     const bool tf = second ? tf1 : tf0;
     if (tf) {
@@ -1470,7 +1555,7 @@
     }
     if (!wfull) {
 #pragma unroll
-      for (int q = 0; q < 18; ++q) raw[q] = (q / 3 < vrows && 3 * hf + q % 3 < vcols) ? raw[q] : 0.f;
+      for (int q = 0; q < 18; ++q) raw[q] = (q / 3 < p.vrows && 3 * hf + q % 3 < p.vcols) ? raw[q] : 0.f;
     }
 #pragma unroll
     for (int xx = 0; xx < 3; ++xx) {
@@ -1500,52 +1585,112 @@
     }
   };
 
-  const int th = wave & 1, cb = wave >> 1;
-  const int mi = lane & 15, mq = lane >> 4;
-  const int aoff = (16 * th + mi) * 8 + wf8_slot(16 * th + mi, mq);
-  const int boff = (16 * cb + mi) * 8 + wf8_slot(mi, mq);
-  floatx4 acc[36];
-#pragma unroll
-  for (int p = 0; p < 36; ++p) acc[p] = (floatx4){0.f, 0.f, 0.f, 0.f};
-
-  __syncthreads();
-  issue_raw(0);
-  issue_v(0, 0);
-  issue_v(0, 1);
-  for (int kc = 0; kc < nk; ++kc) {
-    const int kn = kc + 1 < nk ? kc + 1 : kc;
-    commit(kc);
-    vm_wait<23>();
-    lgkm_wait0();
-    raw_barrier();
-#pragma unroll
-    for (int p = 0; p < PA; ++p) {
-      const float2 a = *reinterpret_cast<const float2*>(Us + p * PU + aoff);
-      const float2 b = *reinterpret_cast<const float2*>(VAs + p * PV + boff);
-      acc[p] = __builtin_amdgcn_mfma_f32_16x16x4f32(b.x, a.x, acc[p], 0, 0, 0);
-      acc[p] = __builtin_amdgcn_mfma_f32_16x16x4f32(b.y, a.y, acc[p], 0, 0, 0);
-    }
-    vm_wait<18>();
-    lgkm_wait0();
-    raw_barrier();
-    issue_v(kn, 0);
-#pragma unroll
-    for (int p = PA; p < 36; ++p) {
-      const float2 a = *reinterpret_cast<const float2*>(Us + p * PU + aoff);
-      const float2 b = *reinterpret_cast<const float2*>(VBs + (p - PA) * PV + boff);
-      acc[p] = __builtin_amdgcn_mfma_f32_16x16x4f32(b.x, a.x, acc[p], 0, 0, 0);
-      acc[p] = __builtin_amdgcn_mfma_f32_16x16x4f32(b.y, a.y, acc[p], 0, 0, 0);
-    }
-    lgkm_wait0();
-    raw_barrier();
-    issue_v(kn, 1);
-  }
-  vm_wait<0>();
-  __syncthreads();
-  wf64_output(acc, g, e, N, T, Th, Tw, t0, n0, th, cb, mi, mq, lane, wave, lds);
+  if constexpr (!PERSIST) __syncthreads();
+  for (int it = 0;; ++it) {
+    roles();
+    if (it == 0) {
+      issue_raw(pc, wfc, 0);
+      issue_v(n0, 0, 0);
+      issue_v(n0, 0, 1);
+      if constexpr (PERSIST) {
+        if (tid == 0) sclaim[1] = wp_resolve(ctr, G, xcd, kfire);
+        __syncthreads();
+      }
+    } else {
+      issue_v(n0, 0, 1);
+    }
+    floatx4 acc[36];
+#pragma unroll
+    for (int p = 0; p < 36; ++p) acc[p] = (floatx4){0.f, 0.f, 0.f, 0.f};
+    WfPatch pn = pc;
+    bool wfn = wfc;
+    int n0n = n0, gnext = -1;
+    TI t0n = t0;
+    for (int kc = 0; kc < nk; ++kc) {
+      int kn = kc + 1 < nk ? kc + 1 : kc;
+      if constexpr (PERSIST) {
+        if (kc + 1 == nk) {
+          gnext = __builtin_amdgcn_readfirstlane(sclaim[1 + (it & 1)]);
+          if (gnext >= 0) {
+            n0n = (int)((unsigned)gnext % (unsigned)NB) * 64;
+            t0n = (unsigned)gnext / (unsigned)NB * 32u;
+            pn = wf_patch<4, TI>(t0n + (TI)lt, (TI)T, Th, Tw, g.Hg, g.Wg);
+            wfn = __all(pn.vrows == 6 && pn.vcols == 6);
+            kn = 0;
+          }
+        }
+      }
+      commit(kc, pc, wfc, pn, wfn, kn);
+      vm_wait<23>();
+      lgkm_wait0();
+      raw_barrier();
+#pragma unroll
+      for (int p = 0; p < PA; ++p) {
+        const float2 a = *reinterpret_cast<const float2*>(Us + p * PU + aoff);
+        const float2 b = *reinterpret_cast<const float2*>(VAs + p * PV + boff);
+        acc[p] = __builtin_amdgcn_mfma_f32_16x16x4f32(b.x, a.x, acc[p], 0, 0, 0);
+        acc[p] = __builtin_amdgcn_mfma_f32_16x16x4f32(b.y, a.y, acc[p], 0, 0, 0);
+      }
+      vm_wait<18>();
+      lgkm_wait0();
+      raw_barrier();
+      issue_v(n0n, kn, 0);
+#pragma unroll
+      for (int p = PA; p < 36; ++p) {
+        const float2 a = *reinterpret_cast<const float2*>(Us + p * PU + aoff);
+        const float2 b = *reinterpret_cast<const float2*>(VBs + (p - PA) * PV + boff);
+        acc[p] = __builtin_amdgcn_mfma_f32_16x16x4f32(b.x, a.x, acc[p], 0, 0, 0);
+        acc[p] = __builtin_amdgcn_mfma_f32_16x16x4f32(b.y, a.y, acc[p], 0, 0, 0);
+      }
+      lgkm_wait0();
+      raw_barrier();
+      if (!PERSIST || kc + 1 < nk) issue_v(n0, kn, 1);
+    }
+    if constexpr (!PERSIST) {
+      vm_wait<0>();
+      __syncthreads();
+    } else {
+      if (tid == 0 && gnext >= 0) kfire = atomicAdd(ctr + xcd, 1u);
+    }
+    wf64_output<FWD, TI>(acc, g, e, N, (TI)T, Th, Tw, t0, n0, th, cb, mi, mq, lane, wave, lds, grp);
+    if constexpr (!PERSIST) {
+      break;
+    } else {
+      if (gnext < 0) {
+        vm_wait<0>();
+        break;
+      }
+      if (tid == 0) sclaim[1 + ((it + 1) & 1)] = wp_resolve(ctr, G, xcd, kfire);
+      if constexpr (!FWD) {
+        lgkm_wait0();
+        raw_barrier();
+      }
+      t0 = t0n;
+      n0 = n0n;
+      grp = (int)(wp_block_of(G, (unsigned)gnext) % kStatGroups);
+    }
+  }
 }
 
 bool wino_fused64p_applies(const IgemmArgs& a) { return wino_fused64_applies(a) && a.a.Cg <= kWf64pMaxCg; }
+
+int g_wino_persist = getenv("UNET_WINO_PERSIST") ? atoi(getenv("UNET_WINO_PERSIST")) : 1;
+int g_wino_persist_wgs = -1;
+std::atomic<long long> g_wino_persist_launches{0};
+
+static size_t wino_persist_ctr_off(const IgemmArgs& a, int P) {
+  return ((size_t)P * a.N * a.a.Cg * 4 + 255) / 256 * 256;
+}
+bool wino_persist_applies(const IgemmArgs& a, int P, long long G, long long T) {
+  if (!g_wino_persist || G < 1 || G > 0x7fffffffLL || T + 64 > 0x7fffffffLL) return false;
+  if (G > num_cus() && G <= 4ll * num_cus()) return false;
+  return a.wino_ws != nullptr && wino_persist_ctr_off(a, P) + kWinoPersistCtrs * sizeof(unsigned) <= a.wino_ws_bytes;
+}
+static unsigned wino_persist_grid(long long G) {
+  long long w = num_cus();
+  if (g_wino_persist_wgs > 0) w = g_wino_persist_wgs;
+  return (unsigned)std::max<long long>(1, std::min(w, G));
+}
 
 hipError_t launch_wino_fused64p(const IgemmArgs& a, hipStream_t s) {
   if (!wino_fused64p_applies(a)) return hipErrorInvalidValue;
@@ -1556,13 +1701,29 @@
   const long long nw = (long long)a.N * g.Cg;
   const int NB = a.N / 64;
   const long long G = (T + 31) / 32 * NB;
-  hipLaunchKernelGGL(k_wino4f_w8, dim3((unsigned)((nw + 255) / 256)), dim3(256), 0, s, a.b, a.N, g.Cg, V);
-  hipLaunchKernelGGL(k_wino4f64p, dim3((unsigned)G), dim3(512), 0, s, g, (const float*)V, a.N, T, Th, Tw, NB, a.e);
+  const bool persist = wino_persist_applies(a, 36, G, T);
+  const unsigned pgrid = persist ? wino_persist_grid(G) : 0u;
+  unsigned* ctr = persist ? reinterpret_cast<unsigned*>(reinterpret_cast<char*>(a.wino_ws) + wino_persist_ctr_off(a, 36))
+                          : nullptr;
+  hipLaunchKernelGGL(k_wino4f_w8, dim3((unsigned)((nw + 255) / 256)), dim3(256), 0, s, a.b, a.N, g.Cg, V, ctr, pgrid);
+  const dim3 grid(persist ? pgrid : (unsigned)G);
+#define WF64P(P_, F_)                                                                                            \
+  hipLaunchKernelGGL((k_wino4f64p<P_, F_>), grid, dim3(512), 0, s, g, (const float*)V, a.N, T, Th, Tw, NB, a.e, \
+                     (unsigned)G, ctr)
+  if (persist) {
+    if (a.e.yref == nullptr) WF64P(true, true); else WF64P(true, false);
+    ++g_wino_persist_launches;
+  } else {
+    if (a.e.yref == nullptr) WF64P(false, true); else WF64P(false, false);
+  }
+#undef WF64P
   return hipGetLastError();
 }
 
-__global__ void k_wino2f_w8(const float* __restrict__ b, int N, int Cg, float* __restrict__ v) {
+__global__ void k_wino2f_w8(const float* __restrict__ b, int N, int Cg, float* __restrict__ v, unsigned* ctr,
+                            unsigned pgrid) {
   const long long i = blockIdx.x * (long long)blockDim.x + threadIdx.x;
+  if (ctr && i < kWinoPersistCtrs) ctr[i] = wp_ctr_init(pgrid, (int)i);
   if (i >= (long long)N * Cg) return;
   const int n = (int)(i / Cg), c = (int)(i - (long long)n * Cg);
   float g[3][3];
@@ -1587,36 +1748,55 @@
   }
 }
 
-template <int NC>
+template <int NC, bool PERSIST, bool FWD>
 __global__ __launch_bounds__(512, NC == 32 ? 2 : 1) void k_wino2f64(Gather g, const float* __restrict__ V, int N,
-                                                                   long long T, int Th, int Tw, int NB, Epilogue e) {
+                                                                   long long T, int Th, int Tw, int NB, Epilogue e,
+                                                                   unsigned G, unsigned* __restrict__ ctr) {
   constexpr int TT = 64;
   constexpr int PU = TT * 8;
   constexpr int PV = NC * 8;
   constexpr int NJ = NC / 32;
   __shared__ __attribute__((aligned(16))) float lds[16 * PU + 16 * PV];
+  __shared__ int sclaim[3];
   float* Us = lds;
   float* Vs = lds + 16 * PU;
   const int tid = threadIdx.x, lane = tid & 63, wave = tid >> 6;
-  long long bid = blockIdx.x;
-  const long long G = gridDim.x;
-  if ((G & 7) == 0) bid = (bid & 7) * (G >> 3) + (bid >> 3);
-  const int nb = (int)(bid % NB);
-  const long long t0 = (bid / NB) * TT;
-  const int n0 = nb * NC;
-
+  using TI = typename std::conditional<PERSIST, unsigned, long long>::type;
   const int lt = tid >> 3, lc = tid & 7;
-  const long long t = t0 + lt;
-  int img = 0, ty = 0, tx = 0;
-  if (t < T) {
-    tx = (int)(t % Tw);
-    const long long r = t / Tw;
-    ty = (int)(r % Th);
-    img = (int)(r / Th);
-  }
-  const int vrows = t < T ? min(4, g.Hg + 2 - 2 * ty) : 0;
-  const int vcols = t < T ? min(4, g.Wg + 2 - 2 * tx) : 0;
-  const bool wfull = __all(vrows == 4 && vcols == 4);
+
+  TI t0;
+  int n0, grp;
+  const int xcd = blockIdx.x & 7;
+  unsigned kfire = 0;
+  if constexpr (PERSIST) {
+    unsigned lo, hi;
+    wp_stretch(G, xcd, lo, hi);
+    const unsigned k0 = blockIdx.x >> 3;
+    int gid;
+    if (k0 < hi - lo) {
+      gid = (int)(lo + k0);
+    } else {
+      if (tid == 0) sclaim[0] = wp_resolve(ctr, G, xcd, k0);
+      __syncthreads();
+      gid = sclaim[0];
+      if (gid < 0) return;
+    }
+    gid = __builtin_amdgcn_readfirstlane(gid);
+    if (tid == 0) kfire = atomicAdd(ctr + xcd, 1u);
+    n0 = (int)((unsigned)gid % (unsigned)NB) * NC;
+    t0 = (unsigned)gid / (unsigned)NB * (unsigned)TT;
+    grp = (int)(wp_block_of(G, (unsigned)gid) % kStatGroups);
+  } else {
+    long long bid = blockIdx.x;
+    const long long Gd = gridDim.x;
+    if ((Gd & 7) == 0) bid = (bid & 7) * (Gd >> 3) + (bid >> 3);
+    n0 = (int)(bid % NB) * NC;
+    t0 = (bid / NB) * TT;
+    grp = (int)(blockIdx.x % kStatGroups);
+  }
+
+  WfPatch pc = wf_patch<2, TI>(t0 + (TI)lt, (TI)T, Th, Tw, g.Hg, g.Wg);
+  bool wfull = __all(pc.vrows == 4 && pc.vcols == 4);
   float* const ubase = Us + lt * 8 + wf8_slot(lt, lc & 3) + (lc >> 2);
   float raw[16];
   float sc = 1.f, sh = 0.f;
@@ -1636,7 +1816,7 @@
       sh = (second ? g.s[1].shift : g.s[0].shift)[cl];
     }
     const char* sb = reinterpret_cast<const char*>(sp);
-    const unsigned o0 = ((unsigned)((img * sH + 2 * ty + soy) * sW + 2 * tx + sox) * sC + cl) * 4u;
+    const unsigned o0 = ((unsigned)((pc.img * sH + 2 * pc.ty + soy) * sW + 2 * pc.tx + sox) * sC + cl) * 4u;
     const unsigned rs = (unsigned)sW * sC * 4u, cs = (unsigned)sC * 4u;
     if (wfull) {
 #pragma unroll
@@ -1645,7 +1825,7 @@
         for (int xx = 0; xx < 4; ++xx)
           raw[yy * 4 + xx] = *reinterpret_cast<const float*>(sb + (o0 + (yy * rs + xx * cs)));
     } else {
-      const unsigned lr = (unsigned)max(vrows - 1, 0), lcn = (unsigned)max(vcols - 1, 0);
+      const unsigned lr = (unsigned)max(pc.vrows - 1, 0), lcn = (unsigned)max(pc.vcols - 1, 0);
 #pragma unroll
       for (int yy = 0; yy < 4; ++yy)
 #pragma unroll
@@ -1660,9 +1840,9 @@
     __builtin_amdgcn_s_waitcnt(0x0F70);
 #pragma unroll
     for (int j = 0; j < 2 * NJ; ++j) {
-      const int pc = wave + 8 * j;
-      dma_sv((unsigned)((((size_t)kc * 16 + pc / NJ) * N + n0) * 32) + (unsigned)((pc % NJ) * 1024 + lane * 16),
-             vbase, vlds + (unsigned)((pc / NJ) * PV * 4 + (pc % NJ) * 1024));
+      const int pc2 = wave + 8 * j;
+      dma_sv((unsigned)((((size_t)kc * 16 + pc2 / NJ) * N + n0) * 32) + (unsigned)((pc2 % NJ) * 1024 + lane * 16),
+             vbase, vlds + (unsigned)((pc2 / NJ) * PV * 4 + (pc2 % NJ) * 1024));
     }
     if (scp) {
 #pragma unroll
@@ -1670,7 +1850,7 @@
     }
     if (!wfull) {
 #pragma unroll
-      for (int q = 0; q < 16; ++q) raw[q] = (q / 4 < vrows && q % 4 < vcols) ? raw[q] : 0.f;
+      for (int q = 0; q < 16; ++q) raw[q] = (q / 4 < pc.vrows && q % 4 < pc.vcols) ? raw[q] : 0.f;
     }
     float ev[4][4];
 #pragma unroll
@@ -1694,122 +1874,150 @@
   const int mi = lane & 15, mq = lane >> 4;
   const int aoff = (16 * th + mi) * 8 + wf8_slot(16 * th + mi, mq);
   const int boff = (16 * NJ * ch + mi) * 8 + wf8_slot(mi, mq);
-  floatx4 acc[16][NJ];
-#pragma unroll
-  for (int p = 0; p < 16; ++p)
-#pragma unroll
-    for (int j = 0; j < NJ; ++j) acc[p][j] = (floatx4){0.f, 0.f, 0.f, 0.f};
-  load(0);
-  for (int kc = 0; kc < nk; ++kc) {
-    commit(kc);
-    __syncthreads();
-    if (kc + 1 < nk) load(kc + 1);
-#pragma unroll
-    for (int p = 0; p < 16; ++p) {
-      const float2 a = *reinterpret_cast<const float2*>(Us + p * PU + aoff);
-#pragma unroll
-      for (int j = 0; j < NJ; ++j) {
-        const float2 b = *reinterpret_cast<const float2*>(Vs + p * PV + boff + 16 * j * 8);
-        acc[p][j] = __builtin_amdgcn_mfma_f32_16x16x4f32(b.x, a.x, acc[p][j], 0, 0, 0);
-        acc[p][j] = __builtin_amdgcn_mfma_f32_16x16x4f32(b.y, a.y, acc[p][j], 0, 0, 0);
-      }
-    }
-    __syncthreads();
-  }
-
-  const long long tt = t0 + 16 * th + mi;
   const bool want = e.stats || e.yref || e.colsum1;
   const int nsplit = e.n_split < N ? e.n_split : N;
-  const int grp = blockIdx.x % kStatGroups;
-#pragma unroll
-  for (int j = 0; j < NJ; ++j) {
-    const int col0 = n0 + 16 * NJ * ch + 16 * j + 4 * mq;
-    const bool second = col0 >= e.n_split;
-    float* dptr = second ? e.d[1].ptr : e.d[0].ptr;
-    const int dC = second ? e.d[1].C : e.d[0].C;
-    const int dcol = second ? col0 - e.n_split : col0;
-    const bool bwd_mask = e.yref != nullptr && !second;
-    const float4 bias = e.bias ? ld4(e.bias + col0) : make_float4(0.f, 0.f, 0.f, 0.f);
-    float4 bsc = make_float4(0.f, 0.f, 0.f, 0.f), bsh = bsc, bmu = bsc, bis = bsc;
-    if (bwd_mask) { bsc = ld4(e.bn_scale + col0); bsh = ld4(e.bn_shift + col0); bmu = ld4(e.bn_mean + col0); bis = ld4(e.bn_invstd + col0); }
-    float s1[4] = {0.f, 0.f, 0.f, 0.f}, s2[4] = {0.f, 0.f, 0.f, 0.f};
-    if (tt < T) {
-      const int ox = (int)(tt % Tw);
-      const long long rq = tt / Tw;
-      const int oy = (int)(rq % Th), on = (int)(rq / Th);
-      float4 y4[4];
-      if (bwd_mask) {
-#pragma unroll
-        for (int a = 0; a < 2; ++a)
-#pragma unroll
-          for (int bb = 0; bb < 2; ++bb) {
-            const int y = min(2 * oy + a, g.Hg - 1), x = min(2 * ox + bb, g.Wg - 1);
-            y4[a * 2 + bb] = ld4(e.yref + ((size_t)(on * g.Hg + y) * g.Wg + x) * dC + dcol);
-          }
-      }
-      __builtin_amdgcn_s_waitcnt(0x0F70);
-      float o[4][2][2];
-#pragma unroll
-      for (int r = 0; r < 4; ++r) {
-        float w[2][4];
-#pragma unroll
-        for (int xx = 0; xx < 4; ++xx) {
-          const float m0 = acc[0 * 4 + xx][j][r], m1 = acc[1 * 4 + xx][j][r];
-          const float m2 = acc[2 * 4 + xx][j][r], m3 = acc[3 * 4 + xx][j][r];
-          w[0][xx] = m0 + m1 + m2;
-          w[1][xx] = m1 - m2 - m3;
-        }
-#pragma unroll
-        for (int a = 0; a < 2; ++a) {
-          o[r][a][0] = w[a][0] + w[a][1] + w[a][2];
-          o[r][a][1] = w[a][1] - w[a][2] - w[a][3];
+  load(0);
+  if constexpr (PERSIST) {
+    if (tid == 0) sclaim[1] = wp_resolve(ctr, G, xcd, kfire);
+  }
+  for (int it = 0;; ++it) {
+    floatx4 acc[16][NJ];
+#pragma unroll
+    for (int p = 0; p < 16; ++p)
+#pragma unroll
+      for (int j = 0; j < NJ; ++j) acc[p][j] = (floatx4){0.f, 0.f, 0.f, 0.f};
+    float4 biasv[NJ];
+    if constexpr (PERSIST) {
+#pragma unroll
+      for (int j = 0; j < NJ; ++j)
+        biasv[j] = e.bias ? ld4(e.bias + n0 + 16 * NJ * ch + 16 * j + 4 * mq) : make_float4(0.f, 0.f, 0.f, 0.f);
+    }
+    for (int kc = 0; kc < nk; ++kc) {
+      commit(kc);
+      __syncthreads();
+      if (kc + 1 < nk) load(kc + 1);
+#pragma unroll
+      for (int p = 0; p < 16; ++p) {
+        const float2 a = *reinterpret_cast<const float2*>(Us + p * PU + aoff);
+#pragma unroll
+        for (int j = 0; j < NJ; ++j) {
+          const float2 b = *reinterpret_cast<const float2*>(Vs + p * PV + boff + 16 * j * 8);
+          acc[p][j] = __builtin_amdgcn_mfma_f32_16x16x4f32(b.x, a.x, acc[p][j], 0, 0, 0);
+          acc[p][j] = __builtin_amdgcn_mfma_f32_16x16x4f32(b.y, a.y, acc[p][j], 0, 0, 0);
         }
       }
-      const float bsv[4] = {bias.x, bias.y, bias.z, bias.w};
-      const float scv[4] = {bsc.x, bsc.y, bsc.z, bsc.w}, shv[4] = {bsh.x, bsh.y, bsh.z, bsh.w};
-      const float muv[4] = {bmu.x, bmu.y, bmu.z, bmu.w}, isv[4] = {bis.x, bis.y, bis.z, bis.w};
-#pragma unroll
-      for (int a = 0; a < 2; ++a) {
-        const int y = 2 * oy + a;
-        if (y >= g.Hg) continue;
-#pragma unroll
-        for (int bb = 0; bb < 2; ++bb) {
-          const int x = 2 * ox + bb;
-          if (x >= g.Wg) continue;
-          const size_t idx = ((size_t)(on * g.Hg + y) * g.Wg + x) * dC + dcol;
-          const float4 yq = bwd_mask ? y4[a * 2 + bb] : make_float4(0.f, 0.f, 0.f, 0.f);
-          const float yv[4] = {yq.x, yq.y, yq.z, yq.w};
-          float v[4];
-#pragma unroll
-          for (int r = 0; r < 4; ++r) v[r] = wf_epi(o[r][a][bb] + bsv[r], yv[r], scv[r], shv[r], muv[r], isv[r],
-                                                     bwd_mask, e.relu, s1[r], s2[r]);
-          st4(dptr + idx, make_float4(v[0], v[1], v[2], v[3]));
+      __syncthreads();
+    }
+
+    const TI tt = t0 + (TI)(16 * th + mi);
+    const int on0 = n0, ogrp = grp;
+    int gnext = -1;
+    if constexpr (PERSIST) {
+      gnext = __builtin_amdgcn_readfirstlane(sclaim[1 + (it & 1)]);
+      if (gnext >= 0) {
+        n0 = (int)((unsigned)gnext % (unsigned)NB) * NC;
+        t0 = (unsigned)gnext / (unsigned)NB * (unsigned)TT;
+        grp = (int)(wp_block_of(G, (unsigned)gnext) % kStatGroups);
+        pc = wf_patch<2, TI>(t0 + (TI)lt, (TI)T, Th, Tw, g.Hg, g.Wg);
+        wfull = __all(pc.vrows == 4 && pc.vcols == 4);
+        load(0);
+        if (tid == 0) kfire = atomicAdd(ctr + xcd, 1u);
+      }
+    }
+#pragma unroll
+    for (int j = 0; j < NJ; ++j) {
+      const int col0 = on0 + 16 * NJ * ch + 16 * j + 4 * mq;
+      const bool second = col0 >= e.n_split;
+      float* dptr = second ? e.d[1].ptr : e.d[0].ptr;
+      const int dC = second ? e.d[1].C : e.d[0].C;
+      const int dcol = second ? col0 - e.n_split : col0;
+      const bool bwd_mask = !FWD && e.yref != nullptr && !second;
+      float4 bias;
+      if constexpr (PERSIST) bias = biasv[j];
+      else bias = e.bias ? ld4(e.bias + col0) : make_float4(0.f, 0.f, 0.f, 0.f);
+      float4 bsc = make_float4(0.f, 0.f, 0.f, 0.f), bsh = bsc, bmu = bsc, bis = bsc;
+      if (bwd_mask) { bsc = ld4(e.bn_scale + col0); bsh = ld4(e.bn_shift + col0); bmu = ld4(e.bn_mean + col0); bis = ld4(e.bn_invstd + col0); }
+      float s1[4] = {0.f, 0.f, 0.f, 0.f}, s2[4] = {0.f, 0.f, 0.f, 0.f};
+      if (tt < (TI)T) {
+        const int ox = (int)(tt % (TI)Tw);
+        const TI rq = tt / (TI)Tw;
+        const int oy = (int)(rq % (TI)Th), on = (int)(rq / (TI)Th);
+        float4 y4[4];
+        if (bwd_mask) {
+#pragma unroll
+          for (int a = 0; a < 2; ++a)
+#pragma unroll
+            for (int bb = 0; bb < 2; ++bb) {
+              const int y = min(2 * oy + a, g.Hg - 1), x = min(2 * ox + bb, g.Wg - 1);
+              y4[a * 2 + bb] = ld4(e.yref + ((size_t)(on * g.Hg + y) * g.Wg + x) * dC + dcol);
+            }
+        }
+        if constexpr (!(PERSIST && FWD)) __builtin_amdgcn_s_waitcnt(0x0F70);
+        float o[4][2][2];
+#pragma unroll
+        for (int r = 0; r < 4; ++r) {
+          float w[2][4];
+#pragma unroll
+          for (int xx = 0; xx < 4; ++xx) {
+            const float m0 = acc[0 * 4 + xx][j][r], m1 = acc[1 * 4 + xx][j][r];
+            const float m2 = acc[2 * 4 + xx][j][r], m3 = acc[3 * 4 + xx][j][r];
+            w[0][xx] = m0 + m1 + m2;
+            w[1][xx] = m1 - m2 - m3;
+          }
+#pragma unroll
+          for (int a = 0; a < 2; ++a) {
+            o[r][a][0] = w[a][0] + w[a][1] + w[a][2];
+            o[r][a][1] = w[a][1] - w[a][2] - w[a][3];
+          }
+        }
+        const float bsv[4] = {bias.x, bias.y, bias.z, bias.w};
+        const float scv[4] = {bsc.x, bsc.y, bsc.z, bsc.w}, shv[4] = {bsh.x, bsh.y, bsh.z, bsh.w};
+        const float muv[4] = {bmu.x, bmu.y, bmu.z, bmu.w}, isv[4] = {bis.x, bis.y, bis.z, bis.w};
+#pragma unroll
+        for (int a = 0; a < 2; ++a) {
+          const int y = 2 * oy + a;
+          if (y >= g.Hg) continue;
+#pragma unroll
+          for (int bb = 0; bb < 2; ++bb) {
+            const int x = 2 * ox + bb;
+            if (x >= g.Wg) continue;
+            const size_t idx = ((size_t)(on * g.Hg + y) * g.Wg + x) * dC + dcol;
+            const float4 yq = bwd_mask ? y4[a * 2 + bb] : make_float4(0.f, 0.f, 0.f, 0.f);
+            const float yv[4] = {yq.x, yq.y, yq.z, yq.w};
+            float v[4];
+#pragma unroll
+            for (int r = 0; r < 4; ++r) v[r] = wf_epi(o[r][a][bb] + bsv[r], yv[r], scv[r], shv[r], muv[r], isv[r],
+                                                       bwd_mask, e.relu, s1[r], s2[r]);
+            st4(dptr + idx, make_float4(v[0], v[1], v[2], v[3]));
+          }
         }
       }
-    }
-    if (!want) continue;
-#pragma unroll
-    for (int r = 0; r < 4; ++r)
-#pragma unroll
-      for (int o2 = 1; o2 < 16; o2 <<= 1) {
-        s1[r] += __shfl_xor(s1[r], o2);
-        s2[r] += __shfl_xor(s2[r], o2);
-      }
-    if (mi == 0) {
-#pragma unroll
-      for (int r = 0; r < 4; ++r) {
-        const int col = col0 + r;
-        if (col < nsplit) {
-          double* st = e.yref ? e.bstats : e.stats;
-          if (st) {
-            atomicAdd(st + ((size_t)grp * nsplit + col) * 2 + 0, (double)s1[r]);
-            atomicAdd(st + ((size_t)grp * nsplit + col) * 2 + 1, (double)s2[r]);
+      if (!want) continue;
+#pragma unroll
+      for (int r = 0; r < 4; ++r)
+#pragma unroll
+        for (int o2 = 1; o2 < 16; o2 <<= 1) {
+          s1[r] += __shfl_xor(s1[r], o2);
+          s2[r] += __shfl_xor(s2[r], o2);
+        }
+      if (mi == 0) {
+#pragma unroll
+        for (int r = 0; r < 4; ++r) {
+          const int col = col0 + r;
+          if (col < nsplit) {
+            double* st = e.yref ? e.bstats : e.stats;
+            if (st) {
+              atomicAdd(st + ((size_t)ogrp * nsplit + col) * 2 + 0, (double)s1[r]);
+              atomicAdd(st + ((size_t)ogrp * nsplit + col) * 2 + 1, (double)s2[r]);
+            }
+          } else if (e.colsum1) {
+            atomicAdd(e.colsum1 + (size_t)ogrp * (N - nsplit) + (col - nsplit), (double)s1[r]);
           }
-        } else if (e.colsum1) {
-          atomicAdd(e.colsum1 + (size_t)grp * (N - nsplit) + (col - nsplit), (double)s1[r]);
         }
       }
     }
+    if (!PERSIST || gnext < 0) break;
+    if (tid == 0) sclaim[1 + ((it + 1) & 1)] = wp_resolve(ctr, G, xcd, kfire);
   }
 }
 
@@ -1838,11 +2046,25 @@
   const long long nw = (long long)a.N * g.Cg;
   const int NB = a.N / nc;
   const long long G = (T + 63) / 64 * NB;
-  hipLaunchKernelGGL(k_wino2f_w8, dim3((unsigned)((nw + 255) / 256)), dim3(256), 0, s, a.b, a.N, g.Cg, V);
-  if (nc == 64)
-    hipLaunchKernelGGL(k_wino2f64<64>, dim3((unsigned)G), dim3(512), 0, s, g, (const float*)V, a.N, T, Th, Tw, NB, a.e);
-  else
-    hipLaunchKernelGGL(k_wino2f64<32>, dim3((unsigned)G), dim3(512), 0, s, g, (const float*)V, a.N, T, Th, Tw, NB, a.e);
+  const bool persist = nc == 64 && wino_persist_applies(a, 16, G, T);
+  const unsigned pgrid = persist ? wino_persist_grid(G) : 0u;
+  unsigned* ctr = persist ? reinterpret_cast<unsigned*>(reinterpret_cast<char*>(a.wino_ws) + wino_persist_ctr_off(a, 16))
+                          : nullptr;
+  hipLaunchKernelGGL(k_wino2f_w8, dim3((unsigned)((nw + 255) / 256)), dim3(256), 0, s, a.b, a.N, g.Cg, V, ctr, pgrid);
+  const dim3 grid(persist ? pgrid : (unsigned)G);
+  const bool fwd = a.e.yref == nullptr;
+#define WF2(NC_, P_, F_)                                                                                            \
+  hipLaunchKernelGGL((k_wino2f64<NC_, P_, F_>), grid, dim3(512), 0, s, g, (const float*)V, a.N, T, Th, Tw, NB, a.e, \
+                     (unsigned)G, ctr)
+  if (persist) {
+    if (fwd) WF2(64, true, true); else WF2(64, true, false);
+    ++g_wino_persist_launches;
+  } else if (nc == 64) {
+    if (fwd) WF2(64, false, true); else WF2(64, false, false);
+  } else {
+    if (fwd) WF2(32, false, true); else WF2(32, false, false);
+  }
+#undef WF2
   return hipGetLastError();
 }
 
diff --git a/unet-segmentation_amd/unet_amd/_lib.py b/unet-segmentation_amd/unet_amd/_lib.py
--- a/unet-segmentation_amd/unet_amd/_lib.py
+++ b/unet-segmentation_amd/unet_amd/_lib.py
@@ -110,6 +110,7 @@
     "unet_fused_bnb_sites": (ctypes.c_longlong, [_i]),
     "unet_wgrad_oihw_sites": (ctypes.c_longlong, [_i]),
     "unet_igemm_plane_launches": (ctypes.c_longlong, [_i]),
+    "unet_wino_persist_launches": (ctypes.c_longlong, [_i]),
     "unet_tuning_save": (_i, [ctypes.c_char_p]),
     "unet_tuning_load": (_i, [ctypes.c_char_p]),
 }
```

After: 322.6 images/s, median of 6. +1.3%, better.
